# microsoft/VidTok

Hardware: AMD Instinct MI355X
Metric: encode+decode frames/sec, vidtok_kl_causal_488_4chn 17x256x256 (higher is better)
Workload: dtype bf16; 1 GPU; vidtok_kl_causal_488_4chn forward (encode+KL+decode), bf16, B=4 clips/GPU, 17x256x256; global_batch=4, launch=hipGraph replay (engine graph cache)

## Files before the change

### include/vidtok_amd.h

```cpp
#ifndef VIDTOK_AMD_H
#define VIDTOK_AMD_H

#include <stddef.h>
#include <stdint.h>

#ifdef __cplusplus
extern "C" {
#endif

typedef void* vt_stream;

typedef enum vt_status {
  VT_OK = 0,
  VT_ERR_ARG = -1,
  VT_ERR_HIP = -2,
  VT_ERR_UNSUPPORTED = -3
} vt_status;

typedef enum vt_dtype { VT_F32 = 0, VT_BF16 = 1, VT_I32 = 2, VT_BF16X3 = 3 , VT_F16 = 4 } vt_dtype;

typedef enum vt_tmode {
  VT_TPAD_ZERO = 0,
  VT_TPAD_REPLICATE = 1,
  VT_TPAD_CACHE = 2,
  VT_TPAD_ZERO_BACK = 3
} vt_tmode;

typedef enum vt_resmode {
  VT_RES_NONE = 0,
  VT_RES_ADD = 1,
  VT_RES_MIX = 2
} vt_resmode;

typedef enum vt_layout { VT_NDHWC = 0, VT_NCTHW = 1 } vt_layout;

const char* vt_last_error(void);
int vt_version(void);
int vt_graph_launch(void* graph_exec, vt_stream stream);
int vt_conv_max_lds_bytes(void);

int vt_set_option(const char* name, int32_t value);
int vt_get_option(const char* name, int32_t* value);
int vt_reset_options(void);
int vt_option_count(void);
const char* vt_option_name(int32_t i);

typedef struct vt_conv_desc {
  const void* x;
  const void* w;
  const float* bias;
  void* y;
  const void* res;
  const void* cache;
  const float* mix_factor;
  const float* ln_gamma;
  const float* ln_beta;
  void* ln_out;
  int32_t B, Ti, Hi, Wi, Cin;
  int32_t To, Ho, Wo, Cout;
  int32_t ldw;
  int32_t ldy;
  int32_t KT, KH, KW;
  int32_t st, sh, sw;
  int32_t pt, ph, pw;
  int32_t tmode, ncache;
  int32_t ups_t, ups_s;
  int32_t res_mode;
  int32_t res_tshift;
  int32_t Tr, ldr;
  int32_t out_layout;
  int32_t t_trim;
  int32_t dtype;
  int32_t out_dtype;
  int32_t nbatch;
  int32_t ln_mode;
  int32_t ln_keep_y;
  int32_t ldn;
  int32_t yt_mul, yt_off;
  int32_t ys_mul, ys_oh, ys_ow;
  float ln_eps;
  int64_t xs_z, ws_z, ys_z, rs_z;
  void* work;
  int64_t work_bytes;
} vt_conv_desc;

int vt_conv(const vt_conv_desc* d, vt_stream stream);
int64_t vt_conv_work_bytes(const vt_conv_desc* d);
int vt_conv_plan(const vt_conv_desc* d, int32_t* out8);
int vt_conv_profile(const vt_conv_desc* d, uint64_t* stamps_out, vt_stream stream);
int vt_conv_desc_size(void);

typedef struct vt_tblock_desc {
  const void* x;
  void* y;
  void* n_out;
  const void* w1; const float* b1;
  const void* w2; const float* b2;
  const float* norm1_gamma; const float* norm1_beta;
  const float* norm2_gamma; const float* norm2_beta;
  const float* next_gamma; const float* next_beta;
  int32_t dtype;
  int32_t C, ld;
  int32_t B, T;
  int64_t HW;
  int32_t tmode;
  int32_t keep_y;
  int32_t ln_next_mode;
  float eps;
  int32_t cache_offset;
  void* cache1;
  void* cache2;
} vt_tblock_desc;

int vt_tblock_desc_size(void);
int vt_temporal_block_supported(const vt_tblock_desc* d);
int vt_temporal_block(const vt_tblock_desc* d, vt_stream stream);
int vt_temporal_block_profile(const vt_tblock_desc* d, uint64_t* stamps_out, vt_stream stream);

int vt_layernorm_act(const void* x, int in_dtype, int64_t ldx, void* y, int out_dtype, int64_t ldy,
                     const float* gamma, const float* beta, int64_t M, int32_t C, float eps,
                     int32_t silu, vt_stream stream);

typedef enum { VT_GN_FRAME = 0, VT_GN_PIXEL = 1, VT_GN_CLIP = 2 } vt_gn_scope;
int64_t vt_groupnorm_work_bytes(int32_t B, int32_t T, int32_t groups, int32_t scope);
int vt_groupnorm_act(const void* x, int in_dtype, int64_t ldx, void* y, int out_dtype, int64_t ldy,
                     const float* gamma, const float* beta, int32_t B, int32_t T, int64_t HW, int32_t C,
                     int32_t groups, int32_t scope, float eps, int32_t silu, void* work, vt_stream stream);

int vt_flash_attention_supported(int32_t dtype, int32_t S, int32_t C, int32_t ldv);
int vt_flash_attention(const void* q, const void* k, const void* vt, const float* bias_v, void* o, int32_t dtype, int32_t Z, int32_t S,
                       int32_t C, int32_t ldv, float scale, vt_stream stream);

int vt_tanh_inplace(float* x, int64_t n, vt_stream stream);
int vt_softmax_rows(const float* s, void* p, int out_dtype, int64_t rows, int32_t cols,
                    int64_t ldp, float scale, vt_stream stream);

int vt_ncthw_to_ndhwc(const float* x, void* y, int out_dtype, int32_t B, int32_t C, int32_t T,
                      int32_t H, int32_t W, int32_t ldy, int32_t tpad, vt_stream stream);
int vt_ndhwc_to_ncthw(const void* x, int in_dtype, float* y, int32_t B, int32_t C, int32_t T,
                      int32_t H, int32_t W, int32_t ldx, int32_t ttrim, vt_stream stream);

int vt_time_avgpool3s2(const void* x, const void* cache, void* y, int dtype, int32_t B, int32_t Ti,
                       int64_t HW, int32_t C, int32_t tmode, vt_stream stream);
int vt_time_lerp2x(const void* x, void* y, int dtype, int32_t B, int32_t Ti, int64_t HWC,
                   vt_stream stream);
int vt_time_lerp2x_cat(const void* head, int32_t nh, const void* x, void* y, int dtype, int32_t B, int32_t Tx, int32_t skip,
                       int64_t HWC, vt_stream stream);

int vt_pack_conv_weight(const float* w, void* out, int32_t out_dtype, int32_t Cout, int32_t Cin, int32_t cin_p, int32_t taps_in,
                        int32_t taps_out, const int32_t* mix_host, int64_t ldw, vt_stream stream);

int vt_fsq_consts(const int32_t* levels_host, int32_t D, float* out_host);
int vt_kl_sample(const float* h, const float* noise, float* z, float* kl_out, int32_t B,
                 int32_t zc, int64_t S, vt_stream stream);
int vt_fsq_quantize(const float* h, float* z, int32_t* indices, const int32_t* levels_host,
                    int32_t D, int32_t B, int64_t S, vt_stream stream);
int vt_fsq_indices_to_codes(const int32_t* indices, float* z, const int32_t* levels_host,
                            int32_t D, int32_t B, int64_t S, vt_stream stream);
int vt_fsq_quantize_cb(const float* h, float* z, int32_t* indices, const int32_t* levels_host,
                       int32_t D, int32_t B, int32_t ncb, int64_t S, vt_stream stream);
int vt_fsq_indices_to_codes_cb(const int32_t* indices, float* z, const int32_t* levels_host,
                               int32_t D, int32_t B, int32_t ncb, int64_t S, vt_stream stream);
int64_t vt_fsq_aux_work_floats(const int32_t* levels_host, int32_t D, int32_t B, int64_t S);
int vt_fsq_aux_stats(const float* h, const int32_t* levels_host, int32_t D, int32_t B, int64_t S,
                     float inv_temperature, float* work, float* out3, vt_stream stream);
int vt_fsq_aux_stats_avg(const float* h, const int32_t* levels_host, int32_t D, int32_t B, int64_t S,
                         float inv_temperature, float* work, float* out3, float* avg_out, vt_stream stream);
int vt_fsq_aux_loss(const float* stats3, const float* codebook_entropy, float diversity_gamma, float entropy_weight,
                    float commitment_weight, float* out, vt_stream stream);
int vt_entropy(const float* avg, int64_t J, float* out, vt_stream stream);

typedef struct vt_model_config {
  int32_t version;
// ... 164 lines not shown
```

### vidtok_amd/build.py

```python
import hashlib
import os
import shutil
import subprocess
import sys

HERE = os.path.dirname(os.path.abspath(__file__))
CSRC = os.path.join(HERE, "csrc")
LIB = os.path.join(HERE, "libvidtok_amd.so")
SOURCES = ["conv_igemm_bf16.hip", "conv_igemm_f16.hip", "conv_igemm_f32.hip", "conv_igemm_x3.hip", "conv_igemm_act.hip", "conv_igemm.hip", "conv_in8.hip", "conv_ws2.hip", "conv_narrow.hip", "tblock_ws128.hip", "attention.hip", "pointwise.hip", "groupnorm.hip", "regularizers.hip", "metrics.hip", "lpips.hip", "lpips_grad.hip", "video_io.hip", "segments.hip", "grad.hip", "grad_decoder.hip", "packing.hip", "error.cpp", "options.cpp", "model.cpp"]
HEADERS = ["common.h", "conv_common.h", "conv_select.h", "conv_igemm_kernel.h", "options.h", "row8.h", os.path.join("..", "..", "include", "vidtok_amd.h")]
FLAGS = ["--offload-arch=gfx950", "-O3", "-std=c++17", "-fPIC", "-Wall", "-Wno-unused-function"]
EXTRA_FLAGS = {"conv_ws2.hip": ["-fno-slp-vectorize"], "tblock_ws128.hip": ["-fno-slp-vectorize"]}


NO_SPILL = {"tblock_ws128.hip": "tblock_pair_kernel", "conv_ws2.hip": "conv3x3_ws2_kernel"}
LLVM_BIN = "/opt/rocm/lib/llvm/bin"


def kernel_resources(obj):
    import re
    import tempfile
    with tempfile.TemporaryDirectory() as d:
        fat, dev = os.path.join(d, "fat.bin"), os.path.join(d, "dev.o")
        subprocess.check_call([f"{LLVM_BIN}/llvm-objcopy", "--dump-section", f".hip_fatbin={fat}", obj])
        subprocess.check_call([f"{LLVM_BIN}/clang-offload-bundler", "--unbundle", "--type=o", f"--input={fat}",
                               "--targets=hipv4-amdgcn-amd-amdhsa--gfx950", f"--output={dev}"])
        notes = subprocess.check_output([f"{LLVM_BIN}/llvm-readelf", "--notes", dev], text=True)
    out = []
    for blk in notes.split("- .agpr_count:")[1:]:
        g = lambda k: re.search(r"\." + k + r":\s+(\S+)", blk).group(1)
        out.append((g("name"), int(g("vgpr_count")), int(blk.split()[0]), int(g("vgpr_spill_count")), int(g("private_segment_fixed_size"))))
    return out


def check_no_spill(objdir):
    if not all(os.path.exists(os.path.join(LLVM_BIN, t)) for t in ("llvm-objcopy", "clang-offload-bundler", "llvm-readelf")):
        print("[vidtok_amd.build] spill check skipped: LLVM binutils not found under", LLVM_BIN, flush=True)
        return
    bad = []
    for src, kern in NO_SPILL.items():
        obj = os.path.join(objdir, os.path.splitext(src)[0] + ".o")
        for name, _v, _a, spill, scratch in kernel_resources(obj):
            measured = name.endswith("Lb1EEEvNS_10TBlockArgsE") or name.endswith("Lb1EEEvNS_8ConvArgsE")
            if kern in name and not measured and (spill or scratch):
                bad.append(f"{name}: {spill} spilled registers, {scratch} B scratch")
    if bad:
        raise RuntimeError("register spills in hand-scheduled kernels (wrong results, not only slow):\n  " + "\n  ".join(bad))


def _hipcc():
    for c in (os.environ.get("HIPCC"), shutil.which("hipcc"), "/opt/rocm/bin/hipcc"):
        if c and os.path.exists(c):
            return c
    raise RuntimeError("hipcc not found (set HIPCC)")


def _src_digest(src):
    h = hashlib.sha256()
    for f in [src] + HEADERS:
        with open(os.path.join(CSRC, f), "rb") as fh:
            h.update(fh.read())
    h.update(" ".join(FLAGS + EXTRA_FLAGS.get(src, [])).encode())
    return h.hexdigest()


def _digest():
    h = hashlib.sha256()
    for src in SOURCES:
        h.update(_src_digest(src).encode())
    return h.hexdigest()


def build(force: bool = False, verbose: bool = True) -> str:
    stamp = LIB + ".stamp"
    dig = _digest()
    if not force and os.path.exists(LIB) and os.path.exists(stamp) and open(stamp).read() == dig:
        return LIB
    hipcc = _hipcc()
    objdir = os.path.join(HERE, "build")
    os.makedirs(objdir, exist_ok=True)
    objs = []
    procs = []
    for src in SOURCES:
        obj = os.path.join(objdir, os.path.splitext(src)[0] + ".o")
        objs.append(obj)
        ostamp, odig = obj + ".stamp", _src_digest(src)
        if not force and os.path.exists(obj) and os.path.exists(ostamp) and open(ostamp).read() == odig:
            continue
        if os.path.exists(ostamp):
            os.remove(ostamp)
        cmd = [hipcc, *FLAGS, *EXTRA_FLAGS.get(src, []), "-x", "hip", "-c", os.path.join(CSRC, src), "-o", obj]
        if verbose:
            print("[vidtok_amd.build]", " ".join(cmd), flush=True)
        procs.append((src, subprocess.Popen(cmd), ostamp, odig))
    failed = []
    for src, p, ostamp, odig in procs:
        if p.wait() != 0:
            failed.append(src)
        else:
            with open(ostamp, "w") as f:
                f.write(odig)
    if failed:
        raise RuntimeError(f"hipcc failed on {', '.join(failed)}")
    check_no_spill(objdir)
    cmd = [hipcc, "--offload-arch=gfx950", "-shared", "-fPIC", *objs, "-o", LIB]
    if verbose:
        print("[vidtok_amd.build]", " ".join(cmd), flush=True)
    subprocess.check_call(cmd)
    with open(stamp, "w") as f:
        f.write(dig)
    return LIB


if __name__ == "__main__":
    build(force="--force" in sys.argv)
    print(LIB)
```

### vidtok_amd/csrc/conv_common.h

```cpp
#pragma once
#include "common.h"
#include "options.h"

namespace {

constexpr int kRowBytes = 128;

struct FastDiv {
  unsigned mul, shift, d;
};
inline FastDiv make_fastdiv(unsigned d) {
  FastDiv f;
  f.d = d;
  if (d <= 1) { f.mul = 0; f.shift = 0; return f; }
  unsigned l = 0;
  while ((1ull << l) < d) ++l;
  f.mul = (unsigned)((((1ull << 32) * ((1ull << l) - d)) / d) + 1);
  f.shift = l - 1;
  return f;
}
__device__ __forceinline__ unsigned fast_div(unsigned n, const FastDiv& f) {
  if (f.d <= 1) return n;
  const unsigned t = __umulhi(n, f.mul);
  return (t + ((n - t) >> 1)) >> f.shift;
}

struct ConvArgs;
__device__ __forceinline__ long long out_row(const ConvArgs& p, int m);

struct ConvArgs {
  const char* x;
  const char* w;
  const float* bias;
  char* y;
  const char* res;
  const char* cache;
  const float* mix_factor;
  const float* ln_gamma;
  const float* ln_beta;
  char* ln_out;
  int B, Ti, Hi, Wi, Cin;
  int To, Ho, Wo, Cout;
  int ldw, ldy;
  int KT, KH, KW;
  int st, sh, sw;
  int pt, ph, pw;
  int tmode, ncache;
  int ups_t, ups_s;
  int res_mode, res_tshift, Tr, ldr;
  int out_layout, t_trim;
  int M, K, ntaps, nsteps;
  int m_tiles, n_tiles;
  int ln_mode, ln_keep_y, ldn;
  float ln_eps;
  FastDiv fd_wo, fd_ho, fd_to;
  FastDiv fd_hw;
  int yt_mul;
  long long yt_step, yt_base;
  int ys_mul, ys_oh, ys_ow;
  int lds_epi;
  int hw_tiles;
  unsigned x_bytes, w_bytes;
  unsigned c_bytes;
  long long xs_z, ws_z, ys_z, rs_z;
  int in8_rt, in8_ct, in8_ctl2, in8_segs;
  int tskip;
  int ksplit;
  unsigned plane_bytes;
  int nt_store;
  unsigned long long* prof;
  int prof_mode;
};

struct split3_t {
  float v;
};
template <typename MT>
struct is_split3 {
  [[maybe_unused]] static constexpr bool value = false;
};
template <>
struct is_split3<split3_t> {
  [[maybe_unused]] static constexpr bool value = true;
};
template <typename MT>
struct storage_of {
  typedef MT type;
};
template <>
struct storage_of<split3_t> {
  typedef float type;
};

__device__ __forceinline__ void split3_x(const u32x4& r0, const u32x4& r1, u32x4& hi, u32x4& lo) {
#pragma unroll
  for (int e = 0; e < 4; ++e) {
    const float f0 = __uint_as_float(e < 2 ? r0[2 * e] : r1[2 * e - 4]);
    const float f1 = __uint_as_float(e < 2 ? r0[2 * e + 1] : r1[2 * e - 3]);
    const uint32_t h = pack_bf16x2(f0, f1);
    hi[e] = h;
    float d0, d1;
    asm("v_sub_f32_e32 %0, %1, %2" : "=v"(d0) : "v"(f0), "v"(h << 16));
    asm("v_sub_f32_e32 %0, %1, %2" : "=v"(d1) : "v"(f1), "v"(h & 0xffff0000u));
    lo[e] = pack_bf16x2(d0, d1);
  }
}
__device__ __forceinline__ void mma_bf16(const u32x4& wfrag, const u32x4& xfrag, f32x16& acc) {
  acc = __builtin_amdgcn_mfma_f32_32x32x16_bf16(__builtin_bit_cast(bf16x8, wfrag), __builtin_bit_cast(bf16x8, xfrag), acc, 0, 0, 0);
}

template <typename MT>
__device__ __forceinline__ void mma_step(const u32x4& wfrag, const u32x4& xfrag, f32x16& acc);

template <>
__device__ __forceinline__ void mma_step<bf16_t>(const u32x4& wfrag, const u32x4& xfrag, f32x16& acc) {
  acc = __builtin_amdgcn_mfma_f32_32x32x16_bf16(__builtin_bit_cast(bf16x8, wfrag),
                                                __builtin_bit_cast(bf16x8, xfrag), acc, 0, 0, 0);
}
template <>
__device__ __forceinline__ void mma_step<f16_t>(const u32x4& wfrag, const u32x4& xfrag, f32x16& acc) {
  acc = h16<f16_t>::mfma32(wfrag, xfrag, acc);
}
template <>
__device__ __forceinline__ void mma_step<float>(const u32x4& wfrag, const u32x4& xfrag, f32x16& acc) {
#pragma unroll
  for (int e = 0; e < 4; ++e)
    acc = __builtin_amdgcn_mfma_f32_32x32x2f32(__uint_as_float(wfrag[e]), __uint_as_float(xfrag[e]),
                                               acc, 0, 0, 0);
}

__device__ __forceinline__ int xcd_remap(int bid, int nblk) {
  const int xcd = bid & 7, loc = bid >> 3;
  const int q = nblk >> 3, r = nblk & 7;
  const int start = (xcd < r) ? xcd * (q + 1) : r * (q + 1) + (xcd - r) * q;
  return start + loc;
}

template <typename TOut>
struct Quad;
template <>
struct Quad<float> {
  f32x4 v;
  __device__ __forceinline__ float get(int e) const { return v[e]; }
};
template <typename H>
struct Quad16 {
  u32x2 v;
  __device__ __forceinline__ float get(int e) const {
    const uint32_t w = v[e >> 1];
    return (e & 1) ? h16<H>::hi(w) : h16<H>::lo(w);
  }
};
template <>
struct Quad<bf16_t> : Quad16<bf16_t> {};
// ... 95 lines not shown
```

### vidtok_amd/csrc/conv_igemm.hip

```cpp
#include <algorithm>
#include <atomic>
#include <type_traits>

#include "conv_select.h"

namespace {

template <typename H>
__global__ __launch_bounds__(256) void splitk_reduce_kernel(const float* __restrict__ part, int planes, long long M, int Cout, const float* __restrict__ bias,
                                                            const H* __restrict__ res, H* __restrict__ y) {
  const long long n8 = M * (Cout / 8);
  const long long plane = M * (long long)Cout;
  for (long long i = (long long)blockIdx.x * blockDim.x + threadIdx.x; i < n8; i += (long long)gridDim.x * blockDim.x) {
    const long long e = i * 8;
    const int c = (int)(e % Cout);
    float v[8];
    {
      const f32x4 a = *reinterpret_cast<const f32x4*>(part + e), b = *reinterpret_cast<const f32x4*>(part + e + 4);
#pragma unroll
      for (int k = 0; k < 4; ++k) { v[k] = a[k]; v[4 + k] = b[k]; }
    }
    for (int pz = 1; pz < planes; ++pz) {
      const f32x4 a = *reinterpret_cast<const f32x4*>(part + pz * plane + e), b = *reinterpret_cast<const f32x4*>(part + pz * plane + e + 4);
#pragma unroll
// ... 54 lines not shown
  return VT_OK;
}

}

extern "C" int vt_conv_max_lds_bytes(void) { return 163840; }

extern "C" int vt_conv_plan(const vt_conv_desc* d, int32_t* out8) {
  VT_CHECK_ARG(out8 != nullptr, "vt_conv_plan: null output");
  ConvArgs a;
  ConvPlan p;
  const int rc = conv_decide(d, a, p);
  if (rc != VT_OK) return rc;
  out8[4] = p.ln_fused ? 1 : 0;
  out8[5] = 1;
  out8[6] = p.kernel;
  out8[7] = 0;
  switch (p.kernel) {
    case CONV_NARROW:
      vt_conv_narrow_plan(&a, out8);
      out8[5] = p.narrow_mode == 2 ? 2 : 1;
      break;
    case CONV_WS2:
      out8[0] = 64; out8[1] = 128; out8[2] = 8;
      out8[3] = (a.Wo / 16) * (a.Ho / 4) * a.B * a.To;
      break;
    case CONV_IN8:
      out8[0] = 128; out8[1] = 128; out8[2] = 4;
      out8[3] = a.M / 128;
      out8[7] = 1;
      break;
    case CONV_IGEMM: {
      const TileShape& t = kTileShapes[p.igemm.tile];
      out8[0] = t.bm(); out8[1] = t.bn(); out8[2] = t.waves();
      out8[3] = (int32_t)((long long)((a.M + t.bm() - 1) / t.bm()) * ((a.Cout + t.bn() - 1) / t.bn()) * p.nbatch);
      if (d->ln_mode != 0 && !p.ln_fused) out8[5] += 1;
      if (splitk_runs(p, a, d, false)) out8[5] += 1;
      out8[7] = p.igemm.tile == TILE_256x256 ? (p.igemm.ln256 ? 1 : 0) : (p.igemm.stages == 4 ? 2 : 0);
      break;
    }
  }
  return VT_OK;
}

extern "C" int vt_conv_profile(const vt_conv_desc* d, uint64_t* stamps_out, vt_stream stream_) {
  VT_CHECK_ARG(stamps_out != nullptr, "vt_conv_profile: null output");
  ConvArgs a;
  ConvPlan p;
  const int rc = conv_decide(d, a, p, reinterpret_cast<unsigned long long*>(stamps_out));
  if (rc != VT_OK) return rc;
  a.prof_mode = vt_opt(OPT_WS_PROF_MODE);
  if (p.kernel == CONV_WS2) return vt_ws2_launch(&a, d->dtype, stream_);
  VT_CHECK_ARG(p.kernel == CONV_IGEMM && ((d->dtype == VT_BF16 && d->out_dtype == VT_BF16) || d->dtype == VT_BF16X3) && d->ln_mode == 0 &&
                   p.igemm.tile == TILE_256x256,
               "vt_conv_profile: bf16 / split-bf16 launches on the 256 x 256 tile without LayerNorm, or on the weight-stationary kernel");
  return launch_igemm(d->dtype, false, a, p.igemm, p.nbatch, stream_);
}

extern "C" int64_t vt_conv_work_bytes(const vt_conv_desc* d) {
  ConvArgs a;
  ConvPlan p;
  if (conv_decide(d, a, p) != VT_OK || p.kernel != CONV_IGEMM) return 0;
  return (int64_t)p.splitk_planes * a.M * a.Cout * 4;
}

extern "C" int vt_conv(const vt_conv_desc* d, vt_stream stream_) {
  ConvArgs a;
  ConvPlan p;
  int rc = conv_decide(d, a, p);
  if (rc != VT_OK) return rc;
  switch (p.kernel) {
    case CONV_WS2: return vt_ws2_launch(&a, d->dtype, stream_);
    case CONV_NARROW: return vt_conv_narrow_launch(&a, stream_, p.narrow_mode);
    case CONV_IN8: return vt_conv_in8_launch(&a, d->dtype, stream_);
    case CONV_IGEMM: break;
  }
  rc = splitk_runs(p, a, d, true) ? launch_splitk(d, a, p, reinterpret_cast<hipStream_t>(stream_))
                                  : launch_igemm(d->dtype, d->out_dtype == VT_F32, a, p.igemm, p.nbatch, stream_);
  if (rc != VT_OK || d->ln_mode == 0 || p.ln_fused) return rc;
  return vt_layernorm_act(d->y, d->out_dtype, d->ldy, d->ln_out, d->out_dtype, d->ldn, d->ln_gamma, d->ln_beta, a.M, d->Cout,
                          d->ln_eps, d->ln_mode == 2 ? 1 : 0, stream_);
}

extern "C" int vt_conv_act(const vt_conv_desc* d, int32_t act, vt_stream stream_) {
  VT_CHECK_ARG(act == VT_ACT_RELU, "vt_conv_act: act %d (VT_ACT_RELU = %d is the one activation)", act, VT_ACT_RELU);
  ConvArgs a;
  ConvPlan p;
  const int rc = conv_decide(d, a, p, nullptr, act);
  if (rc != VT_OK) return rc;
  VT_CHECK_ARG(d->dtype != VT_BF16X3 && d->out_dtype == d->dtype, "vt_conv_act: fp32, bf16 or fp16 arithmetic with results in the same type");
  VT_CHECK_ARG(d->out_layout == VT_NDHWC && d->res_mode == VT_RES_NONE && d->ln_mode == 0 && p.nbatch == 1 && a.yt_mul == 1 && a.ys_mul == 1,
               "vt_conv_act: NDHWC output without residual, LayerNorm, batching or interleave");
  return vt_igemm_dispatch_relu(&a, &p.igemm, d->dtype, stream_);
}
```

### vidtok_amd/csrc/conv_igemm_kernel.h

```cpp
#include <atomic>
#include <type_traits>

#pragma once
#include "conv_select.h"

namespace {

__device__ __forceinline__ float act_relu(float v) { return v > 0.0f ? v : 0.0f; }

template <typename TOut, int TM, int TN, bool GENERAL = true, int ACT = 0>
__device__ __forceinline__ void conv_epilogue(const ConvArgs& p, f32x16 (&acc)[TN][TM], int m_blk, int n_blk, int bn_tile,
                                              int wm, int wn, int lane, long long z) {
  TOut* __restrict__ yg = reinterpret_cast<TOut*>(p.y) + z * p.ys_z;
  const TOut* __restrict__ rg = reinterpret_cast<const TOut*>(p.res) + z * p.rs_z;
  const long long HWo = (long long)p.Ho * p.Wo;
  const bool has_res = p.res_mode != VT_RES_NONE;
  const int nlast = p.Cout - 1;
  const int nq = n_blk + wn * TN * 32 + 4 * (lane >> 5);

  float alpha = 0.0f;
  if (p.res_mode == VT_RES_MIX) alpha = 1.0f / (1.0f + __expf(-p.mix_factor[0]));

  bool store_ok[TM];
  long long mr[TM], ybase[TM];
// ... 259 lines not shown
    {
      const int prl = wm * 32 + (lane & 31);
#pragma unroll
      for (int a = 0; a < 4; ++a)
#pragma unroll
        for (int g = 0; g < 4; ++g) {
          const int c = wn * 128 + 32 * a + 8 * g + 4 * h;
          f32x4 bq;
          if (p.bias) bq = *reinterpret_cast<const f32x4*>(p.bias + n_blk + c);
          else bq[0] = bq[1] = bq[2] = bq[3] = 0.0f;
          f32x4 v;
#pragma unroll
          for (int e = 0; e < 4; ++e) v[e] = acc[a][PZ][4 * g + e] + bq[e];
          *reinterpret_cast<f32x4*>(T + prl * 256 + (((c >> 2) ^ (prl & 63)) << 2)) = v;
        }
    }
    __syncthreads();
#pragma unroll
    for (int it = 0; it < 8; ++it) {
      const int r = rsub + RS * it;
      const int m = m_blk + ((RS * it) >> 5) * 64 + PZ * 32 + rsub + ((RS * it) & 31);
      const long long orow = out_row(p, m);
      const f32x4 t0 = *reinterpret_cast<const f32x4*>(T + r * 256 + (((2 * j) ^ (r & 63)) << 2));
      const f32x4 t1 = *reinterpret_cast<const f32x4*>(T + r * 256 + (((2 * j + 1) ^ (r & 63)) << 2));
      f32x2 v[4] = {f32x2{t0[0], t0[1]}, f32x2{t0[2], t0[3]}, f32x2{t1[0], t1[1]}, f32x2{t1[2], t1[3]}};
      if (p.res_mode == VT_RES_ADD) {
#pragma unroll
        for (int q = 0; q < 4; ++q) v[q] = f32x2{rq[it].get(2 * q), rq[it].get(2 * q + 1)} + v[q];
      } else if (p.res_mode == VT_RES_MIX) {
#pragma unroll
        for (int q = 0; q < 4; ++q) v[q] = f32x2{rq[it].get(2 * q), rq[it].get(2 * q + 1)} * alpha + v[q] * (1.0f - alpha);
      }
      if constexpr (ACT == VT_ACT_RELU) {
#pragma unroll
        for (int q = 0; q < 4; ++q) v[q] = f32x2{act_relu(v[q][0]), act_relu(v[q][1])};
      }
      if (p.ln_keep_y || !has_ln) {
        const float yv[8] = {v[0][0], v[0][1], v[1][0], v[1][1], v[2][0], v[2][1], v[3][0], v[3][1]};
        Oct<TOut>::store(yg + orow * p.ldy + n_blk + 8 * j, yv, p.nt_store != 0);
      }
      if (!has_ln) continue;
      float o[8];
      if constexpr (sizeof(TOut) == 2) {
        const f32x2 s = (v[0] + v[1]) + (v[2] + v[3]);
        f32x2 qq = v[0] * v[0];
#pragma unroll
        for (int q = 1; q < 4; ++q) qq = __builtin_elementwise_fma(v[q], v[q], qq);
        float nm;
        const float rstd = ln_row_stats<32>(s[0] + s[1], qq[0] + qq[1], p.ln_eps, &nm);
        const f32x2 rstd2 = {rstd, rstd}, nm2 = {nm, nm}, c2 = {kNegLog2e, kNegLog2e};
#pragma unroll
        for (int q = 0; q < 4; ++q) {
          f32x2 u = __builtin_elementwise_fma(__builtin_elementwise_fma(v[q], rstd2, nm2), lg[q], lb[q]);
          if (p.ln_mode == 2) {
            const f32x2 den = __builtin_elementwise_fma(f32x2{__builtin_amdgcn_exp2f(u[0]), __builtin_amdgcn_exp2f(u[1])}, c2, c2);
            u = u * f32x2{__builtin_amdgcn_rcpf(den[0]), __builtin_amdgcn_rcpf(den[1])};
          }
          o[2 * q] = u[0];
          o[2 * q + 1] = u[1];
        }
      } else {
        const f32x2 s = (v[0] + v[1]) + (v[2] + v[3]);
        const float mean = group_sum_dpp<32>(s[0] + s[1]) * (1.0f / 256.0f);
        f32x2 d[4], qq = {0.f, 0.f};
#pragma unroll
        for (int q = 0; q < 4; ++q) {
          d[q] = v[q] - mean;
          qq = __builtin_elementwise_fma(d[q], d[q], qq);
        }
        const float rstd = __builtin_amdgcn_rsqf(__builtin_fmaf(group_sum_dpp<32>(qq[0] + qq[1]), 1.0f / 256.0f, p.ln_eps));
#pragma unroll
        for (int q = 0; q < 4; ++q) {
          f32x2 u = __builtin_elementwise_fma(d[q] * rstd, lg[q], lb[q]);
          if (p.ln_mode == 2) {
            const f32x2 t = u * -1.4426950408889634f;
            const f32x2 e = f32x2{__builtin_amdgcn_exp2f(t[0]), __builtin_amdgcn_exp2f(t[1])} + 1.0f;
            u = u * f32x2{__builtin_amdgcn_rcpf(e[0]), __builtin_amdgcn_rcpf(e[1])};
          }
          o[2 * q] = u[0];
          o[2 * q + 1] = u[1];
        }
      }
      Oct<TOut>::store(ng + orow * p.ldn + 8 * j, o, p.nt_store != 0);
    }
  };
  half(std::integral_constant<int, 0>{});
  half(std::integral_constant<int, 1>{});
}

[[maybe_unused]] __device__ u32x4 g_zero_page[8];


template <typename MT, typename TOut, int WAVES_M, int WAVES_N, int TM, int TN, bool FAST, int ROWB, int STAGES, bool BUF, int LN256 = 0, bool PROF = false, int SCHED = 0, int ACT = 0>
__global__ __launch_bounds__(64 * WAVES_M * WAVES_N, 2) void conv_igemm_glds_kernel(const ConvArgs p) {
#if defined(__HIP_DEVICE_COMPILE__)
  constexpr int THREADS = 64 * WAVES_M * WAVES_N;
  constexpr int NS = ROWB / 16;
  constexpr int RSTEP = THREADS / NS;
  constexpr int ROWS_PER_WAVE = 64 / NS;
  constexpr int SWZ_SHIFT = (ROWB == 128) ? 1 : 2;
  constexpr int VEC = 16 / (int)sizeof(MT);
  constexpr int BK = ROWB / (int)sizeof(MT);
  constexpr int KS = ROWB / 32;
  constexpr int BM = WAVES_M * TM * 32;
  constexpr int BN = WAVES_N * TN * 32;
  constexpr int A_VECS = BM * NS / THREADS;
  constexpr int B_VECS = BN * NS / THREADS;
  constexpr int IPS = A_VECS + B_VECS;
  constexpr int A_BYTES = BM * ROWB;
  constexpr int STAGE_BYTES = (BM + BN) * ROWB;
  constexpr int D = STAGES - 1;
  constexpr bool X3 = is_split3<MT>::value;
  static_assert(ROWB == 128 || ROWB == 64, "row bytes");
  static_assert(A_VECS >= 1 && B_VECS >= 1 && BM % RSTEP == 0 && BN % RSTEP == 0, "tile / workgroup mismatch");
  static_assert(D >= 1 && D <= 3 && (D - 1) * IPS <= 63, "pipeline depth");

  extern __shared__ __attribute__((aligned(16))) char smem[];
  typedef __attribute__((address_space(3))) void* lds_ptr_t;
  typedef const __attribute__((address_space(1))) void* glb_ptr_t;

  const int tid = threadIdx.x;
  const int lane = tid & 63;
  const int wave = tid >> 6;
  const int wm = wave % WAVES_M;
  const int wn = wave / WAVES_M;

  const int tile = xcd_remap(blockIdx.x, p.m_tiles * p.n_tiles);
  const int nt = tile / p.m_tiles;
  int mt = tile - nt * p.m_tiles;
  if (p.hw_tiles > 0) {
    const int per_b = p.hw_tiles * p.To;
    const int b = mt / per_b;
    const int r = mt - b * per_b;
    const int hwt = r / p.To;
    mt = (b * p.To + (r - hwt * p.To)) * p.hw_tiles + hwt;
  }
  const int m_blk = mt * BM;
  const int n_blk = nt * BN;

  const long long z = blockIdx.z;
  const MT* __restrict__ xg = reinterpret_cast<const MT*>(p.x) + z * p.xs_z;
  const MT* __restrict__ wg = reinterpret_cast<const MT*>(p.w) + z * p.ws_z;
  const MT* __restrict__ cg = reinterpret_cast<const MT*>(p.cache);
  const MT* zero = reinterpret_cast<const MT*>(g_zero_page);
  constexpr unsigned kOob = 0xFFFF0000u;
  unsigned ext_x = BUF ? p.x_bytes : 0u, ext_w = BUF ? p.w_bytes : 0u;
  const MT* x_cur = xg;
  if constexpr (PROF) {
    if (p.prof_mode & 1) ext_x = 0u;
    if (p.prof_mode & 2) ext_w = 0u;
  }

  const int pos = tid % NS;
  const int srow = tid / NS;
  const int chunk = pos ^ ((srow >> SWZ_SHIFT) & (NS - 1));
  const int lds_row_off = __builtin_amdgcn_readfirstlane(wave * ROWS_PER_WAVE * ROWB);

  const int Hv = p.Hi << p.ups_s, Wv = p.Wi << p.ups_s;
  const int Tv = p.Ti << p.ups_t;

  int a_b[A_VECS], a_t0[A_VECS], a_h0[A_VECS], a_w0[A_VECS];
#pragma unroll
  for (int i = 0; i < A_VECS; ++i) {
    const int m = m_blk + srow + RSTEP * i;
    if (m < p.M) {
      const unsigned r1 = fast_div((unsigned)m, p.fd_wo);
// ... 527 lines not shown
    read_frags(0, 0, 0);
    for (int s = 0; s < nsteps; ++s) {
      s_cur = s;
      stamp(0);
      const bool fire = s < n_fire;
      if (!fire && BUF) ext_x = ext_w = 0u;
      const bool fire_rt = BUF || fire;
      const int dst = (stage + D) % STAGES;
      const int nxt = (stage + 1 == STAGES) ? 0 : stage + 1;
#pragma unroll
      for (int k = 0; k < KS; ++k) {
        if (((k ^ wgrp) & 1) == 0) __builtin_amdgcn_s_setprio(2);
        else __builtin_amdgcn_s_setprio(0);
        if (k + 1 < KS) read_frags(stage, k + 1, (k + 1) & 1);
#pragma unroll
        for (int qq = 0; qq < TM * TN; ++qq) {
          const int a = qq / TM, b = qq % TM;
          const int q = k * TM * TN + qq;
          if (k + 1 == KS && qq == BAR_AT) {
            stamp(1);
            asm volatile("s_waitcnt lgkmcnt(0)" ::: "memory");
            wait_vmcnt<(D - 1) * IPS>();
            stamp(2);
            __builtin_amdgcn_s_barrier();
            asm volatile("" ::: "memory");
            stamp(3);
            read_frags(nxt, 0, 0);
          }
          mma_step<MT>(wf[k & 1][a], xf[k & 1][b], acc[a][b]);
          if ((q + 1) % MPP1 == 0) {
            const int piece = q / MPP1;
            if (piece < IPS && fire_rt) fire_piece(piece, dst);
          }
          if (q + 1 == NM / 2) {
            if (s + 1 < n_fire) prep_step(s + 1 + D);
          }
        }
      }
      stage = nxt;
      stamp(4);
    }
    __builtin_amdgcn_s_setprio(0);
  } else {
  for (int s = 0; s < nsteps; ++s) {
    s_cur = s;
    stamp(0);
    const int newer = min(D - 1, nsteps - 1 - s);
    if (D >= 3 && newer >= 2) wait_vmcnt<2 * IPS>();
    else if (D >= 2 && newer >= 1) wait_vmcnt<IPS>();
    else wait_vmcnt<0>();
    stamp(1);
    __builtin_amdgcn_s_barrier();
    asm volatile("" ::: "memory");
    stamp(2);
    const bool fire = s < n_fire;
    if (fire) prep_step(s + D);
    else if (BUF) ext_x = ext_w = 0u;
    const bool fire_rt = BUF || fire;
    stamp(3);
    if (EIGHT_WAVES) {
      compute_stage(stage, TagTrue{}, fire_rt, (stage + D) % STAGES);
    } else {
      if (fire_rt) {
#pragma unroll
        for (int q = 0; q < IPS; ++q) fire_piece(q, (stage + D) % STAGES);
      }
      compute_stage(stage, TagFalse{}, false, 0);
    }
    stage = (stage + 1 == STAGES) ? 0 : stage + 1;
    stamp(4);
  }
  }
  if constexpr (BUF) wait_vmcnt<0>();
  if constexpr (PROF) {
    if (blockIdx.x == 0 && blockIdx.y == 0 && blockIdx.z == 0 && lane == 0 && p.prof != nullptr) {
      constexpr int NW = THREADS / 64;
      for (int i = 0; i < 4 * 8; ++i) p.prof[(tid >> 6) * 32 + i] = stamps[((i / 8) * NW + (tid >> 6)) * 8 + (i % 8)];
    }
  }
  if constexpr (LN256 != 0) {
    static_assert(WAVES_M == 4 && WAVES_N == 2 && TM == 2 && TN == 4 && std::is_same<typename storage_of<MT>::type, TOut>::value, "LN256: the 8-wave 256 x 256 tile");
    static_assert(STAGES * STAGE_BYTES >= 128 * 256 * 4, "LN256: the transposition tile must fit the ring");
    if constexpr (!BUF) wait_vmcnt<0>();
    conv_epilogue_lds256<TOut, ACT>(p, acc, m_blk, n_blk, wm, wn, lane, tid, smem, z);
    return;
  }
  if constexpr (WAVES_M == 2 && WAVES_N == 2 && TM == 2 && TN == 2 && STAGES * STAGE_BYTES >= 128 * 128 * 4) {
    if (p.lds_epi && m_blk + BM <= p.M && n_blk + BN <= p.Cout) {
      if constexpr (!BUF) wait_vmcnt<0>();
      conv_epilogue_lds128<TOut, ACT>(p, acc, m_blk, n_blk, wm, wn, lane, tid, smem, z);
      return;
    }
  }
  conv_epilogue<TOut, TM, TN, (TM * TN < 8), ACT>(p, acc, m_blk, n_blk, BN, wm, wn, lane, z);
#endif
}

template <typename MT, typename TOut, int WAVES_M, int WAVES_N, int TM, int TN, bool FAST, int LN256 = 0, int STAGES = 2, int ROWB = kRowBytes, int ACT = 0>
int launch_variant(const ConvArgs& a_in, int nbatch, hipStream_t stream) {
  constexpr int BM = WAVES_M * TM * 32;
  constexpr int BN = WAVES_N * TN * 32;
  constexpr int BK = ROWB / (int)sizeof(MT);
  constexpr int THREADS = 64 * WAVES_M * WAVES_N;
  constexpr int LDS = STAGES * (BM + BN) * ROWB;
  ConvArgs a = a_in;
  a.m_tiles = (a.M + BM - 1) / BM;
  a.n_tiles = (a.Cout + BN - 1) / BN;
  a.nsteps = FAST ? a.ntaps * (a.Cin / BK) : (a.K + BK - 1) / BK;
  if (a.ksplit) {
    VT_CHECK_ARG(FAST, "vt_conv: split-K needs the tap-walk form");
    a.nsteps = (a.ksplit == 1 ? a.KH * a.KW : a.KW) * (a.Cin / BK);
  }
  constexpr int kOctAlign = 16 / (int)sizeof(TOut) > 4 ? 8 : 4;
  a.lds_epi = (vt_opt(OPT_CONV_LDSEPI) != 0 && a.out_layout == VT_NDHWC && a.ldy % kOctAlign == 0 &&
               (a.res_mode == VT_RES_NONE || a.ldr % kOctAlign == 0) && (a.ln_mode == 0 || a.ldn % kOctAlign == 0)) ? 1 : 0;
  a.hw_tiles = 0;
  if (conv_tinner() && a.KT > 1 && a.To > 1 && ((long long)a.Ho * a.Wo) % BM == 0) a.hw_tiles = (int)(((long long)a.Ho * a.Wo) / BM);
  const unsigned long long xb = (unsigned long long)a.B * a.Ti * a.Hi * a.Wi * a.Cin * sizeof(MT);
  const unsigned long long wb = (unsigned long long)a.Cout * a.ldw * sizeof(MT);
  const unsigned long long cb = a.tmode == VT_TPAD_CACHE ? (unsigned long long)a.B * a.ncache * a.Hi * a.Wi * a.Cin * sizeof(MT) : 0ull;
  const bool cache_ok = a.tmode != VT_TPAD_CACHE ||
                        (FAST && (nbatch == 1 || a.ksplit) && a.prof == nullptr && cb < 0xFFFF0000ull && ((long long)a.Ho * a.Wo) % BM == 0 && a.ups_t == 0);
  const bool buf = conv_buf() && xb < 0xFFFF0000ull && wb < 0xFFFF0000ull && cache_ok &&
                   a.KH <= 8 && a.KW <= 8;
  VT_CHECK_ARG(!a.ksplit || buf, "vt_conv: split-K needs the descriptor gather");
  a.tskip = (FAST && buf && vt_opt(OPT_CONV_TSKIP) != 0 && a.tmode == VT_TPAD_ZERO && a.KT > 1 && a.pt > 0 && a.ups_t == 0 && !a.ksplit &&
             nbatch == 1 && a.prof == nullptr && ((long long)a.Ho * a.Wo) % BM == 0) ? 1 : 0;
  constexpr bool EIGHT = WAVES_M * WAVES_N == 8;
  constexpr int SCHED_BUF = !(EIGHT && FAST) ? 0
                            : (is_split3<MT>::value ? ((ROWB == 64 && STAGES == 4) ? 5 : 0)
                               : ((ROWB == kRowBytes && STAGES == 2) ? (is_h16<MT>::value ? 2 : 1) : 0));
  const void* kern;
  if (buf) {
    a.x_bytes = (unsigned)xb;
    a.w_bytes = (unsigned)wb;
    a.c_bytes = (unsigned)cb;
    kern = reinterpret_cast<const void*>(&conv_igemm_glds_kernel<MT, TOut, WAVES_M, WAVES_N, TM, TN, FAST, ROWB, STAGES, true, LN256, false, SCHED_BUF, ACT>);
  } else {
    kern = reinterpret_cast<const void*>(&conv_igemm_glds_kernel<MT, TOut, WAVES_M, WAVES_N, TM, TN, FAST, ROWB, STAGES, false, LN256, false, 0, ACT>);
  }
  int lds_bytes = LDS;
  static std::atomic<bool> attr_done[3][kMaxDevices];
  int ki = buf ? 1 : 0;
  if (a.prof != nullptr) {
    if constexpr (EIGHT && FAST && LN256 == 0 && ACT == 0 && (SCHED_BUF == 2 || SCHED_BUF == 5) && !std::is_same<MT, f16_t>::value &&
                  std::is_same<typename storage_of<MT>::type, TOut>::value) {
      VT_CHECK_ARG(buf, "vt_conv_profile: descriptor gather only");
      kern = reinterpret_cast<const void*>(&conv_igemm_glds_kernel<MT, TOut, WAVES_M, WAVES_N, TM, TN, FAST, ROWB, STAGES, true, 0, true, SCHED_BUF>);
      lds_bytes = LDS + 4096;
      ki = 2;
    } else {
      VT_CHECK_ARG(false, "vt_conv_profile: only the bf16 / split-bf16 8-wave 256 x 256 tile without fused LayerNorm is instrumented");
    }
  }
  if (const int rc = vt_dynamic_lds(kern, lds_bytes, attr_done[ki])) return rc;
  const long long nblk = (long long)a.m_tiles * a.n_tiles;
  VT_CHECK_ARG(nblk < (1ll << 31), "vt_conv: too many tiles (%lld)", nblk);
  void* kargs[] = {&a};
  VT_CHECK_HIP(hipLaunchKernel(kern, dim3((unsigned)nblk, 1, (unsigned)nbatch), dim3(THREADS), kargs, lds_bytes, stream));
  return VT_OK;
}

template <typename MT, typename TOut, TileKind T, bool FAST, int LN256 = 0, int STAGES = 2, int ROWB = kRowBytes, int ACT = 0>
int launch_tile(const ConvArgs& a, int nbatch, hipStream_t stream) {
  constexpr TileShape S = kTileShapes[T];
  return launch_variant<MT, TOut, S.wm, S.wn, S.tm, S.tn, FAST, LN256, STAGES, ROWB, ACT>(a, nbatch, stream);
}

#define VT_CHECK_VARIANT(cond) \
  VT_CHECK_ARG(cond, "vt_conv: no instantiation of tile %d with fast %d, ln256 %d, stages %d, row bytes %d in this arithmetic", (int)v.tile, (int)v.fast, v.ln256, v.stages, v.rowb)

template <typename MT, typename TOut, TileKind T>
int launch_fast_or_general(const ConvArgs& a, const IgemmVariant& v, int nbatch, hipStream_t stream) {
  VT_CHECK_VARIANT(v.ln256 == 0 && v.stages == 2 && v.rowb == kRowBytes);
  return v.fast ? launch_tile<MT, TOut, T, true>(a, nbatch, stream) : launch_tile<MT, TOut, T, false>(a, nbatch, stream);
}

template <typename MT, typename TOut>
int dispatch_tile(const ConvArgs& a, const IgemmVariant& v, int nbatch, hipStream_t stream) {
  switch (v.tile) {
    case TILE_256x32: return launch_fast_or_general<MT, TOut, TILE_256x32>(a, v, nbatch, stream);
    case TILE_256x64: return launch_fast_or_general<MT, TOut, TILE_256x64>(a, v, nbatch, stream);
    case TILE_256x256:
      if constexpr (is_split3<MT>::value) {
        if (v.rowb == 64) {
          VT_CHECK_VARIANT(v.fast && v.stages == 4);
          return v.ln256 ? launch_tile<MT, TOut, TILE_256x256, true, 1, 4, 64>(a, nbatch, stream) : launch_tile<MT, TOut, TILE_256x256, true, 0, 4, 64>(a, nbatch, stream);
        }
      } else if constexpr (std::is_same<MT, TOut>::value) {
        if (v.ln256) {
          VT_CHECK_VARIANT(v.fast && v.stages == 2 && v.rowb == kRowBytes);
          return launch_tile<MT, TOut, TILE_256x256, true, 1>(a, nbatch, stream);
        }
      }
      return launch_fast_or_general<MT, TOut, TILE_256x256>(a, v, nbatch, stream);
    default:
      if (v.stages == 4) {
        VT_CHECK_VARIANT(v.tile == TILE_128x128 && v.fast && v.ln256 == 0 && v.rowb == kRowBytes);
        return launch_tile<MT, TOut, TILE_128x128, true, 0, 4>(a, nbatch, stream);
      }
      return launch_fast_or_general<MT, TOut, TILE_128x128>(a, v, nbatch, stream);
  }
}

}
```

### vidtok_amd/csrc/conv_select.h

```cpp
#pragma once
#include "conv_common.h"

namespace {

inline bool conv_buf() { return vt_opt(OPT_CONV_BUF) != 0; }
inline bool conv_tinner() { return vt_opt(OPT_CONV_TINNER) != 0; }

inline bool in8_eligible(const ConvArgs& a, int nbatch, int dtype, int out_dtype, bool ln_fused, int ln_mode_asked) {
  if (vt_opt(OPT_CONV_IN8) == 0 || !conv_buf() || nbatch != 1 || a.prof != nullptr) return false;
  if (!vt_is_h16(dtype) || out_dtype != dtype || a.Cin != 8 || a.Cout != 128 || a.ldw != 216) return false;
  if (a.KT != 3 || a.KH != 3 || a.KW != 3 || a.st != 1 || a.sh != 1 || a.sw != 1 || a.pt != 2 || a.ph != 1 || a.pw != 1) return false;
  if (a.To != a.Ti || a.Ho != a.Hi || a.Wo != a.Wi || a.ups_t || a.ups_s || a.tmode == VT_TPAD_CACHE) return false;
  if (a.out_layout != VT_NDHWC || a.res_mode != VT_RES_NONE || a.yt_mul != 1 || a.ys_mul == 2) return false;
  if (a.Wo < 8 || !((a.Wo % 128 == 0) || (128 % a.Wo == 0)) || ((long long)a.Ho * a.Wo) % 128 != 0) return false;
  if (ln_mode_asked != 0 && !ln_fused) return false;
  if (a.ldy % 8 != 0 || (a.ln_mode != 0 && a.ldn % 8 != 0) || vt_opt(OPT_CONV_LDSEPI) == 0) return false;
  const unsigned long long xb = (unsigned long long)a.B * a.Ti * a.Hi * a.Wi * 8 * 2;
  return xb < 0xFFFF0000ull;
}

inline bool deep_ring_eligible(const ConvArgs& a, int nbatch, int elem_bytes) {
  if (vt_opt(OPT_CONV_DEEP) == 0 || a.prof != nullptr) return false;
  const int bk = kRowBytes / elem_bytes;
  if (a.Cin % bk != 0 || a.ntaps * (a.Cin / bk) < 8) return false;
  const long long tiles = (long long)((a.M + 127) / 128) * ((a.Cout + 127) / 128) * nbatch;
  return tiles <= device_cus();
}

enum TileKind { TILE_256x32 = 0, TILE_256x64, TILE_256x256, TILE_128x128 };
struct TileShape {
  int wm, wn, tm, tn;
  constexpr int bm() const { return wm * tm * 32; }
  constexpr int bn() const { return wn * tn * 32; }
  constexpr int waves() const { return wm * wn; }
};
constexpr TileShape kTileShapes[4] = {{4, 1, 2, 1}, {4, 1, 2, 2}, {4, 2, 2, 4}, {2, 2, 2, 2}};

inline bool ws_eligible(const ConvArgs& a, int nbatch, bool h16_io) {
  if (!h16_io || vt_opt(OPT_CONV_WS) == 0) return false;
  if (a.Cin != 128 || a.Cout != 128 || a.ldw != 1152 || a.ldy != 128) return false;
  if (a.KT != 1 || a.KH != 3 || a.KW != 3 || a.st != 1 || a.sh != 1 || a.sw != 1 || a.ph != 1 || a.pw != 1) return false;
  if (a.ups_t || a.ups_s || a.Ho != a.Hi || a.Wo != a.Wi || a.To != a.Ti) return false;
  if (a.Ho % 8 != 0 || a.Wo % 16 != 0 || (long long)a.Ho * a.Wo * 256 > (1ll << 30)) return false;
  if (a.out_layout != VT_NDHWC || a.yt_mul != 1 || a.ys_mul == 2 || nbatch != 1) return false;
  if (a.res_mode == VT_RES_MIX) return false;
  if (a.res_mode == VT_RES_ADD && (a.ldr != 128 || a.Tr != a.To || a.res_tshift != 0 || (reinterpret_cast<uintptr_t>(a.res) & 15))) return false;
  if ((reinterpret_cast<uintptr_t>(a.y) & 15) || (a.bias && (reinterpret_cast<uintptr_t>(a.bias) & 15))) return false;
  return true;
}

inline bool narrow_eligible(const ConvArgs& a, int nbatch, int dtype, int out_dtype, int ln_mode) {
  if ((!vt_is_h16(dtype) && dtype != VT_BF16X3) || out_dtype != VT_F32 || a.out_layout != VT_NCTHW || vt_opt(OPT_CONV_NARROW) == 0) return false;
  if (a.Cin != 128 || a.Cout > 4 || a.KT != 3 || a.KH != 3 || a.KW != 3) return false;
  if (a.st != 1 || a.sh != 1 || a.sw != 1 || a.ph != 1 || a.pw != 1 || a.pt < 1 || a.pt > 2) return false;
  if (a.ups_t || a.ups_s || a.Ho != a.Hi || a.Wo != a.Wi || a.To != a.Ti) return false;
  if (a.res_mode != VT_RES_NONE || ln_mode != 0 || nbatch != 1 || a.yt_mul != 1 || a.ys_mul == 2) return false;
  if ((long long)a.Ho * a.Wo * 256 > (1ll << 30)) return false;
  if (a.tmode == VT_TPAD_CACHE && a.ncache < a.pt) return false;
  if (dtype == VT_BF16X3 && a.ldw != 27 * 128) return false;
  return true;
}

inline TileKind select_tile(const ConvArgs& a, int nbatch) {
  auto blocks = [&](int bm, int bn) {
    return (long long)((a.M + bm - 1) / bm) * ((a.Cout + bn - 1) / bn) * nbatch;
  };
  const bool vec_epi = a.out_layout == VT_NDHWC && (a.ldy & 3) == 0 && (a.res_mode == VT_RES_NONE || (a.ldr & 3) == 0);
  if (a.Cout <= 32) return TILE_256x32;
  if (a.Cout <= 64) return TILE_256x64;
  const int force = vt_opt(OPT_CONV_TILE);
  if (a.Cout % 256 == 0 && vec_epi && force != 128 && (blocks(256, 256) >= vt_opt(OPT_CONV_TILE_MIN) || force == 256)) return TILE_256x256;
  return TILE_128x128;
}

inline bool lds256_plain_eligible(const ConvArgs& a, int nbatch, bool h16_io) {
  return h16_io && a.ln_mode == 0 && a.prof == nullptr && vt_opt(OPT_CONV_LDSEPI) != 0 &&
         a.M % 256 == 0 && a.Cout % 256 == 0 && nbatch == 1 && a.Cin % (kRowBytes / 2) == 0 && a.out_layout == VT_NDHWC &&
         (a.ldy & 7) == 0 && (a.res_mode == VT_RES_NONE || ((a.ldr & 7) == 0 && a.Tr == a.To && a.res_tshift == 0));
}

struct IgemmVariant {
  TileKind tile;
  bool fast;
  int ln256;
  int stages;
  int rowb;
};

enum ConvKernel { CONV_IGEMM = 0, CONV_NARROW = 2, CONV_WS2 = 3, CONV_IN8 = 4 };

struct ConvPlan {
  ConvKernel kernel;
  IgemmVariant igemm;
  IgemmVariant split;
  int splitk_planes;
  bool ln_fused;
  int nbatch;
  int narrow_mode;
};

inline int splitk_planes(const vt_conv_desc* d, const ConvArgs& a, const ConvPlan& p, TileKind tile) {
  if (vt_opt(OPT_CONV_SPLITK) == 0 || !conv_buf()) return 0;
  if (!vt_is_h16(d->dtype) || d->out_dtype != d->dtype || p.nbatch != 1 || p.ln_fused || a.prof != nullptr) return 0;
  const bool by_kt = a.KT == 3 && a.st == 1, by_kh = a.KT == 1 && a.KH == 3;
  if (!(by_kt || by_kh) || a.ups_t || a.ups_s || a.out_layout != VT_NDHWC || a.yt_mul != 1 || a.ys_mul == 2) return 0;
  if (a.Cin % 64 != 0 || a.Cout % 128 != 0 || a.ldy != a.Cout || a.KT * a.KH * a.KW * a.Cin < 4608) return 0;
  if (a.res_mode == VT_RES_MIX || (a.res_mode == VT_RES_ADD && (a.ldr != a.Cout || a.Tr != a.To || a.res_tshift != 0))) return 0;
  if (a.tmode == VT_TPAD_CACHE && ((long long)a.Ho * a.Wo) % 256 != 0) return 0;
  const unsigned long long xb = (unsigned long long)a.B * a.Ti * a.Hi * a.Wi * a.Cin * 2, wb = (unsigned long long)a.Cout * a.ldw * 2;
  if (xb >= 0xFFFF0000ull || wb >= 0xFFFF0000ull) return 0;
  if (tile != TILE_256x256 && tile != TILE_128x128) return 0;
  const long long clip_tiles = (((long long)a.To * a.Ho * a.Wo + 127) / 128) * ((a.Cout + 127) / 128);
  return clip_tiles <= device_cus() ? 3 : 0;
}

inline int conv_decide(const vt_conv_desc* d, ConvArgs& a, ConvPlan& p, unsigned long long* prof = nullptr, int act = 0) {
  VT_CHECK_ARG(d != nullptr, "vt_conv: null descriptor");
  VT_CHECK_ARG(d->x && d->w && d->y, "vt_conv: null tensor pointer");
  VT_CHECK_ARG(d->dtype == VT_F32 || d->dtype == VT_BF16 || d->dtype == VT_F16 || d->dtype == VT_BF16X3, "vt_conv: dtype %d", d->dtype);
  VT_CHECK_ARG((d->out_dtype == d->dtype && d->dtype != VT_BF16X3) || d->out_dtype == VT_F32, "vt_conv: out_dtype %d with dtype %d",
               d->out_dtype, d->dtype);
  const int vec = vt_is_h16(d->dtype) ? 8 : 4;
  if (d->dtype == VT_BF16X3)
    VT_CHECK_ARG(d->ldw % 32 == 0 && d->ldw >= (d->KT * d->KH * d->KW * d->Cin + 31) / 32 * 32 && d->nbatch <= 1,
                 "vt_conv: VT_BF16X3 needs ldw = K rounded up to 32 (got %d) and nbatch 1", d->ldw);
  VT_CHECK_ARG(d->B > 0 && d->Ti > 0 && d->Hi > 0 && d->Wi > 0 && d->Cin > 0, "vt_conv: bad input dims");
  VT_CHECK_ARG(d->To > 0 && d->Ho > 0 && d->Wo > 0 && d->Cout > 0, "vt_conv: bad output dims");
  VT_CHECK_ARG(d->Cin % vec == 0, "vt_conv: Cin=%d must be a multiple of %d (pad the channel dim)", d->Cin, vec);
  VT_CHECK_ARG(d->KT > 0 && d->KH > 0 && d->KW > 0 && d->KT * d->KH * d->KW <= 64, "vt_conv: bad taps");
  VT_CHECK_ARG(d->st > 0 && d->sh > 0 && d->sw > 0, "vt_conv: bad strides");
  VT_CHECK_ARG(d->ldw >= d->KT * d->KH * d->KW * d->Cin && d->ldw % vec == 0, "vt_conv: ldw=%d", d->ldw);
  VT_CHECK_ARG((reinterpret_cast<uintptr_t>(d->x) & 15) == 0 && (reinterpret_cast<uintptr_t>(d->w) & 15) == 0,
               "vt_conv: x / w must be 16-byte aligned");
  VT_CHECK_ARG(d->ups_t == 0 || d->ups_t == 1, "vt_conv: ups_t");
  VT_CHECK_ARG(d->ups_s == 0 || d->ups_s == 1, "vt_conv: ups_s");
  VT_CHECK_ARG(d->tmode >= VT_TPAD_ZERO && d->tmode <= VT_TPAD_CACHE, "vt_conv: tmode %d", d->tmode);
  if (d->tmode == VT_TPAD_CACHE && d->pt > 0) {
    VT_CHECK_ARG(d->cache != nullptr && d->ncache >= d->pt, "vt_conv: cache mode needs cache with >= pt frames");
    VT_CHECK_ARG(d->ups_t == 0, "vt_conv: cache mode with ups_t");
    VT_CHECK_ARG((reinterpret_cast<uintptr_t>(d->cache) & 15) == 0, "vt_conv: cache must be 16-byte aligned");
  }
  VT_CHECK_ARG(d->res_mode >= VT_RES_NONE && d->res_mode <= VT_RES_MIX, "vt_conv: res_mode %d", d->res_mode);
  if (d->res_mode != VT_RES_NONE) {
    VT_CHECK_ARG(d->res != nullptr && d->Tr > 0 && d->ldr >= d->Cout, "vt_conv: residual operand");
    VT_CHECK_ARG(((d->To - 1) >> d->res_tshift) < d->Tr, "vt_conv: residual time extent");
  }
  if (d->res_mode == VT_RES_MIX) VT_CHECK_ARG(d->mix_factor != nullptr, "vt_conv: mix_factor is null");
  if (d->out_layout == VT_NCTHW) {
    VT_CHECK_ARG(d->out_dtype == VT_F32, "vt_conv: NCTHW output is fp32 only");
    VT_CHECK_ARG(d->t_trim >= 0 && d->t_trim < d->To, "vt_conv: t_trim");
  } else {
    VT_CHECK_ARG(d->out_layout == VT_NDHWC && d->ldy >= d->Cout, "vt_conv: ldy=%d < Cout=%d", d->ldy, d->Cout);
  }
  const long long M = (long long)d->B * d->To * d->Ho * d->Wo;
  VT_CHECK_ARG(M < (1ll << 31), "vt_conv: M too large");
  const int nbatch = d->nbatch > 0 ? d->nbatch : 1;
  const int yt_mul = d->yt_mul > 0 ? d->yt_mul : 1;
  if (yt_mul != 1)
    VT_CHECK_ARG(d->out_layout == VT_NDHWC && nbatch == 1 && d->yt_off >= 0 && d->yt_off < yt_mul,
                 "vt_conv: output frame interleave needs NDHWC, nbatch 1 and 0 <= yt_off < yt_mul");
  const int ys_mul = d->ys_mul == 2 ? 2 : 1;
  VT_CHECK_ARG(d->ys_mul == 0 || d->ys_mul == 1 || d->ys_mul == 2, "vt_conv: ys_mul %d", d->ys_mul);
  if (ys_mul == 2)
    VT_CHECK_ARG(d->out_layout == VT_NDHWC && nbatch == 1 && yt_mul == 1 && (d->ys_oh | d->ys_ow | 1) == 1,
                 "vt_conv: output pixel interleave needs NDHWC, nbatch 1, no frame interleave, offsets in {0,1}");
  if (d->ln_mode != 0) {
    VT_CHECK_ARG(d->ln_mode == 1 || d->ln_mode == 2, "vt_conv: ln_mode %d", d->ln_mode);
    VT_CHECK_ARG(d->ln_gamma && d->ln_beta && d->ln_out, "vt_conv: fused LayerNorm needs gamma, beta and ln_out");
    VT_CHECK_ARG(d->out_layout == VT_NDHWC && nbatch == 1 && d->ldn >= d->Cout, "vt_conv: fused LayerNorm: NDHWC, nbatch 1, ldn >= Cout");
  }

  memset(&a, 0, sizeof(a));
  a.x = (const char*)d->x; a.w = (const char*)d->w; a.bias = d->bias; a.y = (char*)d->y;
  a.res = (const char*)d->res; a.cache = (const char*)d->cache; a.mix_factor = d->mix_factor;
  a.B = d->B; a.Ti = d->Ti; a.Hi = d->Hi; a.Wi = d->Wi; a.Cin = d->Cin;
  a.To = d->To; a.Ho = d->Ho; a.Wo = d->Wo; a.Cout = d->Cout;
  a.ldw = d->ldw; a.ldy = d->ldy;
  a.KT = d->KT; a.KH = d->KH; a.KW = d->KW;
  a.st = d->st; a.sh = d->sh; a.sw = d->sw;
  a.pt = d->pt; a.ph = d->ph; a.pw = d->pw;
  a.tmode = d->tmode; a.ncache = d->ncache;
  a.ups_t = d->ups_t; a.ups_s = d->ups_s;
  a.res_mode = d->res_mode; a.res_tshift = d->res_tshift;
  a.Tr = d->res_mode != VT_RES_NONE ? d->Tr : d->To;
  a.ldr = d->ldr;
  a.nt_store = (vt_opt(OPT_CONV_NT_MB) > 0 && M * d->Cout * (vt_is_h16(d->out_dtype) ? 2 : 4) >= ((long long)vt_opt(OPT_CONV_NT_MB) << 20)) ? 1 : 0;
  a.out_layout = d->out_layout; a.t_trim = d->t_trim;
  a.M = (int)M; a.ntaps = d->KT * d->KH * d->KW; a.K = a.ntaps * d->Cin;
  a.ys_mul = ys_mul; a.ys_oh = d->ys_oh; a.ys_ow = d->ys_ow;
  a.yt_mul = yt_mul;
  a.yt_step = (long long)(yt_mul - 1) * d->Ho * d->Wo;
  a.yt_base = (long long)(yt_mul != 1 ? d->yt_off : 0) * d->Ho * d->Wo;
  a.fd_hw = make_fastdiv((unsigned)(d->Ho * d->Wo));
  a.fd_wo = make_fastdiv((unsigned)d->Wo); a.fd_ho = make_fastdiv((unsigned)d->Ho); a.fd_to = make_fastdiv((unsigned)d->To);
  a.xs_z = d->xs_z; a.ws_z = d->ws_z; a.ys_z = d->ys_z; a.rs_z = d->rs_z;

// ... 73 lines not shown
```

### vidtok_amd/csrc/model.cpp

```cpp
#include <hip/hip_runtime.h>
#include <stdint.h>
#include <string.h>

#include <algorithm>
#include <cmath>
#include <map>
#include <memory>
#include <set>
#include <string>
#include <vector>

#include "../../include/vidtok_amd.h"

void vt_set_error(const char* fmt, ...);

namespace {

struct Fail {
  int code;
};
#define M_CHECK(cond, ...)        \
  do {                            \
    if (!(cond)) {                \
      vt_set_error(__VA_ARGS__);  \
      throw Fail{VT_ERR_ARG};     \
    }                             \
  } while (0)
#define M_CALL(expr)                 \
  do {                               \
    const int rc_ = (expr);          \
    if (rc_ != VT_OK) throw Fail{rc_}; \
  } while (0)
#define M_HIP(expr)                                                        \
  do {                                                                     \
    const hipError_t e_ = (expr);                                          \
    if (e_ != hipSuccess) {                                                \
      vt_set_error("%s: %s", #expr, hipGetErrorString(e_));                \
      throw Fail{VT_ERR_HIP};                                              \
    }                                                                      \
  } while (0)

int pad8(int c) { return (c + 7) / 8 * 8; }
size_t esize(int dt) { return dt == VT_F32 ? 4 : 2; }

uint16_t bf16_rne(float f) {
  uint32_t u;
  memcpy(&u, &f, 4);
  if ((u & 0x7fffffffu) > 0x7f800000u) return (uint16_t)((u >> 16) | 0x40);
  u += 0x7fffu + ((u >> 16) & 1u);
  return (uint16_t)(u >> 16);
}

struct Arena {
  char* base = nullptr;
  size_t cap = 0, off = 0, peak = 0;
  void reset() { off = 0; }
  char* alloc(size_t n, bool dry) {
    off = (off + 255) & ~(size_t)255;
    char* p = base + off;
    off += n;
    if (off > peak) peak = off;
    if (!dry) M_CHECK(off <= cap, "vt_model: workspace too small (%zu of %zu bytes in one arena; ask vt_workspace_bytes)", off, cap);
    return p;
  }
};

struct Tens {
  char* p = nullptr;
  int B = 0, T = 0, H = 0, W = 0, ld = 0, dt = VT_BF16;
  size_t bytes() const { return (size_t)B * T * H * W * ld * esize(dt); }
};

struct Norm;
struct Act {
  Tens y, n;
  const Norm* norm = nullptr;
  bool silu = false;
  bool has_n() const { return norm != nullptr; }
};
struct NormRef {
  const Norm* norm = nullptr;
  bool silu = false;
};

struct Param {
  std::vector<float> data;
  std::vector<int64_t> shape;
};

struct Model;
struct Ctx {
  Model* m;
  hipStream_t stream;
  bool dry;
  Arena* cur;
  Tens alloc(int B, int T, int H, int W, int ld, int dt, int c_real) {
    Tens t;
    t.B = B; t.T = T; t.H = H; t.W = W; t.ld = ld; t.dt = dt;
    t.p = cur->alloc(t.bytes(), dry);
    if (ld != c_real && !dry) M_HIP(hipMemsetAsync(t.p, 0, t.bytes(), stream));
    return t;
  }
};

struct DevBuf {
  void* p = nullptr;
  ~DevBuf() {
    if (p) (void)hipFree(p);
  }
};

struct CState {
  std::unique_ptr<DevBuf> buf;
  size_t cap = 0;
  int frames = 0;
  int offset = 0;
  size_t need = 0;
};

struct Model {
  vt_model_config cfg;
  bool tiled = false;
  bool first_chunk = true;
  std::vector<CState*> states;
  std::vector<std::unique_ptr<DevBuf>> retired;
  char* persistent(CState& st, size_t bytes, bool dry) {
    if (dry) {
      st.need = std::max(st.need, bytes);
      return nullptr;
    }
    if (st.cap < bytes) {
      auto b = std::make_unique<DevBuf>();
      if (hipMalloc(&b->p, bytes) != hipSuccess) {
        vt_set_error("vt_model: hipMalloc of a %zu-byte chunk cache failed", bytes);
        throw Fail{VT_ERR_HIP};
      }
      if (st.buf) retired.push_back(std::move(st.buf));
      st.buf = std::move(b);
      st.cap = bytes;
    }
    return (char*)st.buf->p;
  }
  int dt;
  bool x3 = false;
  bool v11() const { return cfg.version == 1; }
  bool noncausal() const { return cfg.version == 2; }
  std::string cv() const { return noncausal() ? "" : ".conv"; }
  int tpad() const { return v11() ? VT_TPAD_REPLICATE : VT_TPAD_ZERO; }
  std::map<std::string, Param> params;
  std::map<std::string, std::unique_ptr<DevBuf>> packed;
  std::unique_ptr<DevBuf> reg_buf;
  size_t reg_cap = 0;
  float* reg_scratch(size_t floats) {
    if (reg_cap < floats * 4) {
      auto b = std::make_unique<DevBuf>();
      if (hipMalloc(&b->p, floats * 4) != hipSuccess) {
        vt_set_error("vt_model: hipMalloc of the %zu-byte FSQ projection scratch failed", floats * 4);
        throw Fail{VT_ERR_HIP};
      }
      if (reg_buf) retired.push_back(std::move(reg_buf));
      reg_buf = std::move(b);
// ... 20 lines not shown
    void* p = b->p;
    packed[ckey] = std::move(b);
    return p;
  }
  const float* f32(const std::string& key, bool dry) {
    if (dry && !prepare) {
      expected.push_back(key);
      return nullptr;
    }
    auto it = packed.find("f32:" + key);
    if (it != packed.end()) return (const float*)it->second->p;
    const Param& p = param(key);
    return (const float*)upload("f32:" + key, p.data.data(), p.data.size() * 4);
  }
  typedef std::vector<float> (*Xform)(const Param&, std::vector<int64_t>& shape, int a, int b);
  const void* conv_w(const std::string& key, int cin_p, bool dry, Xform xf = nullptr, int xa = 0, int xb = 0, bool rows = false) {
    if (dry && !prepare) {
      expected.push_back(key);
      return nullptr;
    }
    const bool split = x3 && !rows;
    const std::string ckey = "w:" + key + ":" + std::to_string(cin_p) + ":" + std::to_string(dt) + (split ? "x3" : "") + ":" + std::to_string((xf ? 1 : 0) * 100 + xa * 10 + xb);
    auto it = packed.find(ckey);
    if (it != packed.end()) return it->second->p;
    const Param& p = param(key);
    std::vector<int64_t> shape = p.shape;
    std::vector<float> tmp;
    const float* src = p.data.data();
    if (xf) {
      tmp = xf(p, shape, xa, xb);
      src = tmp.data();
    }
    M_CHECK(shape.size() >= 3, "vt_model: '%s' is not a convolution weight", key.c_str());
    const int64_t cout = shape[0], cin = shape[1];
    int64_t taps = 1;
    for (size_t i = 2; i < shape.size(); ++i) taps *= shape[i];
    M_CHECK(cin <= cin_p, "vt_model: '%s' has %lld input channels, the activation stores %d", key.c_str(), (long long)cin, cin_p);
    std::vector<float> w((size_t)cout * taps * cin_p, 0.0f);
    for (int64_t o = 0; o < cout; ++o)
      for (int64_t c = 0; c < cin; ++c)
        for (int64_t t = 0; t < taps; ++t) w[((size_t)o * taps + t) * cin_p + c] = src[((size_t)o * cin + c) * taps + t];
    if (split) {
      const size_t K = (size_t)taps * cin_p, Kp = (K + 31) / 32 * 32;
      std::vector<uint16_t> pl((size_t)cout * Kp * 2, 0);
      for (int64_t o = 0; o < cout; ++o)
        for (size_t k = 0; k < K; ++k) {
          const float v = w[(size_t)o * K + k];
          const uint16_t hi = bf16_rne(v);
          uint32_t hb = (uint32_t)hi << 16;
          float hf;
          memcpy(&hf, &hb, 4);
          uint16_t* blk = &pl[((size_t)o * Kp + (k / 16) * 16) * 2];
          blk[k % 16] = hi;
          blk[16 + k % 16] = bf16_rne(v - hf);
        }
      return upload(ckey, pl.data(), pl.size() * 2);
    }
    if (dt == VT_F32) return upload(ckey, w.data(), w.size() * 4);
    std::vector<uint16_t> h(w.size());
    if (dt == VT_F16) {
      for (size_t i = 0; i < w.size(); ++i) {
        const _Float16 f = (_Float16)w[i];
        memcpy(&h[i], &f, 2);
      }
    } else {
      for (size_t i = 0; i < w.size(); ++i) h[i] = bf16_rne(w[i]);
    }
    return upload(ckey, h.data(), h.size() * 2);
  }
};

std::vector<float> xf_time_parity(const Param& p, std::vector<int64_t>& shape, int early, int) {
  const int64_t co = shape[0], ci = shape[1], hw = shape[3] * shape[4];
  std::vector<float> o((size_t)co * ci * 2 * hw);
  for (int64_t a = 0; a < co * ci; ++a)
    for (int64_t s = 0; s < hw; ++s) {
      const float w0 = p.data[(a * 3 + 0) * hw + s], w1 = p.data[(a * 3 + 1) * hw + s], w2 = p.data[(a * 3 + 2) * hw + s];
      o[(a * 2 + 0) * hw + s] = early ? w0 + w1 : w0;
      o[(a * 2 + 1) * hw + s] = early ? w2 : w1 + w2;
    }
  shape[2] = 2;
  return o;
}
std::vector<float> xf_space_parity(const Param& p, std::vector<int64_t>& shape, int py, int px) {
  const int64_t n = shape[0] * shape[1];
  std::vector<float> o((size_t)n * 4);
  for (int64_t a = 0; a < n; ++a) {
    const float* w = &p.data[a * 9];
    float rows[2][3];
    for (int c = 0; c < 3; ++c) {
      rows[0][c] = py == 0 ? w[0 * 3 + c] : w[0 * 3 + c] + w[1 * 3 + c];
      rows[1][c] = py == 0 ? w[1 * 3 + c] + w[2 * 3 + c] : w[2 * 3 + c];
    }
    for (int r = 0; r < 2; ++r) {
      o[a * 4 + r * 2 + 0] = px == 0 ? rows[r][0] : rows[r][0] + rows[r][1];
      o[a * 4 + r * 2 + 1] = px == 0 ? rows[r][1] + rows[r][2] : rows[r][2];
    }
  }
  shape[2] = 2;
  shape[3] = 2;
  return o;
}

struct Geom {
  int kt = 1, kh = 1, kw = 1, st = 1, sh = 1, sw = 1, pt = 0, ph = 0, pw = 0, ph_hi = 0, pw_hi = 0;
  int pt_hi = 0;
  void out_dims(int Ti, int Hi, int Wi, int& To, int& Ho, int& Wo) const {
    To = (Ti + pt + pt_hi - kt) / st + 1;
    Ho = (Hi + ph + ph_hi - kh) / sh + 1;
    Wo = (Wi + pw + pw_hi - kw) / sw + 1;
  }
};
Geom causal3d(int kt, int kh, int kw, int st = 1, int sh = 1, int sw = 1) {
  Geom g;
  g.kt = kt; g.kh = kh; g.kw = kw; g.st = st; g.sh = sh; g.sw = sw;
  g.pt = (kt - 1) + (1 - st);
  const int hp = (kh - 1) + (1 - sh), wp = (kw - 1) + (1 - sw);
  g.ph = hp / 2; g.pw = wp / 2; g.ph_hi = hp - hp / 2; g.pw_hi = wp - wp / 2;
  return g;
}
Geom centred(Geom g, int before) {
  g.pt_hi = g.pt - before;
  g.pt = before;
  return g;
}

struct Norm {
  std::string key;
  float eps = 1e-6f;
  bool group = false;
  int site = VT_GN_FRAME;
  std::string wkey() const { return key + (group ? ".weight" : ".norm.weight"); }
  std::string bkey() const { return key + (group ? ".bias" : ".norm.bias"); }
  Tens of(Ctx& c, const Tens& t, bool silu, int c_real) const {
    Tens o = c.alloc(t.B, t.T, t.H, t.W, t.ld, c.m->dt, c_real);
    const float* g = c.m->f32(wkey(), c.dry);
    const float* b = c.m->f32(bkey(), c.dry);
    if (!group) {
      if (!c.dry)
        M_CALL(vt_layernorm_act(t.p, t.dt, t.ld, o.p, o.dt, o.ld, g, b, (int64_t)t.B * t.T * t.H * t.W, c_real, eps, silu ? 1 : 0, c.stream));
      return o;
    }
    const int scope = site < 0 ? VT_GN_PIXEL : site;
    const int B = site < 0 ? 1 : t.B, T = site < 0 ? 1 : t.T;
    const int64_t HW = site < 0 ? (int64_t)t.B * t.T * t.H * t.W : (int64_t)t.H * t.W;
    const int64_t wb = std::max<int64_t>(vt_groupnorm_work_bytes(B, T, 32, scope), 8);
    void* work = c.cur->alloc((size_t)wb, c.dry);
    if (!c.dry) M_CALL(vt_groupnorm_act(t.p, t.dt, t.ld, o.p, o.dt, o.ld, g, b, B, T, HW, c_real, 32, scope, eps, silu ? 1 : 0, work, c.stream));
    return o;
  }
  Tens apply(Ctx& c, const Act& x, bool silu, int c_real) const {
    if (x.has_n() && x.norm == this && x.silu == silu) return x.n;
    return of(c, x.y, silu, c_real);
  }
  NormRef ref(bool silu) const { return group ? NormRef() : NormRef{this, silu}; }
};

struct ConvOpts {
  const Tens* res = nullptr;
  int res_mode = VT_RES_NONE;
  const float* mix = nullptr;
  NormRef ln;
  bool keep_y = true;
  Tens* out = nullptr;
  Tens* ln_out = nullptr;
  bool ln_optional = false;
  bool plan_only = false;
  int yt_mul = 1, yt_off = 0, ys = 0, ys_oh = 0, ys_ow = 0;
  float* ncthw = nullptr;
  int t_trim = 0;
  int tmode = VT_TPAD_ZERO;
  const void* cache = nullptr;
  int ncache = 0;
};

Act conv(Ctx& c, const Tens& x, const void* w, int ldw, const float* bias, const Geom& g, int cout, const ConvOpts& o) {
  int To, Ho, Wo;
  g.out_dims(x.T, x.H, x.W, To, Ho, Wo);
  M_CHECK(To > 0 && Ho > 0 && Wo > 0, "vt_model: convolution output is empty (%d x %d x %d)", To, Ho, Wo);
  Act r;
  vt_conv_desc d;
  memset(&d, 0, sizeof(d));
  int ldy;
  if (o.out) {
    r.y = *o.out;
    ldy = o.out->ld;
  } else if (o.ncthw) {
    ldy = cout;
  } else {
    ldy = pad8(cout);
    r.y = c.alloc(x.B, To, Ho, Wo, ldy, c.m->dt, cout);
  }
  d.x = x.p; d.w = w; d.bias = bias; d.y = o.ncthw ? (void*)o.ncthw : (void*)r.y.p;
  d.B = x.B; d.Ti = x.T; d.Hi = x.H; d.Wi = x.W; d.Cin = x.ld;
  d.To = To; d.Ho = Ho; d.Wo = Wo; d.Cout = cout;
  d.ldw = c.m->x3 ? (ldw + 31) / 32 * 32 : ldw; d.ldy = ldy;
  d.KT = g.kt; d.KH = g.kh; d.KW = g.kw; d.st = g.st; d.sh = g.sh; d.sw = g.sw; d.pt = g.pt; d.ph = g.ph; d.pw = g.pw;
  d.tmode = g.pt > 0 ? o.tmode : VT_TPAD_ZERO;
  if (d.tmode == VT_TPAD_CACHE) { d.cache = o.cache; d.ncache = o.ncache; }
  d.res_mode = o.res_mode;
  if (o.res_mode != VT_RES_NONE) {
    d.res = o.res->p; d.res_tshift = 0; d.Tr = o.res->T; d.ldr = o.res->ld;
    d.mix_factor = o.mix;
  }
  d.out_layout = o.ncthw ? VT_NCTHW : VT_NDHWC;
  d.t_trim = o.t_trim;
  d.dtype = c.m->x3 ? VT_BF16X3 : x.dt; d.out_dtype = o.ncthw ? VT_F32 : c.m->dt;
  d.nbatch = 1;
  d.yt_mul = o.yt_mul; d.yt_off = o.yt_off;
  if (o.ys) { d.ys_mul = 2; d.ys_oh = o.ys_oh; d.ys_ow = o.ys_ow; }
  const bool ln_after = o.ln.norm && o.ln.norm->group;
  if (o.ln.norm && !ln_after) {
    r.n = o.ln_out ? *o.ln_out : c.alloc(x.B, To, Ho, Wo, ldy, c.m->dt, cout);
    d.ln_gamma = c.m->f32(o.ln.norm->wkey(), c.dry);
    d.ln_beta = c.m->f32(o.ln.norm->bkey(), c.dry);
    d.ln_out = r.n.p;
    d.ln_mode = o.ln.silu ? 2 : 1; d.ln_keep_y = o.keep_y ? 1 : 0; d.ldn = ldy; d.ln_eps = o.ln.norm->eps;
    r.norm = o.ln.norm; r.silu = o.ln.silu;
  }
  auto standins = [&](vt_conv_desc& q) {
    if (!c.dry) return;
    q.x = q.w = q.y = (void*)16;
    if (q.res_mode != VT_RES_NONE) q.res = (void*)16;
    if (q.res_mode == VT_RES_MIX) q.mix_factor = (const float*)16;
    if (q.tmode == VT_TPAD_CACHE) q.cache = (void*)16;
    if (q.ln_mode != 0) { q.ln_gamma = q.ln_beta = (const float*)16; q.ln_out = (void*)16; }
  };
  if (o.ln_optional && d.ln_mode != 0) {
    vt_conv_desc q = d;
    standins(q);
    int32_t plan[8];
    if (q.ln_out == nullptr) q.ln_out = (void*)16;
    if (!(vt_conv_plan(&q, plan) == VT_OK && plan[4] == 1)) {
      d.ln_gamma = d.ln_beta = nullptr; d.ln_out = nullptr; d.ln_mode = 0;
      r.n = Tens(); r.norm = nullptr;
    }
  }
  if (o.plan_only) return r;
  {
    vt_conv_desc q = d;
    standins(q);
    const int64_t wb = ((x.dt == VT_BF16 || x.dt == VT_F16) && (g.kt == 3 || g.kh == 3)) ? vt_conv_work_bytes(&q) : 0;
    if (wb > 0) {
      d.work = c.cur->alloc((size_t)wb, c.dry);
      d.work_bytes = wb;
    }
  }
  if (!c.dry) M_CALL(vt_conv(&d, c.stream));
  if (ln_after) {
    M_CHECK(!o.out && !o.ncthw, "vt_model: GroupNorm of an interleaved / NCTHW result");
    r.n = o.ln.norm->of(c, r.y, o.ln.silu, cout);
    r.norm = o.ln.norm; r.silu = o.ln.silu;
  }
  return r;
}

void gather(Ctx& c, const char* src, int Ts, char* dst, int Td, int t0, const std::vector<int>& idx, int B, int64_t frame_elems, int es) {
  for (size_t j0 = 0; j0 < idx.size(); j0 += 128) {
    int32_t part[128];
    const int n = (int)std::min<size_t>(128, idx.size() - j0);
    for (int j = 0; j < n; ++j) part[j] = idx[j0 + j];
    if (!c.dry)
      M_CALL(vt_gather_frames(src, dst + (size_t)(t0 + (int)j0) * frame_elems * es, es, B, frame_elems, (int64_t)Ts * frame_elems, (int64_t)Td * frame_elems, part, n, c.stream));
  }
}

void update_cache(Ctx& c, CState& st, const Tens& x, int P) {
  if (P == 0) return;
  Model* m = c.m;
  const int T = x.T, off = st.offset, es = (int)esize(x.dt);
  const int64_t fr = (int64_t)x.H * x.W * x.ld;
  std::vector<int> sx, sc;
  int jx = -1, jc = -1;
  for (int j = 0; j < P; ++j) {
    const int q = T - off + j;
    M_CHECK(q >= 0, "vt_model: chunk of %d frames is shorter than its cache offset %d", T, off);
    if (q >= P) { if (jx < 0) jx = j; sx.push_back(q - P); }
    else if (m->first_chunk) { if (jx < 0) jx = j; sx.push_back(0); }
    else { if (jc < 0) jc = j; sc.push_back(q); }
  }
  char* kept = nullptr;
  if (!sc.empty()) {
    M_CHECK(c.dry || st.frames >= P, "vt_model: causal cache missing (the first chunk must come first)");
    kept = c.cur->alloc((size_t)x.B * sc.size() * fr * es, c.dry);
    gather(c, c.dry ? nullptr : (const char*)st.buf->p, P, kept, (int)sc.size(), 0, sc, x.B, fr, es);
  }
  char* buf = m->persistent(st, (size_t)x.B * P * fr * es, c.dry);
  if (kept) {
    std::vector<int> id(sc.size());
    for (size_t i = 0; i < id.size(); ++i) id[i] = (int)i;
    gather(c, kept, (int)sc.size(), buf, P, jc, id, x.B, fr, es);
  }
  if (!sx.empty()) gather(c, x.p, T, buf, P, jx, sx, x.B, fr, es);
  if (!c.dry) st.frames = P;
}

Act conv_causal(Ctx& c, CState& st, const Tens& x, const void* w, int ldw, const float* bias, const Geom& g, int cout, ConvOpts o) {
  Model* m = c.m;
  const int P = g.pt;
  if (m->tiled && P > 0) {
    if (m->first_chunk) o.tmode = VT_TPAD_REPLICATE;
    else {
      M_CHECK(c.dry || st.frames >= P, "vt_model: causal cache missing (the first chunk must come first)");
      o.tmode = VT_TPAD_CACHE;
      o.cache = c.dry ? (const void*)16 : st.buf->p;
      o.ncache = c.dry ? P : st.frames;
    }
  }
  const Act r = conv(c, x, w, ldw, bias, g, cout, o);
  if (m->tiled) update_cache(c, st, x, P);
  return r;
}

char* gemm_nt(Ctx& c, const void* a, bool a_batched, const void* b, int Z, int M, int N, int K, int in_dt, int out_dt, int ldo, const float* bias) {
  const size_t bytes = (size_t)Z * M * ldo * esize(out_dt);
  char* y = c.cur->alloc(bytes, c.dry);
  if (ldo != N && !c.dry) M_HIP(hipMemsetAsync(y, 0, bytes, c.stream));
  vt_conv_desc d;
  memset(&d, 0, sizeof(d));
  d.x = a; d.w = b; d.y = y; d.bias = bias;
  d.B = 1; d.Ti = 1; d.Hi = 1; d.Wi = M; d.Cin = K;
// ... 252 lines not shown
      char* buf = m->persistent(su, (size_t)xp.B * keep.size() * fr * es, c.dry);
      gather(c, xp.p, T, buf, (int)keep.size(), 0, keep, xp.B, fr, es);
      if (!c.dry) su.frames = (int)keep.size();
      return up;
    }
    Tens xc = c.alloc(xp.B, Tc, xp.H, xp.W, xp.ld, xp.dt, xp.ld);
    std::vector<int> all;
    for (int t = 0; t < nc; ++t) all.push_back(t);
    gather(c, head, nc, xc.p, Tc, 0, all, xp.B, fr, es);
    all.clear();
    for (int t = 0; t < T; ++t) all.push_back(t);
    gather(c, xp.p, T, xc.p, Tc, nc, all, xp.B, fr, es);
    std::vector<int> keep;
    for (int t = std::max(0, Tc - 2 * n); t < Tc - n; ++t) keep.push_back(t);
    char* buf = m->persistent(su, (size_t)xp.B * keep.size() * fr * es, c.dry);
    gather(c, xc.p, Tc, buf, (int)keep.size(), 0, keep, xp.B, fr, es);
    if (!c.dry) su.frames = (int)keep.size();
    Tens full = c.alloc(xp.B, 2 * Tc, xp.H, xp.W, xp.ld, xp.dt, xp.ld);
    if (!c.dry) M_CALL(vt_time_lerp2x(xc.p, full.p, xp.dt, xp.B, Tc, fr, c.stream));
    Tens up = c.alloc(xp.B, 2 * Tc - 2 * n, xp.H, xp.W, xp.ld, xp.dt, xp.ld);
    all.clear();
    for (int t = 2 * n; t < 2 * Tc; ++t) all.push_back(t);
    gather(c, full.p, 2 * Tc, up.p, 2 * Tc - 2 * n, 0, all, xp.B, fr, es);
    return up;
  }
  Act conv_of(Ctx& c, const Tens& up, NormRef next) {
    ConvOpts o = emit(next, VT_TPAD_REPLICATE);
    o.res = &up;
    o.res_mode = VT_RES_MIX;
    o.mix = c.m->f32(key + ".mix_factor", c.dry);
    return conv_causal(c, sc, up, c.m->conv_w(key + ".conv.conv.weight", up.ld, c.dry), 27 * up.ld, c.m->f32(key + ".conv.conv.bias", c.dry), causal3d(3, 3, 3), ch, o);
  }
  Act run_v11(Ctx& c, const Act& x, NormRef next) {
    const Tens& xp = x.y;
    const int T = xp.T;
    const int64_t fr = (int64_t)xp.H * xp.W * xp.ld;
    if (c.m->tiled && !c.m->first_chunk && c.m->cfg.interpolation_mode == 1) return conv_of(c, interp_cached(c, xp), next);
    Tens up = c.alloc(xp.B, 2 * T, xp.H, xp.W, xp.ld, xp.dt, xp.ld);
    if (c.m->cfg.interpolation_mode == 0) {
      for (int j0 = 0; j0 < 2 * T; j0 += 128) {
        int32_t idx[128];
        const int n = std::min(128, 2 * T - j0);
        for (int j = 0; j < n; ++j) idx[j] = (j0 + j) / 2;
        if (!c.dry) M_CALL(vt_gather_frames(xp.p, up.p + (size_t)j0 * fr * esize(xp.dt), (int)esize(xp.dt), xp.B, fr, (int64_t)T * fr, (int64_t)2 * T * fr, idx, n, c.stream));
      }
    } else {
      const int hn = std::min(n_up, T);
      auto lerp_part = [&](int t0, int n, int out_t0) {
        Tens part = c.alloc(xp.B, n, xp.H, xp.W, xp.ld, xp.dt, xp.ld);
        for (int j0 = 0; j0 < n; j0 += 128) {
          int32_t idx[128];
          const int m = std::min(128, n - j0);
          for (int j = 0; j < m; ++j) idx[j] = t0 + j0 + j;
          if (!c.dry) M_CALL(vt_gather_frames(xp.p, part.p + (size_t)j0 * fr * esize(xp.dt), (int)esize(xp.dt), xp.B, fr, (int64_t)T * fr, (int64_t)n * fr, idx, m, c.stream));
        }
        for (int b = 0; b < xp.B; ++b)
          if (!c.dry)
            M_CALL(vt_time_lerp2x(part.p + (size_t)b * n * fr * esize(xp.dt), up.p + ((size_t)b * 2 * T + out_t0) * fr * esize(xp.dt), xp.dt, 1, n, fr, c.stream));
      };
      if (c.m->tiled) {
        std::vector<int> keep;
        for (int t = std::max(0, T - n_up); t < T; ++t) keep.push_back(t);
        char* buf = c.m->persistent(su, (size_t)xp.B * keep.size() * fr * esize(xp.dt), c.dry);
        gather(c, xp.p, T, buf, (int)keep.size(), 0, keep, xp.B, fr, (int)esize(xp.dt));
        if (!c.dry) su.frames = (int)keep.size();
      }
      lerp_part(0, hn, 0);
      if (T > n_up) lerp_part(n_up, T - n_up, 2 * hn);
    }
    return conv_of(c, up, next);
  }
  Act run(Ctx& c, const Act& x, NormRef next) override {
    if (c.m->v11()) return run_v11(c, x, next);
    const Tens& xp = x.y;
    Act r;
    r.y = c.alloc(xp.B, 2 * xp.T, xp.H, xp.W, pad8(ch), c.m->dt, ch);
    bool emit_ln = next.norm != nullptr;
    Tens nbuf;
    Geom g;
    g.kt = 2; g.kh = 3; g.kw = 3; g.pt = 1; g.ph = 1; g.pw = 1; g.ph_hi = 1; g.pw_hi = 1;
    const float* mf = c.m->f32(key + ".mix_factor", c.dry);
    const bool nc = c.m->noncausal();
    const std::string ck = key + ".conv" + c.m->cv();
    if (emit_ln) {
      ConvOpts o;
      Tens probe = r.y;
      probe.p = nullptr;
      o.out = &r.y; o.yt_mul = 2; o.yt_off = 0; o.ln = next; o.ln_out = &probe; o.ln_optional = true; o.plan_only = true;
      o.res = &xp; o.res_mode = VT_RES_MIX; o.mix = mf;
      Geom gp = g;
      if (nc) gp = centred(g, 1);
      emit_ln = conv(c, xp, c.m->conv_w(ck + ".weight", xp.ld, c.dry, xf_time_parity, nc ? 0 : 1, 0), 18 * xp.ld, c.m->f32(ck + ".bias", c.dry), gp, ch, o).has_n();
      if (emit_ln) nbuf = c.alloc(xp.B, 2 * xp.T, xp.H, xp.W, pad8(ch), c.m->dt, ch);
    }
    for (int par = 0; par < 2; ++par) {
      ConvOpts o;
      o.out = &r.y; o.yt_mul = 2; o.yt_off = par;
      if (emit_ln) { o.ln = next; o.ln_out = &nbuf; o.ln_optional = true; }
      o.res = &xp; o.res_mode = VT_RES_MIX; o.mix = mf;
      const int early = nc ? par : (par == 0 ? 1 : 0);
      Geom gp = g;
      if (nc) gp = centred(g, par == 0 ? 1 : 0);
      const Act a = conv(c, xp, c.m->conv_w(ck + ".weight", xp.ld, c.dry, xf_time_parity, early, 0), 18 * xp.ld, c.m->f32(ck + ".bias", c.dry), gp, ch, o);
      if (emit_ln && !a.has_n()) emit_ln = false;
    }
    if (emit_ln) { r.n = nbuf; r.norm = next.norm; r.silu = next.silu; }
    return r;
  }
};

bool in_list(const int32_t* v, int n, int x) {
  for (int i = 0; i < n; ++i)
    if (v[i] == x) return true;
  return false;
}

typedef std::map<std::string, std::vector<int64_t>> Shapes;
void sh_conv(Shapes& sh, const std::string& key, int cout, int cin, std::vector<int64_t> k) {
  std::vector<int64_t> w = {cout, cin};
  w.insert(w.end(), k.begin(), k.end());
  sh[key + ".weight"] = w;
  sh[key + ".bias"] = {cout};
}
bool g_group_norm = false;
void sh_norm(Shapes& sh, const std::string& key, int c) {
  sh[key + (g_group_norm ? ".weight" : ".norm.weight")] = {c};
  sh[key + (g_group_norm ? ".bias" : ".norm.bias")] = {c};
}
void set_norm(Norm& n, const std::string& key, int site) {
  n.key = key;
  n.group = g_group_norm;
  n.site = site;
}

struct Graph {
  std::vector<std::unique_ptr<Stage>> stages;
  std::string conv_in, conv_out;
  Norm norm_out;
  int c_first = 0, c_last = 0;
  CState st_in, st_out;
  void states(std::vector<CState*>& v) {
    v.push_back(&st_in);
    for (auto& st : stages) st->states(v);
    v.push_back(&st_out);
  }
  void set_offsets(bool overlap) {
    int off = overlap ? 1 : 0;
    st_in.offset = off;
    for (auto& st : stages) {
      if (st->time_up()) off *= 2;
      std::vector<CState*> v;
      st->states(v);
      for (CState* s : v) s->offset = off;
    }
    st_out.offset = off;
  }
};

ResBlock* res_block(Shapes& sh, const std::string& key, int cin, int cout, bool causal, bool wrap = true, int site = VT_GN_FRAME) {
  const std::string sfx0 = (causal && wrap) ? ".conv" : "";
  const std::vector<int64_t> k3 = causal ? std::vector<int64_t>{3, 3, 3} : std::vector<int64_t>{3, 3};
  const std::vector<int64_t> k1 = causal ? std::vector<int64_t>{1, 1, 1} : std::vector<int64_t>{1, 1};
  sh_norm(sh, key + ".norm1", cin);
  sh_norm(sh, key + ".norm2", cout);
  sh_conv(sh, key + ".conv1" + sfx0, cout, cin, k3);
  sh_conv(sh, key + ".conv2" + sfx0, cout, cout, k3);
// ... 934 lines not shown
```

### vidtok_amd/csrc/options.cpp

```cpp
#include "options.h"

#include <stdlib.h>
#include <string.h>

#include <atomic>
#include <mutex>

#include "../../include/vidtok_amd.h"

void vt_set_error(const char* fmt, ...);

namespace {
struct OptDef {
  const char* name;
  int dflt;
};
const OptDef kDefs[OPT_COUNT] = {
    {"conv_buf", 1},        {"conv_tinner", 1},     {"conv_ldsepi", 1},      {"conv_ws", 2},
    {"conv_narrow", 1},     {"conv_tile", 0},       {"conv_tile_min", 128},  {"conv_fuse_ln", 1}, {"conv_fuse_ln256", 1},
    {"tblock_fused", 1},    {"tblock_prof_mode", 0},
    {"conv_deep", 1},       {"ws_prof_mode", 0},    {"attn_flash", 1},      {"conv_splitk", 1},
    {"conv_tskip", 1},      {"conv_in8", 1},        {"conv_tup_ln", 1},     {"conv_nt_mb", 64},
};
std::atomic<int> g_val[OPT_COUNT];
std::once_flag g_once;

int env_default(int id) {
  char var[64] = "VT_";
  size_t n = 3;
  for (const char* s = kDefs[id].name; *s && n + 1 < sizeof(var); ++s) var[n++] = (*s >= 'a' && *s <= 'z') ? (char)(*s - 32) : *s;
  var[n] = 0;
  const char* e = getenv(var);
  return e ? atoi(e) : kDefs[id].dflt;
}
void init_all() {
  for (int i = 0; i < OPT_COUNT; ++i) g_val[i].store(env_default(i), std::memory_order_relaxed);
}
int find(const char* name) {
  if (!name) return -1;
  for (int i = 0; i < OPT_COUNT; ++i)
    if (strcmp(name, kDefs[i].name) == 0) return i;
  return -1;
}
}

int vt_opt(int id) {
  std::call_once(g_once, init_all);
  return g_val[id].load(std::memory_order_relaxed);
}

extern "C" int vt_set_option(const char* name, int32_t value) {
  const int id = find(name);
  if (id < 0) {
    vt_set_error("vt_set_option: unknown option '%s'", name ? name : "(null)");
    return VT_ERR_ARG;
  }
  std::call_once(g_once, init_all);
  g_val[id].store(value, std::memory_order_relaxed);
  return VT_OK;
}

extern "C" int vt_get_option(const char* name, int32_t* value) {
  const int id = find(name);
  if (id < 0 || !value) {
    vt_set_error("vt_get_option: unknown option '%s' or null output", name ? name : "(null)");
    return VT_ERR_ARG;
  }
  *value = vt_opt(id);
  return VT_OK;
}

extern "C" int vt_reset_options(void) {
  std::call_once(g_once, init_all);
  init_all();
  return VT_OK;
}

extern "C" int vt_option_count(void) { return OPT_COUNT; }
extern "C" const char* vt_option_name(int32_t i) { return (i >= 0 && i < OPT_COUNT) ? kDefs[i].name : nullptr; }
```

### vidtok_amd/csrc/options.h

```cpp
#pragma once

enum VtOpt {
  OPT_CONV_BUF = 0,
  OPT_CONV_TINNER,
  OPT_CONV_LDSEPI,
  OPT_CONV_WS,
  OPT_CONV_NARROW,
  OPT_CONV_TILE,
  OPT_CONV_TILE_MIN,
  OPT_CONV_FUSE_LN,
  OPT_CONV_FUSE_LN256,
  OPT_TBLOCK_FUSED,
  OPT_TBLOCK_PROF_MODE,
  OPT_CONV_DEEP,
  OPT_WS_PROF_MODE,
  OPT_ATTN_FLASH,
  OPT_CONV_SPLITK,
  OPT_CONV_TSKIP,
  OPT_CONV_IN8,
  OPT_CONV_TUP_LN,
  OPT_CONV_NT_MB,
  OPT_COUNT
};

int vt_opt(int id);
```

### vidtok_amd/lib.py

```python
import ctypes as C
import os

import torch

_HERE = os.path.dirname(os.path.abspath(__file__))
LIB_PATH = os.path.join(_HERE, "libvidtok_amd.so")

VT_F32, VT_BF16, VT_I32, VT_BF16X3, VT_F16 = 0, 1, 2, 3, 4
VT_TPAD_ZERO, VT_TPAD_REPLICATE, VT_TPAD_CACHE, VT_TPAD_ZERO_BACK = 0, 1, 2, 3
VT_GN_FRAME, VT_GN_PIXEL, VT_GN_CLIP = 0, 1, 2
VT_RES_NONE, VT_RES_ADD, VT_RES_MIX = 0, 1, 2
VT_NDHWC, VT_NCTHW = 0, 1
VT_ACT_RELU = 1
VT_LPIPS_CLAMP_Y, VT_LPIPS_ROUNDTRIP, VT_LPIPS_UNIT = 1, 2, 4
VT_SESSION_ENCODE, VT_SESSION_DECODE = 0, 1


class VtError(RuntimeError):
    pass


class ConvDesc(C.Structure):

    _fields_ = (
# ... 39 lines not shown
        [(n, C.c_void_p) for n in ("x", "dy", "dw", "db", "work")]
        + [("work_bytes", C.c_int64)]
        + [(n, C.c_int32) for n in (
            "B", "Ti", "Hi", "Wi", "ldx", "Cin",
            "To", "Ho", "Wo", "lddy", "Cout",
            "KT", "KH", "KW", "st", "sh", "sw",
            "pt", "ph", "pw", "pt_hi", "ph_hi", "pw_hi",
            "tmode", "ups_t", "ups_s", "dtype",
        )]
    )


class DgradDesc(C.Structure):

    _fields_ = (
        [(n, C.c_void_p) for n in ("dy", "wt", "dx", "acc", "work")]
        + [("work_bytes", C.c_int64)]
        + [(n, C.c_int32) for n in (
            "B", "Ti", "Hi", "Wi", "lddx", "Cin",
            "To", "Ho", "Wo", "lddy", "Cout",
            "KT", "KH", "KW", "st", "sh", "sw",
            "pt", "ph", "pw", "pt_hi", "ph_hi", "pw_hi",
            "tmode", "ups_t", "ups_s", "dtype", "dx_dtype",
            "ldw", "ldacc",
        )]
    )


class ModelConfig(C.Structure):

    _fields_ = (
        [(n, C.c_int32) for n in ("version", "ch", "num_res_blocks", "in_channels", "out_ch", "z_channels", "double_z", "num_resolutions")]
        + [("ch_mult", C.c_int32 * 8)]
        + [("n_spatial_ds", C.c_int32), ("spatial_ds", C.c_int32 * 8), ("n_tempo_ds", C.c_int32), ("tempo_ds", C.c_int32 * 8)]
        + [("n_spatial_us", C.c_int32), ("spatial_us", C.c_int32 * 8), ("n_tempo_us", C.c_int32), ("tempo_us", C.c_int32 * 8)]
        + [("time_downsample_factor", C.c_int32), ("regularizer", C.c_int32), ("n_levels", C.c_int32), ("levels", C.c_int32 * 8),
           ("interpolation_mode", C.c_int32), ("norm_type", C.c_int32), ("fsq_num_codebooks", C.c_int32), ("fsq_dim", C.c_int32)]
    )


_P, _I32, _I64, _F = C.c_void_p, C.c_int32, C.c_int64, C.c_float
SIGNATURES = {
    "vt_last_error": (C.c_char_p, []),
    "vt_version": (C.c_int, []),
    "vt_graph_launch": (C.c_int, [_P, _P]),
    "vt_conv_max_lds_bytes": (C.c_int, []),
    "vt_set_option": (C.c_int, [C.c_char_p, _I32]),
    "vt_get_option": (C.c_int, [C.c_char_p, C.POINTER(_I32)]),
    "vt_reset_options": (C.c_int, []),
    "vt_option_count": (C.c_int, []),
    "vt_option_name": (C.c_char_p, [_I32]),
    "vt_model_config_size": (C.c_int, []),
    "vt_create": (C.c_int, [C.POINTER(ModelConfig), _I32, C.POINTER(_P)]),
    "vt_destroy": (C.c_int, [_P]),
    "vt_load_weight": (C.c_int, [_P, C.c_char_p, _P, C.POINTER(_I64), _I32]),
    "vt_weight_count": (C.c_int, [_P]),
    "vt_weight_name": (C.c_char_p, [_P, _I32]),
    "vt_weight_shape": (C.c_int, [_P, _I32, C.POINTER(_I64), C.POINTER(_I32)]),
    "vt_workspace_bytes": (_I64, [_P, _I32, _I32, _I32, _I32]),
    "vt_latent_dims": (C.c_int, [_P, _I32, _I32, _I32, C.POINTER(_I32)]),
    "vt_encode": (C.c_int, [_P, _P, _I32, _I32, _I32, _I32, _P, _P, _I64, _P]),
    "vt_regularize_kl": (C.c_int, [_P, _P, _P, _P, _P, _I32, _I32, _I32, _I32, _P]),
    "vt_regularize_fsq": (C.c_int, [_P, _P, _P, _P, _I32, _I32, _I32, _I32, _P]),
    "vt_indices_to_latent": (C.c_int, [_P, _P, _P, _I32, _I32, _I32, _I32, _P]),
    "vt_decode": (C.c_int, [_P, _P, _I32, _I32, _I32, _I32, _P, _P, _I64, _P]),
    "vt_reset_cache": (C.c_int, [_P]),
    "vt_prepare": (C.c_int, [_P]),
    "vt_regularize_fsq_aux": (C.c_int, [_P, _P, _I32, _I32, _I32, _I32, _F, _P, _P, _P]),
    "vt_tile_latent_frames": (_I32, [_P, _I32, _I32]),
    "vt_tile_workspace_bytes": (_I64, [_P, _I32, _I32, _I32, _I32, _I32, _I32]),
    "vt_tile_encode": (C.c_int, [_P, _P, _I32, _I32, _I32, _I32, _I32, _P, _P, _I64, _P]),
    "vt_tile_decode": (C.c_int, [_P, _P, _I32, _I32, _I32, _I32, _I32, _I32, _P, _P, _I64, _P]),
    "vt_session_create": (C.c_int, [_P, _I32, _I32, _I32, _I32, _I32, _I32, C.POINTER(_P)]),
    "vt_session_workspace_bytes": (_I64, [_P]),
    "vt_session_push": (C.c_int, [_P, _P, _I32, _P, _I32, C.POINTER(_I32), _P, _I64, _P]),
    "vt_session_finish": (C.c_int, [_P, _P, _I32, C.POINTER(_I32), _P, _I64, _P]),
    "vt_session_destroy": (C.c_int, [_P]),
    "vt_copy_segments": (C.c_int, [_P, _I32, _I64, _P]),
    "vt_conv": (C.c_int, [C.POINTER(ConvDesc), _P]),
    "vt_conv_desc_size": (C.c_int, []),
    "vt_conv_work_bytes": (_I64, [C.POINTER(ConvDesc)]),
    "vt_conv_plan": (C.c_int, [C.POINTER(ConvDesc), C.POINTER(_I32)]),
    "vt_conv_profile": (C.c_int, [C.POINTER(ConvDesc), _P, _P]),
    "vt_frames_work_floats": (_I64, [_I32, _I32, _I32]),
    "vt_frames_u8_to_ncthw": (C.c_int, [_P, _I32, _I32, _I32, _I32, _I32, _I32, _I32, _P, _I32, _I32, _I32, _I32, _P, _P]),
    "vt_ncthw_to_frames_u8": (C.c_int, [_P, _I32, _I32, _I32, _I32, _I32, _P, _I32, _I32, _P]),
    "vt_ncthw_copy_frames": (C.c_int, [_P, _P, _I32, _I32, _I32, _I32, _I32, _I32, _I64, _I32, _P]),
    "vt_tblock_desc_size": (C.c_int, []),
    "vt_temporal_block_supported": (C.c_int, [C.POINTER(TBlockDesc)]),
    "vt_temporal_block": (C.c_int, [C.POINTER(TBlockDesc), _P]),
    "vt_temporal_block_profile": (C.c_int, [C.POINTER(TBlockDesc), _P, _P]),
    "vt_flash_attention_supported": (C.c_int, [_I32, _I32, _I32, _I32]),
    "vt_flash_attention": (C.c_int, [_P, _P, _P, _P, _P, _I32, _I32, _I32, _I32, _I32, _F, _P]),
    "vt_layernorm_act": (C.c_int, [_P, C.c_int, _I64, _P, C.c_int, _I64, _P, _P, _I64, _I32, _F, _I32, _P]),
    "vt_tanh_inplace": (C.c_int, [_P, _I64, _P]),
    "vt_softmax_rows": (C.c_int, [_P, _P, C.c_int, _I64, _I32, _I64, _F, _P]),
    "vt_ncthw_to_ndhwc": (C.c_int, [_P, _P, C.c_int, _I32, _I32, _I32, _I32, _I32, _I32, _I32, _P]),
    "vt_ndhwc_to_ncthw": (C.c_int, [_P, C.c_int, _P, _I32, _I32, _I32, _I32, _I32, _I32, _I32, _P]),
    "vt_time_avgpool3s2": (C.c_int, [_P, _P, _P, C.c_int, _I32, _I32, _I64, _I32, _I32, _P]),
    "vt_time_lerp2x": (C.c_int, [_P, _P, C.c_int, _I32, _I32, _I64, _P]),
    "vt_time_lerp2x_cat": (C.c_int, [_P, _I32, _P, _P, C.c_int, _I32, _I32, _I32, _I64, _P]),
    "vt_pack_conv_weight": (C.c_int, [_P, _P, _I32, _I32, _I32, _I32, _I32, _I32, C.POINTER(_I32), _I64, _P]),
    "vt_fsq_consts": (C.c_int, [C.POINTER(_I32), _I32, C.POINTER(_F)]),
    "vt_kl_sample": (C.c_int, [_P, _P, _P, _P, _I32, _I32, _I64, _P]),
    "vt_fsq_quantize": (C.c_int, [_P, _P, _P, C.POINTER(_I32), _I32, _I32, _I64, _P]),
    "vt_fsq_indices_to_codes": (C.c_int, [_P, _P, C.POINTER(_I32), _I32, _I32, _I64, _P]),
    "vt_fsq_quantize_cb": (C.c_int, [_P, _P, _P, C.POINTER(_I32), _I32, _I32, _I32, _I64, _P]),
    "vt_fsq_indices_to_codes_cb": (C.c_int, [_P, _P, C.POINTER(_I32), _I32, _I32, _I32, _I64, _P]),
    "vt_fsq_aux_work_floats": (_I64, [C.POINTER(_I32), _I32, _I32, _I64]),
    "vt_fsq_aux_stats": (C.c_int, [_P, C.POINTER(_I32), _I32, _I32, _I64, _F, _P, _P, _P]),
    "vt_fsq_aux_stats_avg": (C.c_int, [_P, C.POINTER(_I32), _I32, _I32, _I64, _F, _P, _P, _P, _P]),
    "vt_entropy": (C.c_int, [_P, _I64, _P, _P]),
    "vt_fsq_aux_loss": (C.c_int, [_P, _P, _F, _F, _F, _P, _P]),
    "vt_groupnorm_work_bytes": (_I64, [_I32, _I32, _I32, _I32]),
    "vt_groupnorm_act": (C.c_int, [_P, C.c_int, _I64, _P, C.c_int, _I64, _P, _P, _I32, _I32, _I64, _I32, _I32, _I32,
                                   C.c_float, _I32, _P, _P]),
    "vt_channel_linear": (C.c_int, [_P, _P, _P, _P, _I32, _I32, _I32, _I64, _P]),
    "vt_eval_work_floats": (_I64, [_I32, _I32]),
    "vt_eval_psnr_ssim": (C.c_int, [_P, _P, _P, _P, _P, _I32, _I32, _I32, _I32, _I32, _I32, _P]),
    "vt_gather_frames": (C.c_int, [_P, _P, _I32, _I32, _I64, _I64, _I64, C.POINTER(_I32), _I32, _P]),
    "vt_conv_act": (C.c_int, [C.POINTER(ConvDesc), _I32, _P]),
    "vt_lpips_work_bytes": (_I64, [_I32, _I32, _I32]),
    "vt_lpips_prep": (C.c_int, [_P, _P, _P, _P, _P, _I32, _I32, _I32, _I32, _I32, _I32, _P]),
    "vt_lpips_tap": (C.c_int, [_P, _P, _P, _P, _I64, _I32, _I32, _I32, _I32, _I32, _I32, _P]),
    "vt_lpips_finish": (C.c_int, [_P, _I64, _P, _P, _I32, _I32, _I32, _P]),
    "vt_lpips_tap_backward": (C.c_int, [_P, _P, _P, _P, _I32, _P, _I32, _I32, _I32, _I32, _I32, _P]),
    "vt_relu_backward": (C.c_int, [_P, _I32, _P, _P, _I32, _I64, _P]),
    "vt_lpips_prep_backward": (C.c_int, [_P, _I32, _P, _P, _I32, _I32, _I32, _P]),
    "vt_wgrad_desc_size": (C.c_int, []),
    "vt_conv_wgrad_work_bytes": (_I64, [C.POINTER(WgradDesc)]),
    "vt_conv_wgrad": (C.c_int, [C.POINTER(WgradDesc), _P]),
    "vt_layernorm_act_backward_work_bytes": (_I64, [_I64, _I32]),
    "vt_layernorm_act_backward": (C.c_int, [_P, _P, _I32, _I64, _P, _I32, _I64, _P, _P, _P, _P, _I64, _I32, _F, _I32, _P, _I64, _P]),
    "vt_dgrad_desc_size": (C.c_int, []),
    "vt_pack_conv_weight_dgrad": (C.c_int, [_P, _P, _I32, _I32, _I32, _I32, _I32, _I32, _I32, _I64, _P]),
    "vt_conv_dgrad_work_bytes": (_I64, [C.POINTER(DgradDesc)]),
    "vt_conv_dgrad": (C.c_int, [C.POINTER(DgradDesc), _P]),
    "vt_grad_fold": (C.c_int, [_P, _I32, _P, _P, _I32, _I32, _I32, _I32, _I32, _I32, _I32, _I32, _I32, _I32, _I32, _I32, _P]),
    "vt_softmax_rows_backward": (C.c_int, [_P, _I64, _P, _P, _I64, _I32, _I64, _I32, _F, _P]),
    "vt_transpose_batched": (C.c_int, [_P, _P, _I32, _I32, _I32, _I32, _I64, _I64, _P]),
    "vt_upsample_mix": (C.c_int, [_P, _P, _P, _P, _I32, _I64, _I32, _I32, _P]),
    "vt_upsample_mix_backward_work_bytes": (_I64, [_I64, _I32]),
    "vt_upsample_mix_backward": (C.c_int, [_P, _P, _P, _P, _P, _P, _P, _I32, _I64, _I32, _I32, _P, _I64, _P]),
    "vt_time_lerp2x_backward": (C.c_int, [_P, _P, _I32, _I32, _I32, _I64, _P]),
    "vt_grad_ncthw_to_ndhwc": (C.c_int, [_P, _P, _I32, _I32, _I32, _I32, _I32, _I32, _I32, _I32, _P]),
    "vt_grad_add": (C.c_int, [_P, _P, _P, _I32, _I64, _P]),
}

_lib = None


def load(path: str = None):
    global _lib
    if _lib is not None and path is None:
        return _lib
    path = path or os.environ.get("VIDTOK_AMD_LIB", LIB_PATH)
    if not os.path.exists(path):
        raise VtError(
            f"{path} not found: build the HIP extension first (python -m vidtok_amd.build). "
            "vidtok_amd has no CPU fallback."
        )
    lib = C.CDLL(path)
    for name, (res, args) in SIGNATURES.items():
        fn = getattr(lib, name)
        fn.restype = res
        fn.argtypes = args
# ... 41 lines not shown
```

### vidtok_amd/modules.py

```python
import dataclasses
import functools
import os

import torch
import torch.nn as nn

from . import lib as L
from . import ops
from .ops import ConvGeom
from .packing import (ConvSite, space_upsample_parity_mix, space_upsample_parity_weights, time_upsample_parity_mix,
                      time_upsample_parity_weights)


def _check_norm(norm_type):
    if norm_type not in ("layernorm", "groupnorm"):
        raise NotImplementedError(f"norm_type={norm_type!r}: the reference knows 'layernorm' and 'groupnorm'")


SITE_FRAME, SITE_PIXEL, SITE_CLIP, SITE_POS = L.VT_GN_FRAME, L.VT_GN_PIXEL, L.VT_GN_CLIP, ops.GN_POS


class Normed:

    __slots__ = ("y", "n", "norm", "silu")

    def __init__(self, y, n, norm, silu):
        self.y, self.n, self.norm, self.silu = y, n, norm, silu


def plain(x):
    return x.y if isinstance(x, Normed) else x


_EMIT_NEXT_NORM = os.environ.get("VIDTOK_AMD_EMIT_NEXT_NORM", "1") != "0"
_FUSE_TBLOCK = os.environ.get("VIDTOK_AMD_FUSE_TBLOCK", "1") != "0"


def _emit(next_norm):
    if next_norm is None or not _EMIT_NEXT_NORM or not next_norm[0].fusable:
        return {}
    return dict(ln=next_norm[0].fused(next_norm[1]), ln_keep_y=True)


def _wrap(out, next_norm):
    if next_norm is None or not _EMIT_NEXT_NORM or not next_norm[0].fusable:
        return out
    return Normed(out[0], out[1], next_norm[0], next_norm[1])


class LayerNorm(nn.Module):

    def __init__(self, num_channels, eps=1e-6):
        super().__init__()
        self.norm = nn.LayerNorm(num_channels, eps=eps, elementwise_affine=True)
        self._cache = None

    def affine(self):
        w, b = self.norm.weight, self.norm.bias
        key = (w._version, b._version, w.device, w.data_ptr())
        if self._cache is None or self._cache[0] != key:
            self._cache = (key, w.detach().float().contiguous(), b.detach().float().contiguous())
        return self._cache[1], self._cache[2]

    fusable = True

    def apply_ndhwc(self, x, silu, dt, site=None):
        if isinstance(x, Normed):
            if x.norm is self and x.silu == silu:
                return x.n
            x = x.y
        g, b = self.affine()
        return ops.layernorm_act(x, g, b, silu=silu, eps=self.norm.eps, out_dtype=dt)

    def fused(self, silu):
        g, b = self.affine()
        return (g, b, self.norm.eps, silu)

    def after(self, conv, silu, dt, site=None):
        return conv(ln=self.fused(silu), ln_keep_y=False)


class GroupNorm32(nn.GroupNorm):

    fusable = False

    def __init__(self, num_channels):
        super().__init__(num_groups=32, num_channels=num_channels, eps=1e-6, affine=True)

    def apply_ndhwc(self, x, silu, dt, site=SITE_FRAME):
        x = plain(x)
        return ops.groupnorm_act(x, self.weight.detach().float().contiguous(), self.bias.detach().float().contiguous(),
                                 scope=site, silu=silu, eps=self.eps, out_dtype=dt, c=self.num_channels)

    def after(self, conv, silu, dt, site=SITE_FRAME):
# ... 116 lines not shown
        self.with_conv = with_conv
        self.in_channels = in_channels
        self._ident = {}
        if not with_conv:
            return
        self.conv = nn.Conv2d(in_channels, in_channels, kernel_size=3, stride=1, padding=1)
        self.parity_sites = [(py, px, ConvSite(self.conv, ConvGeom(kh=2, kw=2, ph=1 - py, pw=1 - px, ph_hi=py, pw_hi=px),
                                               transform=functools.partial(space_upsample_parity_weights, py=py, px=px),
                                               mix=functools.partial(space_upsample_parity_mix, py=py, px=px)))
                             for py in (0, 1) for px in (0, 1)]
        self.fold_site = ConvSite(self.conv, dataclasses.replace(_G3x3, ups_s=1))

    def run(self, x, dt, next_norm=None):
        x = plain(x)
        B, T, H, W, C = x.shape
        if not self.with_conv:
            key = (dt, x.device, C)
            if key not in self._ident:
                self._ident[key] = torch.eye(C, dtype=torch.float32, device=x.device).to(dt).contiguous()
            return ops.conv(x, self._ident[key], None, ConvGeom(ups_s=1), cout=self.in_channels, ldy=C)
        cout = self.conv.out_channels
        ld = ops.pad_channels(cout)
        y = (torch.empty if ld == cout else torch.zeros)((B, T, 2 * H, 2 * W, ld), dtype=dt, device=x.device)
        for py, px, site in self.parity_sites:
            site.run(x, dt, out=y, out_s=(py, px))
        return y


class Downsample(nn.Module):

    def __init__(self, in_channels, with_conv):
        super().__init__()
        self.with_conv = with_conv
        self.in_channels = in_channels
        self._pool_w = {}
        if not with_conv:
            return
        self.conv = nn.Conv2d(in_channels, in_channels, kernel_size=3, stride=2, padding=0)
        self.site = ConvSite(self.conv, ConvGeom(kh=3, kw=3, sh=2, sw=2, ph=0, pw=0, ph_hi=1, pw_hi=1))

    def run(self, x, dt, next_norm=None):
        if not self.with_conv:
            xp = plain(x)
            C = xp.shape[-1]
            key = (dt, xp.device, C)
            if key not in self._pool_w:
                w = (0.25 * torch.eye(C, dtype=torch.float32, device=xp.device)).repeat(1, 4)
                self._pool_w[key] = w.to(dt).contiguous()
            y = ops.conv(xp, self._pool_w[key], None, ConvGeom(kh=2, kw=2, sh=2, sw=2), cout=self.in_channels, ldy=C,
                         **_emit(next_norm))
            return _wrap(y, next_norm)
        return _wrap(self.site.run(plain(x), dt, **_emit(next_norm)), next_norm)


class TimeDownsampleResCausal2x(nn.Module):

    def __init__(self, in_channels, out_channels, mix_factor: float = 2.0, version="v1_0"):
        super().__init__()
        self.conv = CausalConv3d(in_channels, out_channels, 3, stride=(2, 1, 1), version=version)
        self.mix_factor = nn.Parameter(torch.Tensor([mix_factor]))
        self.version = version
        self.is_first_chunk = True
        self.causal_cache = None

    def run(self, x, dt, next_norm=None):
        x = plain(x)
        if self.version == "v1_0":
            x1 = ops.time_avgpool3s2(x, L.VT_TPAD_ZERO)
        else:
            if self.is_first_chunk:
                x1 = ops.time_avgpool3s2(x, L.VT_TPAD_REPLICATE)
            else:
                x1 = ops.time_avgpool3s2(x, L.VT_TPAD_CACHE, cache=self.causal_cache)
            self.causal_cache = ops.gather_frames(x, [x.shape[1] - 1], out=_persistent_cache(self, (x.shape[0], 1) + tuple(x.shape[2:]), x))
        return _wrap(self.conv.run(x, dt, res=x1, res_mode=L.VT_RES_MIX, mix_factor=self.mix_factor.detach(),
                                   **_emit(next_norm)), next_norm)


def time_parity_class(conv, geom, early):
    return ConvSite(conv, geom, transform=functools.partial(time_upsample_parity_weights, early=early),
                    mix=functools.partial(time_upsample_parity_mix, early=early))


def time_parity_upsample(sites, x, dt, mix_factor, next_norm):
    B, T, H, W, _C = x.shape
    cout = sites[0].cout
    ld = ops.pad_channels(cout)
    y = (torch.empty if ld == cout else torch.zeros)((B, 2 * T, H, W, ld), dtype=dt, device=x.device)
    emit = dict(_emit(next_norm))
    n = None

    def alloc_n():
        return (torch.empty if ld == cout else torch.zeros)(y.shape, dtype=dt, device=x.device)

    for par, site in enumerate(sites):
        r = site.run(x, dt, res=x, res_mode=L.VT_RES_MIX, mix_factor=mix_factor, out=y, out_t=(2, par),
                     **(dict(emit, ln_out=(alloc_n if n is None else n), ln_optional=True) if emit else {}))
        if emit and not isinstance(r, tuple):
            emit, n = {}, None
        elif emit:
            n = r[1]
    return y if n is None else Normed(y, n, next_norm[0], next_norm[1])


class TimeUpsampleResCausal2x(nn.Module):

    def __init__(self, in_channels, out_channels, mix_factor: float = 2.0, interpolation_mode="nearest",
                 num_temp_upsample=1, version="v1_0"):
        super().__init__()
        self.conv = CausalConv3d(in_channels, out_channels, 3, version=version)
        self.mix_factor = nn.Parameter(torch.Tensor([mix_factor]))
        self.interpolation_mode = interpolation_mode
        self.num_temp_upsample = num_temp_upsample
        self.enable_cached = interpolation_mode == "trilinear"
        self.version = version
        self.is_first_chunk = True
        self.causal_cache = None
        g = ConvGeom(kt=2, kh=3, kw=3, pt=1, ph=1, pw=1, ph_hi=1, pw_hi=1)
        self.parity_sites = (time_parity_class(self.conv.conv, g, early=True), time_parity_class(self.conv.conv, g, early=False))

    def _interp_v11(self, x):
        n, T = self.num_temp_upsample, x.shape[1]
        if not self.enable_cached:
            return ops.gather_frames(x, [t // 2 for t in range(2 * T)])
        if not self.is_first_chunk:
            nc = self.causal_cache.shape[1]
            Tc = nc + T
            if Tc - 2 * n >= nc:
                up = ops.time_lerp2x_cat(self.causal_cache, x, 2 * n)
                keep = list(range(Tc - 2 * n - nc, Tc - n - nc))
                self.causal_cache = ops.gather_frames(x, keep, out=_persistent_cache(self, (x.shape[0], len(keep)) + tuple(x.shape[2:]), x))
                return up
            xc = torch.empty((x.shape[0], Tc) + tuple(x.shape[2:]), dtype=x.dtype, device=x.device)
            ops.gather_frames(self.causal_cache, list(range(nc)), out=xc, out_t0=0)
            ops.gather_frames(x, list(range(T)), out=xc, out_t0=nc)
            keep = list(range(max(0, Tc - 2 * n), Tc - n))
            self.causal_cache = ops.gather_frames(xc, keep, out=_persistent_cache(self, (x.shape[0], len(keep)) + tuple(x.shape[2:]), x))
            up = ops.time_lerp2x(xc)
            return ops.gather_frames(up, list(range(2 * n, 2 * Tc)))
        keep = list(range(max(0, T - n), T))
        self.causal_cache = ops.gather_frames(x, keep, out=_persistent_cache(self, (x.shape[0], len(keep)) + tuple(x.shape[2:]), x))
        hn = min(n, T)
        up = torch.empty((x.shape[0], 2 * T) + tuple(x.shape[2:]), dtype=x.dtype, device=x.device)
        ops.time_lerp2x(ops.gather_frames(x, list(range(0, hn))), out=up, out_t0=0)
        if T > n:
            ops.time_lerp2x(ops.gather_frames(x, list(range(n, T))), out=up, out_t0=2 * hn)
        return up

    def run(self, x, dt, next_norm=None):
        x = plain(x)
        mf = self.mix_factor.detach()
        if self.version == "v1_0":
            return time_parity_upsample(self.parity_sites, x, dt, mf, next_norm)
        xi = self._interp_v11(x)
        return _wrap(self.conv.run(xi, dt, res=xi, res_mode=L.VT_RES_MIX, mix_factor=mf, **_emit(next_norm)), next_norm)


def residual_block(blk, view, convs, x, dt, next_norm):
    conv1, conv2, nin = convs
    h = blk.norm1.apply_ndhwc(x, True, dt, view)
    x = plain(x)
    h = blk.norm2.after(lambda **kw: conv1.run(h, dt, **kw), True, dt, view)
    if nin is not None:
        x = nin.run(x, dt)
    return _wrap(conv2.run(h, dt, res=x, res_mode=L.VT_RES_ADD, **_emit(next_norm)), next_norm)


class ResnetBlock(nn.Module):

    def __init__(self, *, in_channels, out_channels=None, conv_shortcut=False, dropout=0.0, temb_channels=0,
                 use_checkpoint=False, norm_type="layernorm"):
        super().__init__()
        assert temb_channels == 0 and not conv_shortcut
        out_channels = in_channels if out_channels is None else out_channels
        self.in_channels, self.out_channels = in_channels, out_channels
        self.norm1 = Normalize(in_channels, norm_type)
        self.conv1 = nn.Conv2d(in_channels, out_channels, kernel_size=3, stride=1, padding=1)
        self.norm2 = Normalize(out_channels, norm_type)
        self.conv2 = nn.Conv2d(out_channels, out_channels, kernel_size=3, stride=1, padding=1)
        if in_channels != out_channels:
            self.nin_shortcut = nn.Conv2d(in_channels, out_channels, kernel_size=1, stride=1, padding=0)
        self.sites = (ConvSite(self.conv1, _G3x3), ConvSite(self.conv2, _G3x3),
                      ConvSite(self.nin_shortcut, _G1x1) if in_channels != out_channels else None)

    def first_norm(self, dt=None):
        return (self.norm1, True)

    def run(self, x, dt, next_norm=None):
        return residual_block(self, SITE_FRAME, self.sites, x, dt, next_norm)


def _causal_convs(blk):
    return blk.conv1, blk.conv2, (blk.nin_shortcut if blk.in_channels != blk.out_channels else None)


class ResnetCausalBlock(nn.Module):

    def __init__(self, *, in_channels, out_channels=None, conv_shortcut=False, dropout=0.0, temb_channels=0,
                 use_checkpoint=False, norm_type="layernorm", version="v1_0"):
        super().__init__()
        assert temb_channels == 0 and not conv_shortcut
        out_channels = in_channels if out_channels is None else out_channels
        self.in_channels, self.out_channels = in_channels, out_channels
        self.norm1 = Normalize(in_channels, norm_type)
        self.conv1 = CausalConv3d(in_channels, out_channels, 3, version=version)
        self.norm2 = Normalize(out_channels, norm_type)
        self.conv2 = CausalConv3d(out_channels, out_channels, 3, version=version)
        if in_channels != out_channels:
            self.nin_shortcut = CausalConv3d(in_channels, out_channels, 1, version=version)
        self.sites = tuple(c and c.site for c in _causal_convs(self))

    def first_norm(self, dt=None):
        return (self.norm1, True)

    def run(self, x, dt, next_norm=None):
        return residual_block(self, SITE_FRAME, _causal_convs(self), x, dt, next_norm)


class ResnetCausalBlock1D(nn.Module):

    def __init__(self, *, in_channels, out_channels=None, conv_shortcut=False, dropout=0.0, temb_channels=0,
                 zero_init=False, use_checkpoint=False, norm_type="layernorm", version="v1_0"):
        super().__init__()
        assert temb_channels == 0 and not conv_shortcut
        out_channels = in_channels if out_channels is None else out_channels
        self.in_channels, self.out_channels = in_channels, out_channels
        self.norm1 = Normalize(in_channels, norm_type)
        self.conv1 = CausalConv1d(in_channels, out_channels, 3, version=version)
        self.norm2 = Normalize(out_channels, norm_type)
        self.conv2 = CausalConv1d(out_channels, out_channels, 3, version=version)
        if in_channels != out_channels:
            self.nin_shortcut = CausalConv1d(in_channels, out_channels, 1, version=version)
        self.sites = tuple(c and c.site for c in _causal_convs(self))
        if zero_init:
            self.conv2.conv.weight.data.zero_()
            self.conv2.conv.bias.data.zero_()
# ... 327 lines not shown
```

### vidtok_amd/ops.py

```python
import ctypes as C
from dataclasses import dataclass
from typing import Optional

import torch

from . import lib as L

_DT = {torch.float32: L.VT_F32, torch.bfloat16: L.VT_BF16, torch.float16: L.VT_F16}
H16 = (torch.bfloat16, torch.float16)
CH_ALIGN = 8


CONV_RECORD = None


def _conv_launch(lib, d, what, keep=()):
    L.check(lib.vt_conv(C.byref(d), _stream()), what)
    if CONV_RECORD is not None:
        CONV_RECORD.append((d, keep, (d.B * d.To * d.Ho * d.Wo * max(1, d.nbatch), d.Cout, d.KT * d.KH * d.KW * d.Cin)))


def conv_plan(d):
    out = (C.c_int32 * 8)()
    L.check(L.load().vt_conv_plan(C.byref(d), out), "vt_conv_plan")
    return dict(tile=(out[0], out[1]), waves=out[2], workgroups=out[3], ln_fused=bool(out[4]), launches=out[5],
                kernel={2: "narrow", 3: "ws2", 4: "in8"}.get(out[6], "igemm"), lds_epilogue=out[7] == 1, deep_ring=out[7] == 2)


def replay_convs(record, conv_kernel_only=True):
    lib = L.load()
    for d, _keep, _label in record:
        if isinstance(d, L.TBlockDesc):
            L.check(lib.vt_temporal_block(C.byref(d), _stream()), "vt_temporal_block(replay)")
            continue
        if isinstance(d, tuple):
            _, q, k, vT, bias, o, scale = d
            L.check(lib.vt_flash_attention(_ptr(q), _ptr(k), _ptr(vT), _ptr(bias), _ptr(o), _DT[q.dtype], q.shape[0], q.shape[1], q.shape[2],
                                           vT.shape[2], scale, _stream()), "vt_flash_attention(replay)")
            continue
        if conv_kernel_only and d.ln_mode != 0 and not conv_plan(d)["ln_fused"]:
            d2 = L.ConvDesc()
            C.memmove(C.byref(d2), C.byref(d), C.sizeof(d))
            d2.ln_mode = 0
            d = d2
        L.check(lib.vt_conv(C.byref(d), _stream()), "vt_conv(replay)")


def pad_channels(c: int) -> int:
    return (c + CH_ALIGN - 1) // CH_ALIGN * CH_ALIGN


def _stream():
    return C.c_void_p(torch.cuda.current_stream().cuda_stream)


def _ptr(t: Optional[torch.Tensor]):
    return None if t is None else C.c_void_p(t.data_ptr())


def _chk(t: torch.Tensor, name: str):
    if not t.is_cuda:
        raise L.VtError(f"{name}: tensor is on {t.device}; vidtok_amd runs on the GPU only (no CPU fallback)")
    if not t.is_contiguous():
        raise L.VtError(f"{name}: tensor must be contiguous")


@dataclass(frozen=True)
class ConvGeom:

    kt: int = 1
    kh: int = 1
    kw: int = 1
    st: int = 1
    sh: int = 1
    sw: int = 1
    pt: int = 0
    ph: int = 0
    pw: int = 0
    ph_hi: int = 0
    pw_hi: int = 0
    pt_hi: int = 0
    ups_t: int = 0
    ups_s: int = 0

    def out_dims(self, Ti, Hi, Wi):
        Tv, Hv, Wv = Ti << self.ups_t, Hi << self.ups_s, Wi << self.ups_s
        To = (Tv + self.pt + self.pt_hi - self.kt) // self.st + 1
        Ho = (Hv + self.ph + self.ph_hi - self.kh) // self.sh + 1
        Wo = (Wv + self.pw + self.pw_hi - self.kw) // self.sw + 1
        return To, Ho, Wo


def conv(x, w, bias, geom: ConvGeom, *, cout: int, out_dtype=None, tmode=L.VT_TPAD_ZERO, cache=None,
         res=None, res_mode=L.VT_RES_NONE, res_tshift=0, mix_factor=None, out_layout=L.VT_NDHWC,
         t_trim=0, ldy=None, ln=None, ln_keep_y=True, out=None, ln_out=None, out_t=None, out_s=None, ln_optional=False):
    lib = L.load()
    _chk(x, "conv.x"); _chk(w, "conv.w")
    B, Ti, Hi, Wi, Cin = x.shape
    x3 = w.dtype == torch.int32
    assert (w.dtype == x.dtype or (x3 and x.dtype == torch.float32)) and x.dtype in _DT, (w.dtype, x.dtype)
    out_dtype = out_dtype or x.dtype
    To, Ho, Wo = geom.out_dims(Ti, Hi, Wi)
    assert To > 0 and Ho > 0 and Wo > 0, (To, Ho, Wo)
    mul, off = out_t or (1, 0)
    if out is not None:
        assert out_layout == L.VT_NDHWC and out.is_contiguous() and out.dtype == out_dtype
        smul = 2 if out_s is not None else 1
        assert tuple(out.shape[:4]) == (B, To * mul, Ho * smul, Wo * smul), (out.shape, (B, To * mul, Ho, Wo))
        y, ldy = out, out.shape[4]
    elif out_layout == L.VT_NCTHW:
        y = torch.empty((B, cout, To - t_trim, Ho, Wo), dtype=torch.float32, device=x.device)
        out_dtype = torch.float32
        ldy = cout
    else:
        assert mul == 1
        ldy = ldy or pad_channels(cout)
        if ldy != cout:
            y = torch.zeros((B, To, Ho, Wo, ldy), dtype=out_dtype, device=x.device)
        else:
            y = torch.empty((B, To, Ho, Wo, ldy), dtype=out_dtype, device=x.device)
    d = L.ConvDesc()
    d.x, d.w, d.bias, d.y = x.data_ptr(), w.data_ptr(), (bias.data_ptr() if bias is not None else None), y.data_ptr()
    if bias is not None:
        assert bias.dtype == torch.float32 and bias.numel() >= cout
    d.B, d.Ti, d.Hi, d.Wi, d.Cin = B, Ti, Hi, Wi, Cin
    d.To, d.Ho, d.Wo, d.Cout = To, Ho, Wo, cout
    d.ldw, d.ldy = w.shape[1], ldy
    assert not x3 or out_dtype == torch.float32
    d.KT, d.KH, d.KW = geom.kt, geom.kh, geom.kw
    d.st, d.sh, d.sw = geom.st, geom.sh, geom.sw
    d.pt, d.ph, d.pw = geom.pt, geom.ph, geom.pw
    d.tmode = tmode
    if cache is not None:
        _chk(cache, "conv.cache")
        assert cache.dtype == x.dtype and cache.shape[0] == B and tuple(cache.shape[2:]) == (Hi, Wi, Cin), cache.shape
        d.cache, d.ncache = cache.data_ptr(), cache.shape[1]
    d.ups_t, d.ups_s = geom.ups_t, geom.ups_s
    d.res_mode = res_mode
    if res_mode != L.VT_RES_NONE:
        _chk(res, "conv.res")
        assert res.dtype == out_dtype, (res.dtype, out_dtype)
        assert res.shape[0] == B and tuple(res.shape[2:4]) == (Ho, Wo) and res.shape[4] >= cout, (res.shape, y.shape)
        d.res, d.res_tshift, d.Tr, d.ldr = res.data_ptr(), res_tshift, res.shape[1], res.shape[4]
        if res_mode == L.VT_RES_MIX:
            assert mix_factor is not None and mix_factor.dtype == torch.float32 and mix_factor.is_cuda
            d.mix_factor = mix_factor.data_ptr()
    d.out_layout, d.t_trim = out_layout, t_trim
    d.dtype, d.out_dtype = (L.VT_BF16X3 if x3 else _DT[x.dtype]), _DT[out_dtype]
    d.nbatch = 1
    d.yt_mul, d.yt_off = mul, off
    if out_s is not None:
        assert out is not None and mul == 1
        d.ys_mul, d.ys_oh, d.ys_ow = 2, int(out_s[0]), int(out_s[1])
    n = None
    if ln is not None:
        gamma, beta, eps, silu = ln
        assert out_layout == L.VT_NDHWC and gamma.dtype == torch.float32 and beta.dtype == torch.float32
        assert gamma.numel() >= cout and beta.numel() >= cout and gamma.is_cuda and beta.is_cuda
        d.ln_gamma, d.ln_beta, d.ln_out = gamma.data_ptr(), beta.data_ptr(), y.data_ptr()
        d.ln_mode, d.ln_keep_y, d.ldn, d.ln_eps = (2 if silu else 1), int(bool(ln_keep_y)), ldy, float(eps)
        fused = True
        if ln_optional:
            try:
                fused = conv_plan(d)["ln_fused"]
            except L.VtError:
                fused = False
        if fused:
            if callable(ln_out):
                ln_out = ln_out()
            if ln_out is not None:
                assert ln_out.shape == y.shape and ln_out.dtype == out_dtype and ln_out.is_contiguous()
                n = ln_out
            else:
                n = (torch.zeros if ldy != cout else torch.empty)(y.shape, dtype=out_dtype, device=x.device)
            d.ln_out = n.data_ptr()
        else:
            assert ln_keep_y
            d.ln_gamma = d.ln_beta = d.ln_out = None
            d.ln_mode = 0
            ln, n = None, None
    work = None
    if x.dtype in H16 and (geom.kt == 3 or geom.kh == 3):
        nb = lib.vt_conv_work_bytes(C.byref(d))
        if nb > 0:
            work = torch.empty((nb,), dtype=torch.uint8, device=x.device)
            d.work, d.work_bytes = work.data_ptr(), nb
    _conv_launch(lib, d, "vt_conv", (x, w, bias, y, res, cache, mix_factor, n, ln, work))
    if ln is None:
        return y
    return (y, n) if ln_keep_y else n


def _tblock_desc(x, tmode, c=None, caches=None, cache_offset=0):
    d = L.TBlockDesc()
    B, T, H, W, ld = x.shape
    d.dtype, d.C, d.ld, d.B, d.T, d.HW, d.tmode = _DT.get(x.dtype, -1), (ld if c is None else c), ld, B, T, H * W, tmode
    if caches is not None:
        for t in caches:
            _chk(t, "tblock.cache")
            assert tuple(t.shape) == (B, 2, H, W, ld) and t.dtype == x.dtype, (tuple(t.shape), tuple(x.shape))
        d.cache1, d.cache2, d.cache_offset = caches[0].data_ptr(), caches[1].data_ptr(), int(cache_offset)
    return d


def temporal_block_supported(x, tmode, c=None, caches=None, cache_offset=0) -> bool:
    if not x.is_cuda or x.dtype not in _DT:
        return False
    return bool(L.load().vt_temporal_block_supported(C.byref(_tblock_desc(x, tmode, c, caches, cache_offset))))


def temporal_block(x, w1, b1, w2, b2, norm1, norm2, *, tmode=L.VT_TPAD_ZERO, eps=1e-6, next_ln=None, keep_y=True, profile_out=None, c=None,
                   caches=None, cache_offset=0):
    lib = L.load()
    _chk(x, "tblock.x"); _chk(w1, "tblock.w1"); _chk(w2, "tblock.w2")
    d = _tblock_desc(x, tmode, c, caches, cache_offset)
    y = torch.empty_like(x) if keep_y else None
    n = torch.empty_like(x) if next_ln is not None else None
    d.x, d.y, d.n_out = x.data_ptr(), (y.data_ptr() if keep_y else None), (n.data_ptr() if n is not None else None)
    d.w1, d.w2 = w1.data_ptr(), w2.data_ptr()
    d.b1 = b1.data_ptr() if b1 is not None else None
    d.b2 = b2.data_ptr() if b2 is not None else None
    for t in (norm1[0], norm1[1], norm2[0], norm2[1]):
        assert t.dtype == torch.float32 and t.is_cuda and t.numel() >= x.shape[-1]
    d.norm1_gamma, d.norm1_beta, d.norm2_gamma, d.norm2_beta = (t.data_ptr() for t in (norm1[0], norm1[1], norm2[0], norm2[1]))
    if next_ln is not None:
        assert next_ln[0].dtype == torch.float32 and next_ln[1].dtype == torch.float32
        d.next_gamma, d.next_beta, d.ln_next_mode = next_ln[0].data_ptr(), next_ln[1].data_ptr(), (2 if next_ln[2] else 1)
    d.keep_y, d.eps = int(bool(keep_y)), float(eps)
    if profile_out is not None:
        L.check(lib.vt_temporal_block_profile(C.byref(d), profile_out.data_ptr(), _stream()), "vt_temporal_block_profile")
        return (y, n)
    L.check(lib.vt_temporal_block(C.byref(d), _stream()), "vt_temporal_block")
    if CONV_RECORD is not None:
        CONV_RECORD.append((d, (x, w1, b1, w2, b2, norm1, norm2, next_ln, y, n, caches), (d.B * d.T * d.HW, d.C, 6 * d.C)))
    if next_ln is None:
        return y
    return (y, n) if keep_y else n


def gemm_nt(a, b, *, out_dtype=None, bias=None, ld_out=None):
    lib = L.load()
    _chk(a, "gemm.a"); _chk(b, "gemm.b")
    Za, M, K = a.shape
    Z, N, Kb = b.shape
    assert Za in (1, Z) and K == Kb and a.dtype == b.dtype
    out_dtype = out_dtype or a.dtype
    ldo = ld_out or N
    assert ldo >= N
    y = (torch.empty if ldo == N else torch.zeros)((Z, M, ldo), dtype=out_dtype, device=a.device)
    d = L.ConvDesc()
    d.x, d.w, d.y = a.data_ptr(), b.data_ptr(), y.data_ptr()
    d.bias = bias.data_ptr() if bias is not None else None
    d.B, d.Ti, d.Hi, d.Wi, d.Cin = 1, 1, 1, M, K
    d.To, d.Ho, d.Wo, d.Cout = 1, 1, M, N
    d.ldw, d.ldy = K, ldo
    d.KT = d.KH = d.KW = 1
    d.st = d.sh = d.sw = 1
    d.dtype, d.out_dtype = _DT[a.dtype], _DT[out_dtype]
    d.nbatch = Z
    d.xs_z, d.ws_z, d.ys_z = (M * K if Za == Z else 0), N * K, M * ldo
    _conv_launch(lib, d, "vt_conv(gemm)", (a, b, bias, y))
    return y


def flash_attention_supported(q, vT) -> bool:
    if not q.is_cuda or q.dtype not in _DT:
        return False
    return bool(L.load().vt_flash_attention_supported(_DT[q.dtype], q.shape[1], q.shape[2], vT.shape[2]))


def flash_attention(q, k, vT, bias_v, scale: float):
    lib = L.load()
    _chk(q, "attn.q"); _chk(k, "attn.k"); _chk(vT, "attn.vT")
    Z, S, Cc = q.shape
    assert k.shape == q.shape and k.dtype == q.dtype == vT.dtype and vT.shape[:2] == (Z, Cc)
    o = torch.empty_like(q)
    if bias_v is not None:
        assert bias_v.dtype == torch.float32 and bias_v.numel() >= Cc and bias_v.is_cuda
    L.check(lib.vt_flash_attention(_ptr(q), _ptr(k), _ptr(vT), _ptr(bias_v), _ptr(o), _DT[q.dtype], Z, S, Cc, vT.shape[2], float(scale), _stream()),
            "vt_flash_attention")
    if CONV_RECORD is not None:
        CONV_RECORD.append((("flash", q, k, vT, bias_v, o, float(scale)), (), (Z * S, S, 2 * Cc)))
    return o


LN_RECORD = None


def layernorm_act(x, gamma, beta, *, silu: bool, eps: float = 1e-6, out_dtype=None, c: int = None):
    lib = L.load()
    _chk(x, "layernorm.x")
    ld = x.shape[-1]
    c = c or ld
    M = x.numel() // ld
    out_dtype = out_dtype or x.dtype
    y = torch.empty(x.shape, dtype=out_dtype, device=x.device) if c == ld else torch.zeros(
        x.shape, dtype=out_dtype, device=x.device)
    assert gamma.dtype == torch.float32 and beta.dtype == torch.float32 and gamma.numel() == c
    L.check(lib.vt_layernorm_act(_ptr(x), _DT[x.dtype], ld, _ptr(y), _DT[out_dtype], ld, _ptr(gamma), _ptr(beta),
                                 M, c, float(eps), int(bool(silu)), _stream()), "vt_layernorm_act")
    if LN_RECORD is not None:
        LN_RECORD.append((x, y, gamma, beta, M, c, float(eps), bool(silu)))
    return y


def replay_layernorms(record):
    lib = L.load()
    for x, y, gamma, beta, M, c, eps, silu in record:
        ld = x.shape[-1]
        L.check(lib.vt_layernorm_act(_ptr(x), _DT[x.dtype], ld, _ptr(y), _DT[y.dtype], ld, _ptr(gamma), _ptr(beta), M, c, eps,
                                     int(silu), _stream()), "vt_layernorm_act(replay)")


def launch_bytes(d):
    if isinstance(d, tuple):
        _, q, k, vT, _b, o, _s = d
        return (q.numel() + k.numel() + vT.numel() + o.numel()) * q.element_size()
    if isinstance(d, L.TBlockDesc):
        es = 2
        px = d.B * d.T * d.HW
        return px * d.ld * es * (1 + (1 if d.keep_y else 0) + (1 if d.ln_next_mode else 0)) + 2 * d.C * 3 * d.C * es
    es = 2 if d.dtype in (L.VT_BF16, L.VT_F16) else 4
    eo = 4 if d.out_dtype == L.VT_F32 else 2
    nb = max(1, d.nbatch)
    M = d.B * d.To * d.Ho * d.Wo * nb
    plan = conv_plan(d)
    nbytes = d.B * d.Ti * d.Hi * d.Wi * d.Cin * es * (nb if d.xs_z or nb == 1 else 1) + d.Cout * d.ldw * es * nb
    if not (d.ln_mode != 0 and plan["ln_fused"] and not d.ln_keep_y):
        nbytes += M * d.Cout * eo
    if d.res_mode != L.VT_RES_NONE:
        nbytes += M * d.Cout * eo
    if d.ln_mode != 0 and plan["ln_fused"]:
        nbytes += M * d.Cout * eo
    return nbytes


def launch_class(d):
    if isinstance(d, tuple):
        return None
    if isinstance(d, L.TBlockDesc):
        return "temporal block fused (C=128)", launch_bytes(d)
    taps = d.KT * d.KH * d.KW
    if conv_plan(d)["kernel"] == "narrow":
        name = "conv_out 3x3x3 128->3 (conv3d_narrow_kernel)"
    elif taps == 1 and d.nbatch <= 1:
        name = "1x1 convolutions (nin_shortcut, attention projections)"
    elif d.Cin <= 8:
        name = "conv_in 3x3x3 (3 -> C)"
    elif d.KH == 1 and d.KW == 1 and d.KT == 3 and d.Cin <= 256:
        name = f"temporal k3 convolutions, unfused (C={d.Cin})"
    else:
        return None
    return name, launch_bytes(d)


GN_POS = 3


def groupnorm_act(x, gamma, beta, *, scope, silu, eps=1e-6, out_dtype=None, c=None, groups=32):
    lib = L.load()
    _chk(x, "groupnorm.x")
    if scope == GN_POS:
        shp = x.shape
        return groupnorm_act(x.reshape(1, 1, -1, 1, shp[-1]), gamma, beta, scope=L.VT_GN_PIXEL, silu=silu, eps=eps,
                             out_dtype=out_dtype, c=c, groups=groups).reshape(shp)
    B, T, H, W, ld = x.shape
    c = c or ld
    out_dtype = out_dtype or x.dtype
    y = (torch.zeros if c != ld else torch.empty)(x.shape, dtype=out_dtype, device=x.device)
    nbytes = lib.vt_groupnorm_work_bytes(B, T, groups, scope)
    work = torch.empty((max(nbytes, 8) // 8,), dtype=torch.float64, device=x.device)
    L.check(lib.vt_groupnorm_act(_ptr(x), _DT[x.dtype], ld, _ptr(y), _DT[out_dtype], ld, _ptr(gamma), _ptr(beta), B, T, H * W,
                                 c, groups, scope, float(eps), int(bool(silu)), _ptr(work), _stream()), "vt_groupnorm_act")
    return y


def tanh_(x):
    _chk(x, "tanh.x")
    assert x.dtype == torch.float32
    L.check(L.load().vt_tanh_inplace(_ptr(x), x.numel(), _stream()), "vt_tanh_inplace")
    return x


def softmax_rows(s, scale: float, out_dtype, ld_out=None):
    lib = L.load()
    _chk(s, "softmax.s")
    assert s.dtype == torch.float32
    cols = s.shape[-1]
    rows = s.numel() // cols
    ldo = ld_out or cols
    p = (torch.empty if ldo == cols else torch.zeros)(tuple(s.shape[:-1]) + (ldo,), dtype=out_dtype, device=s.device)
    L.check(lib.vt_softmax_rows(_ptr(s), _ptr(p), _DT[out_dtype], rows, cols, ldo, float(scale), _stream()),
            "vt_softmax_rows")
    return p


def ncthw_to_ndhwc(x, dtype, tpad: int = 0, ld: int = None):
    lib = L.load()
    _chk(x, "ncthw_to_ndhwc.x")
    assert x.dtype == torch.float32 and x.dim() == 5
    B, Cc, T, H, W = x.shape
    ld = ld or pad_channels(Cc)
    y = torch.empty((B, T + tpad, H, W, ld), dtype=dtype, device=x.device)
    L.check(lib.vt_ncthw_to_ndhwc(_ptr(x), _ptr(y), _DT[dtype], B, Cc, T, H, W, ld, tpad, _stream()),
# ... 591 lines not shown
```

### vidtok_amd/packing.py

```python
import torch

from . import lib as L
from . import ops
from .ops import pad_channels


def pack_conv_weight(weight: torch.Tensor, dtype: torch.dtype, cin_stored: int = None) -> torch.Tensor:
    cout, cin = weight.shape[:2]
    cin_p = cin_stored or pad_channels(cin)
    nd = weight.dim() - 2
    w = weight.detach().to(torch.float32)
    perm = (0,) + tuple(range(2, 2 + nd)) + (1,)
    w = w.permute(*perm)
    if cin_p != cin:
        w = torch.nn.functional.pad(w, (0, cin_p - cin))
    return w.reshape(cout, -1).to(dtype).contiguous()


ARITH_SPLIT3 = "bf16x3"
SPLIT3_DTYPE = torch.int32


def pack_split3(w2d: torch.Tensor) -> torch.Tensor:
    cout, K = w2d.shape
    Kp = (K + 31) // 32 * 32
    w = w2d.detach().to(torch.float32)
    if Kp != K:
        w = torch.nn.functional.pad(w, (0, Kp - K))
    hi = w.to(torch.bfloat16)
    lo = (w - hi.to(torch.float32)).to(torch.bfloat16)
    planes = torch.stack([hi.view(cout, Kp // 16, 16), lo.view(cout, Kp // 16, 16)], dim=2).contiguous()
    return planes.view(SPLIT3_DTYPE).reshape(cout, Kp)


def packed_caches(root: torch.nn.Module):
    def visit(v):
        if isinstance(v, ConvSite):
            yield v.pack
        elif isinstance(v, (tuple, list)):
            for e in v:
                yield from visit(e)

    for m in root.modules():
        for v in vars(m).values():
            yield from visit(v)


def set_arith(root: torch.nn.Module, arith):
    assert arith in (None, ARITH_SPLIT3)
    for cache in packed_caches(root):
        if not cache.pin_native:
            cache.arith = arith


def time_upsample_parity_weights(weight: torch.Tensor, early: bool):
    w = weight.detach().to(torch.float32)
    assert w.dim() == 5 and w.shape[2] == 3
    if early:
        return torch.stack([w[:, :, 0] + w[:, :, 1], w[:, :, 2]], dim=2)
    return torch.stack([w[:, :, 0], w[:, :, 1] + w[:, :, 2]], dim=2)


def space_upsample_parity_weights(weight: torch.Tensor, py: int, px: int):
    w = weight.detach().to(torch.float32)
    assert w.dim() == 4 and tuple(w.shape[2:]) == (3, 3)
    rows = torch.stack([w[:, :, 0], w[:, :, 1] + w[:, :, 2]], dim=2) if py == 0 else \
        torch.stack([w[:, :, 0] + w[:, :, 1], w[:, :, 2]], dim=2)
    return torch.stack([rows[..., 0], rows[..., 1] + rows[..., 2]], dim=3) if px == 0 else \
        torch.stack([rows[..., 0] + rows[..., 1], rows[..., 2]], dim=3)


def time_upsample_parity_mix(kdims, early: bool):
    kt, kh, kw = kdims
    assert kt == 3
    s = kh * kw
    first = [[0 * s + i, 1 * s + i] if early else [0 * s + i] for i in range(s)]
    second = [[2 * s + i] if early else [1 * s + i, 2 * s + i] for i in range(s)]
    return first + second


def space_upsample_parity_mix(kdims, py: int, px: int):
    assert tuple(kdims) == (3, 3)
    rows = [[0], [1, 2]] if py == 0 else [[0, 1], [2]]
    cols = [[0], [1, 2]] if px == 0 else [[0, 1], [2]]
    out = []
    for R in rows:
        for Cc in cols:
            m = [-1, -1, -1, -1]
            for ci, c in enumerate(Cc):
                for ri, r in enumerate(R):
                    m[2 * ci + ri] = r * 3 + c
            out.append(m)
    return out


class PackedCache:

    def __init__(self, transform=None, pin_native=False, mix=None):
        self._entries = {}
        self._transform = transform
        self._mix = mix
        assert (transform is None) == (mix is None)
        self.arith = None
        self.pin_native = pin_native

    def get(self, weight: torch.nn.Parameter, bias, dtype, cin_stored=None):
        arith = self.arith if dtype == torch.float32 else None
        key = (dtype, weight.device, weight._version, None if bias is None else bias._version, cin_stored,
               weight.data_ptr(), arith)
        slot = (dtype, arith, cin_stored)
        ent = self._entries.get(slot)
        if ent is None or ent[0] != key:
            if weight.is_cuda:
                wd = weight.detach()
                wd = wd if wd.dtype == torch.float32 and wd.is_contiguous() else wd.float().contiguous()
                mix = None if self._mix is None else self._mix(tuple(wd.shape[2:]))
                w = ops.pack_conv_weight(wd, dtype, cin_stored, mix=mix, split3=arith == ARITH_SPLIT3)
            else:
                w = pack_conv_weight(weight if self._transform is None else self._transform(weight), dtype, cin_stored)
                if arith == ARITH_SPLIT3:
                    w = pack_split3(w)
            b = None if bias is None else bias.detach().to(torch.float32).contiguous()
            ent = self._entries[slot] = (key, (w, b))
        return ent[1]


class DgradPackCache:

    def __init__(self):
        self._entries = {}

    def get(self, weight: torch.nn.Parameter, dtype, cout_stored):
        key = (weight.device, weight._version, weight.data_ptr())
        slot = (dtype, cout_stored)
        ent = self._entries.get(slot)
        if ent is None or ent[0] != key:
            wd = weight.detach()
            wd = wd if wd.dtype == torch.float32 and wd.is_contiguous() else wd.float().contiguous()
            ent = self._entries[slot] = (key, ops.pack_conv_weight_dgrad(wd, dtype, cout_stored))
        return ent[1]


class ConvSite:

    def __init__(self, conv, geom, *, clip_tmode=L.VT_TPAD_ZERO, transform=None, mix=None, pin_native=False):
        self.conv, self.geom, self.clip_tmode = conv, geom, clip_tmode
        self.cin, self.cout = conv.in_channels, conv.out_channels
        self.pack = PackedCache(transform, pin_native, mix)
        self._dgrad = None

    def rows(self, dt, cin_stored):
        return self.pack.get(self.conv.weight, self.conv.bias, dt, cin_stored=cin_stored)

    def run(self, x, dt, *, tmode=L.VT_TPAD_ZERO, cache=None, **kw):
        w, b = self.pack.get(self.conv.weight, self.conv.bias, dt, cin_stored=x.shape[-1])
        return ops.conv(x, w, b, self.geom, cout=self.cout, tmode=tmode, cache=cache, **kw)

    def run_clip(self, x, dt, **kw):
        return self.run(x, dt, tmode=self.clip_tmode, **kw)

    def dgrad_rows(self, dtype, cout_stored):
        if self._dgrad is None:
            self._dgrad = DgradPackCache()
        return self._dgrad.get(self.conv.weight, dtype, cout_stored)
```

Measured before the change: 918.9 frames/s.

## Fuse time-upsample parity convs into one paired 256x256 igemm with shared center tap

Replaces the two per-parity time-upsample conv launches with one path. A 2D 3x3 conv computes the shared center-tap term v. A single 256x256 igemm then computes the outer-tap term and writes both output frames from a paired epilogue that adds v for the current and previous frame, applies the mix with the residual, and optionally fuses LayerNorm. This removes duplicated GEMM work across the two parities but adds an extra conv pass and extra reads of v. Eligibility is gated by an option and by shape checks, and the build now checks the new kernel instantiations for register spills.

```diff
diff --git a/include/vidtok_amd.h b/include/vidtok_amd.h
--- a/include/vidtok_amd.h
+++ b/include/vidtok_amd.h
@@ -89,6 +89,9 @@
 int vt_conv_plan(const vt_conv_desc* d, int32_t* out8);
 int vt_conv_profile(const vt_conv_desc* d, uint64_t* stamps_out, vt_stream stream);
 int vt_conv_desc_size(void);
+
+int vt_time_upsample3_supported(const vt_conv_desc* u);
+int vt_time_upsample3(const vt_conv_desc* u, const void* v, int32_t ldv, vt_stream stream);
 
 typedef struct vt_tblock_desc {
   const void* x;
diff --git a/vidtok_amd/build.py b/vidtok_amd/build.py
--- a/vidtok_amd/build.py
+++ b/vidtok_amd/build.py
@@ -1,5 +1,6 @@
 import hashlib
 import os
+import re
 import shutil
 import subprocess
 import sys
@@ -13,7 +14,9 @@
 EXTRA_FLAGS = {"conv_ws2.hip": ["-fno-slp-vectorize"], "tblock_ws128.hip": ["-fno-slp-vectorize"]}
 
 
-NO_SPILL = {"tblock_ws128.hip": "tblock_pair_kernel", "conv_ws2.hip": "conv3x3_ws2_kernel"}
+NO_SPILL = {"tblock_ws128.hip": "tblock_pair_kernel", "conv_ws2.hip": "conv3x3_ws2_kernel",
+            "conv_igemm_bf16.hip": re.compile(r"conv_igemm_glds_kernel.*Lb[01]ELi2ELb0ELi\dELi0EEEvNS_8ConvArgsE$"),
+            "conv_igemm_f16.hip": re.compile(r"conv_igemm_glds_kernel.*Lb[01]ELi2ELb0ELi\dELi0EEEvNS_8ConvArgsE$")}
 LLVM_BIN = "/opt/rocm/lib/llvm/bin"
 
 
@@ -42,7 +45,8 @@
         obj = os.path.join(objdir, os.path.splitext(src)[0] + ".o")
         for name, _v, _a, spill, scratch in kernel_resources(obj):
             measured = name.endswith("Lb1EEEvNS_10TBlockArgsE") or name.endswith("Lb1EEEvNS_8ConvArgsE")
-            if kern in name and not measured and (spill or scratch):
+            hit = kern in name if isinstance(kern, str) else kern.search(name) is not None
+            if hit and not measured and (spill or scratch):
                 bad.append(f"{name}: {spill} spilled registers, {scratch} B scratch")
     if bad:
         raise RuntimeError("register spills in hand-scheduled kernels (wrong results, not only slow):\n  " + "\n  ".join(bad))
diff --git a/vidtok_amd/csrc/conv_common.h b/vidtok_amd/csrc/conv_common.h
--- a/vidtok_amd/csrc/conv_common.h
+++ b/vidtok_amd/csrc/conv_common.h
@@ -70,6 +70,8 @@
   int nt_store;
   unsigned long long* prof;
   int prof_mode;
+  const char* pair_v;
+  int ldv;
 };
 
 struct split3_t {
diff --git a/vidtok_amd/csrc/conv_igemm.hip b/vidtok_amd/csrc/conv_igemm.hip
--- a/vidtok_amd/csrc/conv_igemm.hip
+++ b/vidtok_amd/csrc/conv_igemm.hip
@@ -160,6 +160,27 @@
                           d->ln_eps, d->ln_mode == 2 ? 1 : 0, stream_);
 }
 
+extern "C" int vt_time_upsample3_supported(const vt_conv_desc* u) {
+  ConvArgs a;
+  ConvPlan p;
+  if (conv_decide(u, a, p) != VT_OK) return 0;
+  return tup3_eligible(u, a, p) ? 1 : 0;
+}
+
+extern "C" int vt_time_upsample3(const vt_conv_desc* u, const void* v, int32_t ldv, vt_stream stream_) {
+  ConvArgs a;
+  ConvPlan p;
+  const int rc = conv_decide(u, a, p);
+  if (rc != VT_OK) return rc;
+  VT_CHECK_ARG(tup3_eligible(u, a, p), "vt_time_upsample3: descriptor not covered (ask vt_time_upsample3_supported; the parity launches of vt_conv serve it)");
+  VT_CHECK_ARG(v != nullptr && (reinterpret_cast<uintptr_t>(v) & 15) == 0 && ldv >= u->Cout && ldv % 8 == 0,
+               "vt_time_upsample3: v must be 16-byte aligned with ldv = %d >= Cout and a multiple of 8", ldv);
+  a.pair_v = reinterpret_cast<const char*>(v);
+  a.ldv = ldv;
+  const IgemmVariant pair = {TILE_256x256, true, 2, 2, kRowBytes};
+  return launch_igemm(u->dtype, false, a, pair, 1, stream_);
+}
+
 extern "C" int vt_conv_act(const vt_conv_desc* d, int32_t act, vt_stream stream_) {
   VT_CHECK_ARG(act == VT_ACT_RELU, "vt_conv_act: act %d (VT_ACT_RELU = %d is the one activation)", act, VT_ACT_RELU);
   ConvArgs a;
diff --git a/vidtok_amd/csrc/conv_igemm_kernel.h b/vidtok_amd/csrc/conv_igemm_kernel.h
--- a/vidtok_amd/csrc/conv_igemm_kernel.h
+++ b/vidtok_amd/csrc/conv_igemm_kernel.h
@@ -365,6 +365,123 @@
         }
       }
       Oct<TOut>::store(ng + orow * p.ldn + 8 * j, o, p.nt_store != 0);
+    }
+  };
+  half(std::integral_constant<int, 0>{});
+  half(std::integral_constant<int, 1>{});
+}
+
+template <typename TOut>
+__device__ __forceinline__ void conv_epilogue_lds256_pair(const ConvArgs& p, f32x16 (&acc)[4][2], int m_blk, int n_blk, int wm, int wn, int lane,
+                                                          int tid, char* smem) {
+#pragma clang fp contract(off)
+  static_assert(sizeof(TOut) == 2, "paired epilogue: 16-bit storage");
+  typedef float f32x2 __attribute__((ext_vector_type(2)));
+  TOut* __restrict__ yg = reinterpret_cast<TOut*>(p.y);
+  const TOut* __restrict__ rg = reinterpret_cast<const TOut*>(p.res);
+  const TOut* __restrict__ vg = reinterpret_cast<const TOut*>(p.pair_v);
+  TOut* __restrict__ ng = reinterpret_cast<TOut*>(p.ln_out);
+  float* T = reinterpret_cast<float*>(smem);
+  const bool has_ln = p.ln_mode != 0;
+  const float alpha = 1.0f / (1.0f + __expf(-p.mix_factor[0]));
+  constexpr int RS = 16;
+  const int j = tid & 31, rsub = tid >> 5;
+  const long long hw = (long long)p.Ho * p.Wo;
+  const unsigned frame = fast_div((unsigned)m_blk, p.fd_hw);
+  const bool has_prev = frame != fast_div(frame, p.fd_to) * (unsigned)p.To;
+  const long long row0 = (long long)frame * hw;
+  f32x2 lg[4], lb[4];
+  if (has_ln) {
+    const f32x4 g0 = *reinterpret_cast<const f32x4*>(p.ln_gamma + 8 * j), g1 = *reinterpret_cast<const f32x4*>(p.ln_gamma + 8 * j + 4);
+    const f32x4 b0 = *reinterpret_cast<const f32x4*>(p.ln_beta + 8 * j), b1 = *reinterpret_cast<const f32x4*>(p.ln_beta + 8 * j + 4);
+    lg[0] = f32x2{g0[0], g0[1]}; lg[1] = f32x2{g0[2], g0[3]}; lg[2] = f32x2{g1[0], g1[1]}; lg[3] = f32x2{g1[2], g1[3]};
+    lb[0] = f32x2{b0[0], b0[1]}; lb[1] = f32x2{b0[2], b0[3]}; lb[2] = f32x2{b1[0], b1[1]}; lb[3] = f32x2{b1[2], b1[3]};
+    if (p.ln_mode == 2) {
+#pragma unroll
+      for (int q = 0; q < 4; ++q) {
+        lg[q] = lg[q] * kNegLog2e;
+        lb[q] = lb[q] * kNegLog2e;
+      }
+    }
+  }
+  auto emit = [&](const f32x2 (&t)[4], const Oct<TOut>& vq, const Oct<TOut>& xq, long long orow) {
+    f32x2 v[4];
+#pragma unroll
+    for (int q = 0; q < 4; ++q) {
+      v[q] = t[q] + f32x2{vq.get(2 * q), vq.get(2 * q + 1)};
+      v[q] = f32x2{xq.get(2 * q), xq.get(2 * q + 1)} * alpha + v[q] * (1.0f - alpha);
+    }
+    if (p.ln_keep_y || !has_ln) {
+      const float yv[8] = {v[0][0], v[0][1], v[1][0], v[1][1], v[2][0], v[2][1], v[3][0], v[3][1]};
+      Oct<TOut>::store(yg + orow * p.ldy + n_blk + 8 * j, yv, p.nt_store != 0);
+    }
+    if (!has_ln) return;
+    float o[8];
+    const f32x2 s = (v[0] + v[1]) + (v[2] + v[3]);
+    f32x2 qq = v[0] * v[0];
+#pragma unroll
+    for (int q = 1; q < 4; ++q) qq = __builtin_elementwise_fma(v[q], v[q], qq);
+    float nm;
+    const float rstd = ln_row_stats<32>(s[0] + s[1], qq[0] + qq[1], p.ln_eps, &nm);
+    const f32x2 rstd2 = {rstd, rstd}, nm2 = {nm, nm}, c2 = {kNegLog2e, kNegLog2e};
+#pragma unroll
+    for (int q = 0; q < 4; ++q) {
+      f32x2 u = __builtin_elementwise_fma(__builtin_elementwise_fma(v[q], rstd2, nm2), lg[q], lb[q]);
+      if (p.ln_mode == 2) {
+        const f32x2 den = __builtin_elementwise_fma(f32x2{__builtin_amdgcn_exp2f(u[0]), __builtin_amdgcn_exp2f(u[1])}, c2, c2);
+        u = u * f32x2{__builtin_amdgcn_rcpf(den[0]), __builtin_amdgcn_rcpf(den[1])};
+      }
+      o[2 * q] = u[0];
+      o[2 * q + 1] = u[1];
+    }
+    Oct<TOut>::store(ng + orow * p.ldn + 8 * j, o, p.nt_store != 0);
+  };
+  const int h = lane >> 5;
+  auto half = [&](auto pz_c) {
+    constexpr int PZ = decltype(pz_c)::value;
+    Oct<TOut> xq[8];
+#pragma unroll
+    for (int it = 0; it < 8; ++it) {
+      const long long m = (long long)m_blk + ((RS * it) >> 5) * 64 + PZ * 32 + rsub + ((RS * it) & 31);
+      xq[it].load(rg + m * p.ldr + n_blk + 8 * j);
+    }
+    __syncthreads();
+    {
+      const int prl = wm * 32 + (lane & 31);
+#pragma unroll
+      for (int a = 0; a < 4; ++a)
+#pragma unroll
+        for (int g = 0; g < 4; ++g) {
+          const int c = wn * 128 + 32 * a + 8 * g + 4 * h;
+          f32x4 bq;
+          if (p.bias) bq = *reinterpret_cast<const f32x4*>(p.bias + n_blk + c);
+          else bq[0] = bq[1] = bq[2] = bq[3] = 0.0f;
+          f32x4 v;
+#pragma unroll
+          for (int e = 0; e < 4; ++e) v[e] = acc[a][PZ][4 * g + e] + bq[e];
+          *reinterpret_cast<f32x4*>(T + prl * 256 + (((c >> 2) ^ (prl & 63)) << 2)) = v;
+        }
+    }
+    __syncthreads();
+    Oct<TOut> vp[4], vc[4];
+#pragma unroll
+    for (int it = 0; it < 8; ++it) {
+      if ((it & 3) == 0) {
+#pragma unroll
+        for (int k = 0; k < 4; ++k) {
+          const long long m = (long long)m_blk + ((RS * (it + k)) >> 5) * 64 + PZ * 32 + rsub + ((RS * (it + k)) & 31);
+          vc[k].load(vg + m * p.ldv + n_blk + 8 * j);
+          if (has_prev) vp[k].load(vg + (m - hw) * p.ldv + n_blk + 8 * j);
+          else vp[k].w = u32x4{0u, 0u, 0u, 0u};
+        }
+      }
+      const int r = rsub + RS * it;
+      const long long m = (long long)m_blk + ((RS * it) >> 5) * 64 + PZ * 32 + rsub + ((RS * it) & 31);
+      const f32x4 t0 = *reinterpret_cast<const f32x4*>(T + r * 256 + (((2 * j) ^ (r & 63)) << 2));
+      const f32x4 t1 = *reinterpret_cast<const f32x4*>(T + r * 256 + (((2 * j + 1) ^ (r & 63)) << 2));
+      const f32x2 t[4] = {f32x2{t0[0], t0[1]}, f32x2{t0[2], t0[3]}, f32x2{t1[0], t1[1]}, f32x2{t1[2], t1[3]}};
+      emit(t, vp[it & 3], xq[it], m + row0);
+      emit(t, vc[it & 3], xq[it], m + row0 + hw);
     }
   };
   half(std::integral_constant<int, 0>{});
@@ -1058,7 +1175,12 @@
     static_assert(WAVES_M == 4 && WAVES_N == 2 && TM == 2 && TN == 4 && std::is_same<typename storage_of<MT>::type, TOut>::value, "LN256: the 8-wave 256 x 256 tile");
     static_assert(STAGES * STAGE_BYTES >= 128 * 256 * 4, "LN256: the transposition tile must fit the ring");
     if constexpr (!BUF) wait_vmcnt<0>();
-    conv_epilogue_lds256<TOut, ACT>(p, acc, m_blk, n_blk, wm, wn, lane, tid, smem, z);
+    if constexpr (LN256 == 2) {
+      static_assert(ACT == 0 && is_h16<MT>::value, "LN256 = 2: the paired epilogue of vt_time_upsample3, 16-bit types");
+      conv_epilogue_lds256_pair<TOut>(p, acc, m_blk, n_blk, wm, wn, lane, tid, smem);
+    } else {
+      conv_epilogue_lds256<TOut, ACT>(p, acc, m_blk, n_blk, wm, wn, lane, tid, smem, z);
+    }
     return;
   }
   if constexpr (WAVES_M == 2 && WAVES_N == 2 && TM == 2 && TN == 2 && STAGES * STAGE_BYTES >= 128 * 128 * 4) {
@@ -1097,7 +1219,7 @@
   const unsigned long long cb = a.tmode == VT_TPAD_CACHE ? (unsigned long long)a.B * a.ncache * a.Hi * a.Wi * a.Cin * sizeof(MT) : 0ull;
   const bool cache_ok = a.tmode != VT_TPAD_CACHE ||
                         (FAST && (nbatch == 1 || a.ksplit) && a.prof == nullptr && cb < 0xFFFF0000ull && ((long long)a.Ho * a.Wo) % BM == 0 && a.ups_t == 0);
-  const bool buf = conv_buf() && xb < 0xFFFF0000ull && wb < 0xFFFF0000ull && cache_ok &&
+  const bool buf = desc_gather_fits(a, (int)sizeof(MT)) && cache_ok &&
                    a.KH <= 8 && a.KW <= 8;
   VT_CHECK_ARG(!a.ksplit || buf, "vt_conv: split-K needs the descriptor gather");
   a.tskip = (FAST && buf && vt_opt(OPT_CONV_TSKIP) != 0 && a.tmode == VT_TPAD_ZERO && a.KT > 1 && a.pt > 0 && a.ups_t == 0 && !a.ksplit &&
@@ -1106,12 +1228,14 @@
   constexpr int SCHED_BUF = !(EIGHT && FAST) ? 0
                             : (is_split3<MT>::value ? ((ROWB == 64 && STAGES == 4) ? 5 : 0)
                                : ((ROWB == kRowBytes && STAGES == 2) ? (is_h16<MT>::value ? 2 : 1) : 0));
-  const void* kern;
+  const void* kern = nullptr;
   if (buf) {
     a.x_bytes = (unsigned)xb;
     a.w_bytes = (unsigned)wb;
     a.c_bytes = (unsigned)cb;
     kern = reinterpret_cast<const void*>(&conv_igemm_glds_kernel<MT, TOut, WAVES_M, WAVES_N, TM, TN, FAST, ROWB, STAGES, true, LN256, false, SCHED_BUF, ACT>);
+  } else if constexpr (LN256 == 2) {
+    VT_CHECK_ARG(false, "vt_time_upsample3: the descriptor gather is required (option conv_buf, tensors below 4 GiB)");
   } else {
     kern = reinterpret_cast<const void*>(&conv_igemm_glds_kernel<MT, TOut, WAVES_M, WAVES_N, TM, TN, FAST, ROWB, STAGES, false, LN256, false, 0, ACT>);
   }
@@ -1164,6 +1288,12 @@
           return v.ln256 ? launch_tile<MT, TOut, TILE_256x256, true, 1, 4, 64>(a, nbatch, stream) : launch_tile<MT, TOut, TILE_256x256, true, 0, 4, 64>(a, nbatch, stream);
         }
       } else if constexpr (std::is_same<MT, TOut>::value) {
+        if constexpr (is_h16<MT>::value) {
+          if (v.ln256 == 2) {
+            VT_CHECK_VARIANT(v.fast && v.stages == 2 && v.rowb == kRowBytes && a.pair_v != nullptr);
+            return launch_tile<MT, TOut, TILE_256x256, true, 2>(a, nbatch, stream);
+          }
+        }
         if (v.ln256) {
           VT_CHECK_VARIANT(v.fast && v.stages == 2 && v.rowb == kRowBytes);
           return launch_tile<MT, TOut, TILE_256x256, true, 1>(a, nbatch, stream);
diff --git a/vidtok_amd/csrc/conv_select.h b/vidtok_amd/csrc/conv_select.h
--- a/vidtok_amd/csrc/conv_select.h
+++ b/vidtok_amd/csrc/conv_select.h
@@ -61,6 +61,16 @@
   return true;
 }
 
+inline bool tile256_wanted(long long tiles) {
+  const int force = vt_opt(OPT_CONV_TILE);
+  return force != 128 && (tiles >= vt_opt(OPT_CONV_TILE_MIN) || force == 256);
+}
+
+inline bool desc_gather_fits(const ConvArgs& a, int elem_bytes) {
+  const unsigned long long xb = (unsigned long long)a.B * a.Ti * a.Hi * a.Wi * a.Cin * elem_bytes, wb = (unsigned long long)a.Cout * a.ldw * elem_bytes;
+  return conv_buf() && xb < 0xFFFF0000ull && wb < 0xFFFF0000ull;
+}
+
 inline TileKind select_tile(const ConvArgs& a, int nbatch) {
   auto blocks = [&](int bm, int bn) {
     return (long long)((a.M + bm - 1) / bm) * ((a.Cout + bn - 1) / bn) * nbatch;
@@ -68,8 +78,7 @@
   const bool vec_epi = a.out_layout == VT_NDHWC && (a.ldy & 3) == 0 && (a.res_mode == VT_RES_NONE || (a.ldr & 3) == 0);
   if (a.Cout <= 32) return TILE_256x32;
   if (a.Cout <= 64) return TILE_256x64;
-  const int force = vt_opt(OPT_CONV_TILE);
-  if (a.Cout % 256 == 0 && vec_epi && force != 128 && (blocks(256, 256) >= vt_opt(OPT_CONV_TILE_MIN) || force == 256)) return TILE_256x256;
+  if (a.Cout % 256 == 0 && vec_epi && tile256_wanted(blocks(256, 256))) return TILE_256x256;
   return TILE_128x128;
 }
 
@@ -112,6 +121,21 @@
   if (tile != TILE_256x256 && tile != TILE_128x128) return 0;
   const long long clip_tiles = (((long long)a.To * a.Ho * a.Wo + 127) / 128) * ((a.Cout + 127) / 128);
   return clip_tiles <= device_cus() ? 3 : 0;
+}
+
+inline bool tup3_eligible(const vt_conv_desc* d, const ConvArgs& a, const ConvPlan& p) {
+  if (vt_opt(OPT_CONV_TUP3) == 0 || a.prof != nullptr) return false;
+  const bool h16_io = vt_is_h16(d->dtype) && d->out_dtype == d->dtype;
+  if (a.KT != 2 || a.KH != 3 || a.KW != 3 || a.st != 1 || a.sh != 1 || a.sw != 1 || a.pt != 1 || a.ph != 1 || a.pw != 1) return false;
+  if (a.tmode != VT_TPAD_ZERO || a.ups_t || a.ups_s || a.To != a.Ti || a.Ho != a.Hi || a.Wo != a.Wi) return false;
+  if (a.yt_mul != 2 || a.yt_base != 0 || a.ys_mul == 2 || a.res_mode != VT_RES_MIX) return false;
+  if (d->ln_mode != 0 && (!p.ln_fused || (a.ldn & 7) != 0)) return false;
+  ConvArgs e = a;
+  e.ln_mode = 0;
+  if (!lds256_plain_eligible(e, p.nbatch, h16_io)) return false;
+  const long long hw = (long long)a.Ho * a.Wo;
+  if (!desc_gather_fits(a, 2) || hw % 256 != 0) return false;
+  return tile256_wanted((a.To * hw / 256) * (a.Cout / 256));
 }
 
 inline int conv_decide(const vt_conv_desc* d, ConvArgs& a, ConvPlan& p, unsigned long long* prof = nullptr, int act = 0) {
diff --git a/vidtok_amd/csrc/model.cpp b/vidtok_amd/csrc/model.cpp
--- a/vidtok_amd/csrc/model.cpp
+++ b/vidtok_amd/csrc/model.cpp
@@ -77,6 +77,7 @@
   const Norm* norm = nullptr;
   bool silu = false;
   bool has_n() const { return norm != nullptr; }
+  bool tup3 = false;
 };
 struct NormRef {
   const Norm* norm = nullptr;
@@ -263,6 +264,22 @@
   shape[2] = 2;
   return o;
 }
+std::vector<float> xf_time_up3(const Param& p, std::vector<int64_t>& shape, int part, int) {
+  const int64_t co = shape[0], ci = shape[1], hw = shape[3] * shape[4];
+  const int kt = part == 2 ? 2 : 1;
+  std::vector<float> o((size_t)co * ci * kt * hw);
+  for (int64_t a = 0; a < co * ci; ++a)
+    for (int64_t s = 0; s < hw; ++s) {
+      if (part == 2) {
+        o[(a * 2 + 0) * hw + s] = p.data[(a * 3 + 0) * hw + s];
+        o[(a * 2 + 1) * hw + s] = p.data[(a * 3 + 2) * hw + s];
+      } else {
+        o[a * hw + s] = p.data[(a * 3 + 1) * hw + s];
+      }
+    }
+  shape[2] = kt;
+  return o;
+}
 std::vector<float> xf_space_parity(const Param& p, std::vector<int64_t>& shape, int py, int px) {
   const int64_t n = shape[0] * shape[1];
   std::vector<float> o((size_t)n * 4);
@@ -347,6 +364,8 @@
   Tens* ln_out = nullptr;
   bool ln_optional = false;
   bool plan_only = false;
+  bool tup3_probe = false;
+  const Tens* tup3_v = nullptr;
   int yt_mul = 1, yt_off = 0, ys = 0, ys_oh = 0, ys_ow = 0;
   float* ncthw = nullptr;
   int t_trim = 0;
@@ -417,7 +436,17 @@
       r.n = Tens(); r.norm = nullptr;
     }
   }
+  if (o.tup3_probe) {
+    vt_conv_desc q = d;
+    standins(q);
+    if (q.ln_mode != 0 && q.ln_out == nullptr) q.ln_out = (void*)16;
+    r.tup3 = vt_time_upsample3_supported(&q) == 1;
+  }
   if (o.plan_only) return r;
+  if (o.tup3_v) {
+    if (!c.dry) M_CALL(vt_time_upsample3(&d, o.tup3_v->p, o.tup3_v->ld, c.stream));
+    return r;
+  }
   {
     vt_conv_desc q = d;
     standins(q);
@@ -836,6 +865,30 @@
     const float* mf = c.m->f32(key + ".mix_factor", c.dry);
     const bool nc = c.m->noncausal();
     const std::string ck = key + ".conv" + c.m->cv();
+    if (!nc) {
+      ConvOpts o;
+      Tens probe = r.y;
+      probe.p = nullptr;
+      o.out = &r.y; o.yt_mul = 2; o.yt_off = 0; o.plan_only = true; o.tup3_probe = true;
+      if (emit_ln) { o.ln = next; o.ln_out = &probe; o.ln_optional = true; }
+      o.res = &xp; o.res_mode = VT_RES_MIX; o.mix = mf;
+      const Act q = conv(c, xp, (const void*)16, 18 * xp.ld, nullptr, g, ch, o);
+      if (q.tup3) {
+        Geom gv;
+        gv.kh = 3; gv.kw = 3; gv.ph = 1; gv.pw = 1; gv.ph_hi = 1; gv.pw_hi = 1;
+        const Act v = conv(c, xp, c.m->conv_w(ck + ".weight", xp.ld, c.dry, xf_time_up3, 3, 0), 9 * xp.ld, nullptr, gv, ch, ConvOpts());
+        ConvOpts u;
+        u.out = &r.y; u.yt_mul = 2; u.yt_off = 0; u.tup3_v = &v.y;
+        u.res = &xp; u.res_mode = VT_RES_MIX; u.mix = mf;
+        if (q.has_n()) {
+          nbuf = c.alloc(xp.B, 2 * xp.T, xp.H, xp.W, pad8(ch), c.m->dt, ch);
+          u.ln = next; u.ln_out = &nbuf;
+        }
+        conv(c, xp, c.m->conv_w(ck + ".weight", xp.ld, c.dry, xf_time_up3, 2, 0), 18 * xp.ld, c.m->f32(ck + ".bias", c.dry), g, ch, u);
+        if (q.has_n()) { r.n = nbuf; r.norm = next.norm; r.silu = next.silu; }
+        return r;
+      }
+    }
     if (emit_ln) {
       ConvOpts o;
       Tens probe = r.y;
diff --git a/vidtok_amd/csrc/options.cpp b/vidtok_amd/csrc/options.cpp
--- a/vidtok_amd/csrc/options.cpp
+++ b/vidtok_amd/csrc/options.cpp
@@ -21,6 +21,7 @@
     {"tblock_fused", 1},    {"tblock_prof_mode", 0},
     {"conv_deep", 1},       {"ws_prof_mode", 0},    {"attn_flash", 1},      {"conv_splitk", 1},
     {"conv_tskip", 1},      {"conv_in8", 1},        {"conv_tup_ln", 1},     {"conv_nt_mb", 64},
+    {"conv_tup3", 1},
 };
 std::atomic<int> g_val[OPT_COUNT];
 std::once_flag g_once;
diff --git a/vidtok_amd/csrc/options.h b/vidtok_amd/csrc/options.h
--- a/vidtok_amd/csrc/options.h
+++ b/vidtok_amd/csrc/options.h
@@ -20,6 +20,7 @@
   OPT_CONV_IN8,
   OPT_CONV_TUP_LN,
   OPT_CONV_NT_MB,
+  OPT_CONV_TUP3,
   OPT_COUNT
 };
 
diff --git a/vidtok_amd/lib.py b/vidtok_amd/lib.py
--- a/vidtok_amd/lib.py
+++ b/vidtok_amd/lib.py
@@ -145,6 +145,8 @@
     "vt_conv_work_bytes": (_I64, [C.POINTER(ConvDesc)]),
     "vt_conv_plan": (C.c_int, [C.POINTER(ConvDesc), C.POINTER(_I32)]),
     "vt_conv_profile": (C.c_int, [C.POINTER(ConvDesc), _P, _P]),
+    "vt_time_upsample3_supported": (C.c_int, [C.POINTER(ConvDesc)]),
+    "vt_time_upsample3": (C.c_int, [C.POINTER(ConvDesc), _P, _I32, _P]),
     "vt_frames_work_floats": (_I64, [_I32, _I32, _I32]),
     "vt_frames_u8_to_ncthw": (C.c_int, [_P, _I32, _I32, _I32, _I32, _I32, _I32, _I32, _P, _I32, _I32, _I32, _I32, _P, _P]),
     "vt_ncthw_to_frames_u8": (C.c_int, [_P, _I32, _I32, _I32, _I32, _I32, _P, _I32, _I32, _P]),
diff --git a/vidtok_amd/modules.py b/vidtok_amd/modules.py
--- a/vidtok_amd/modules.py
+++ b/vidtok_amd/modules.py
@@ -8,8 +8,8 @@
 from . import lib as L
 from . import ops
 from .ops import ConvGeom
-from .packing import (ConvSite, space_upsample_parity_mix, space_upsample_parity_weights, time_upsample_parity_mix,
-                      time_upsample_parity_weights)
+from .packing import (ConvSite, space_upsample_parity_mix, space_upsample_parity_weights, time_upsample3_mix, time_upsample3_weights,
+                      time_upsample_parity_mix, time_upsample_parity_weights)
 
 
 def _check_norm(norm_type):
@@ -292,7 +292,7 @@
                     mix=functools.partial(time_upsample_parity_mix, early=early))
 
 
-def time_parity_upsample(sites, x, dt, mix_factor, next_norm):
+def time_parity_upsample(sites, x, dt, mix_factor, next_norm, tup3=None):
     B, T, H, W, _C = x.shape
     cout = sites[0].cout
     ld = ops.pad_channels(cout)
@@ -303,6 +303,12 @@
     def alloc_n():
         return (torch.empty if ld == cout else torch.zeros)(y.shape, dtype=dt, device=x.device)
 
+    if tup3 is not None:
+        su, sv = tup3
+        r = ops.time_upsample3(x, lambda: su.rows(dt, x.shape[-1]), lambda: sv.run(x, dt), mix_factor, y, cout=cout,
+                               **(dict(ln=emit["ln"], ln_out=alloc_n) if emit else {}))
+        if r is not None:
+            return Normed(y, r[1], next_norm[0], next_norm[1]) if isinstance(r, tuple) else y
     for par, site in enumerate(sites):
         r = site.run(x, dt, res=x, res_mode=L.VT_RES_MIX, mix_factor=mix_factor, out=y, out_t=(2, par),
                      **(dict(emit, ln_out=(alloc_n if n is None else n), ln_optional=True) if emit else {}))
@@ -328,6 +334,11 @@
         self.causal_cache = None
         g = ConvGeom(kt=2, kh=3, kw=3, pt=1, ph=1, pw=1, ph_hi=1, pw_hi=1)
         self.parity_sites = (time_parity_class(self.conv.conv, g, early=True), time_parity_class(self.conv.conv, g, early=False))
+        self.tup3_sites = (ConvSite(self.conv.conv, ops.TUP3_GEOM, transform=functools.partial(time_upsample3_weights, part="u"),
+                                    mix=functools.partial(time_upsample3_mix, part="u")),
+                           ConvSite(self.conv.conv, ConvGeom(kh=3, kw=3, ph=1, pw=1, ph_hi=1, pw_hi=1), bias=False,
+                                    transform=functools.partial(time_upsample3_weights, part="v"),
+                                    mix=functools.partial(time_upsample3_mix, part="v")))
 
     def _interp_v11(self, x):
         n, T = self.num_temp_upsample, x.shape[1]
@@ -361,7 +372,7 @@
         x = plain(x)
         mf = self.mix_factor.detach()
         if self.version == "v1_0":
-            return time_parity_upsample(self.parity_sites, x, dt, mf, next_norm)
+            return time_parity_upsample(self.parity_sites, x, dt, mf, next_norm, tup3=self.tup3_sites)
         xi = self._interp_v11(x)
         return _wrap(self.conv.run(xi, dt, res=xi, res_mode=L.VT_RES_MIX, mix_factor=mf, **_emit(next_norm)), next_norm)
 
diff --git a/vidtok_amd/ops.py b/vidtok_amd/ops.py
--- a/vidtok_amd/ops.py
+++ b/vidtok_amd/ops.py
@@ -18,6 +18,16 @@
     L.check(lib.vt_conv(C.byref(d), _stream()), what)
     if CONV_RECORD is not None:
         CONV_RECORD.append((d, keep, (d.B * d.To * d.Ho * d.Wo * max(1, d.nbatch), d.Cout, d.KT * d.KH * d.KW * d.Cin)))
+
+
+class TimeUp3Desc(L.ConvDesc):
+
+    v_ptr = None
+    ldv = 0
+
+
+def time_upsample3_supported(d) -> bool:
+    return bool(L.load().vt_time_upsample3_supported(C.byref(d)))
 
 
 def conv_plan(d):
@@ -37,6 +47,9 @@
             _, q, k, vT, bias, o, scale = d
             L.check(lib.vt_flash_attention(_ptr(q), _ptr(k), _ptr(vT), _ptr(bias), _ptr(o), _DT[q.dtype], q.shape[0], q.shape[1], q.shape[2],
                                            vT.shape[2], scale, _stream()), "vt_flash_attention(replay)")
+            continue
+        if isinstance(d, TimeUp3Desc):
+            L.check(lib.vt_time_upsample3(C.byref(d), C.c_void_p(d.v_ptr), d.ldv, _stream()), "vt_time_upsample3(replay)")
             continue
         if conv_kernel_only and d.ln_mode != 0 and not conv_plan(d)["ln_fused"]:
             d2 = L.ConvDesc()
@@ -191,6 +204,66 @@
     return (y, n) if ln_keep_y else n
 
 
+TUP3_GEOM = ConvGeom(kt=2, kh=3, kw=3, pt=1, ph=1, pw=1, ph_hi=1, pw_hi=1)
+
+
+def time_upsample3(x, wu, v, mix_factor, out, *, cout: int, ln=None, ln_out=None):
+    if not x.is_cuda or x.dtype not in _DT:
+        return None
+    lib = L.load()
+    _chk(x, "time_upsample3.x"); _chk(out, "time_upsample3.out")
+    B, T, H, W, Cin = x.shape
+    ld = out.shape[4]
+    assert out.dtype == x.dtype and tuple(out.shape[:4]) == (B, 2 * T, H, W) and ld >= cout, (out.shape, x.shape)
+    assert mix_factor.dtype == torch.float32 and mix_factor.is_cuda
+    g = TUP3_GEOM
+    d = TimeUp3Desc()
+    d.x, d.w, d.y = x.data_ptr(), x.data_ptr(), out.data_ptr()
+    d.B, d.Ti, d.Hi, d.Wi, d.Cin = B, T, H, W, Cin
+    d.To, d.Ho, d.Wo, d.Cout = T, H, W, cout
+    d.ldw, d.ldy = g.kt * g.kh * g.kw * Cin, ld
+    d.KT, d.KH, d.KW, d.st, d.sh, d.sw, d.pt, d.ph, d.pw = g.kt, g.kh, g.kw, 1, 1, 1, g.pt, g.ph, g.pw
+    d.tmode = L.VT_TPAD_ZERO
+    d.res_mode, d.res, d.res_tshift, d.Tr, d.ldr, d.mix_factor = L.VT_RES_MIX, x.data_ptr(), 0, T, Cin, mix_factor.data_ptr()
+    d.out_layout, d.dtype, d.out_dtype, d.nbatch = L.VT_NDHWC, _DT[x.dtype], _DT[x.dtype], 1
+    d.yt_mul, d.yt_off = 2, 0
+    if ln is not None:
+        gamma, beta, eps, silu = ln
+        assert gamma.dtype == torch.float32 and beta.dtype == torch.float32 and gamma.numel() >= cout and beta.numel() >= cout
+        d.ln_gamma, d.ln_beta, d.ln_out = gamma.data_ptr(), beta.data_ptr(), out.data_ptr()
+        d.ln_mode, d.ln_keep_y, d.ldn, d.ln_eps = (2 if silu else 1), 1, ld, float(eps)
+        try:
+            fused = conv_plan(d)["ln_fused"]
+        except L.VtError:
+            fused = False
+        if not fused:
+            d.ln_gamma = d.ln_beta = d.ln_out = None
+            d.ln_mode = 0
+            ln = None
+    if not time_upsample3_supported(d):
+        return None
+    w, bias = wu() if callable(wu) else wu
+    _chk(w, "time_upsample3.w")
+    assert w.dtype == x.dtype and tuple(w.shape) == (cout, d.ldw), (w.shape, w.dtype)
+    assert bias is None or (bias.dtype == torch.float32 and bias.numel() >= cout)
+    d.w, d.bias = w.data_ptr(), (bias.data_ptr() if bias is not None else None)
+    v = v() if callable(v) else v
+    _chk(v, "time_upsample3.v")
+    assert v.dtype == x.dtype and tuple(v.shape[:4]) == (B, T, H, W) and v.shape[4] >= cout, (v.shape, x.shape)
+    d.v_ptr, d.ldv = v.data_ptr(), v.shape[4]
+    n = None
+    if ln is not None:
+        n = ln_out() if callable(ln_out) else ln_out
+        if n is None:
+            n = (torch.zeros if ld != cout else torch.empty)(out.shape, dtype=out.dtype, device=x.device)
+        assert n.shape == out.shape and n.dtype == out.dtype and n.is_contiguous()
+        d.ln_out = n.data_ptr()
+    L.check(lib.vt_time_upsample3(C.byref(d), C.c_void_p(d.v_ptr), d.ldv, _stream()), "vt_time_upsample3")
+    if CONV_RECORD is not None:
+        CONV_RECORD.append((d, (x, w, bias, out, mix_factor, n, ln, v), (B * T * H * W, cout, d.ldw)))
+    return out if n is None else (out, n)
+
+
 def _tblock_desc(x, tmode, c=None, caches=None, cache_offset=0):
     d = L.TBlockDesc()
     B, T, H, W, ld = x.shape
@@ -320,6 +393,9 @@
         es = 2
         px = d.B * d.T * d.HW
         return px * d.ld * es * (1 + (1 if d.keep_y else 0) + (1 if d.ln_next_mode else 0)) + 2 * d.C * 3 * d.C * es
+    if isinstance(d, TimeUp3Desc):
+        px = d.B * d.To * d.Ho * d.Wo
+        return px * d.Cin * 2 + d.Cout * d.ldw * 2 + px * d.Cout * 2 * (1 + 2 + (2 if d.ln_mode != 0 else 0))
     es = 2 if d.dtype in (L.VT_BF16, L.VT_F16) else 4
     eo = 4 if d.out_dtype == L.VT_F32 else 2
     nb = max(1, d.nbatch)
diff --git a/vidtok_amd/packing.py b/vidtok_amd/packing.py
--- a/vidtok_amd/packing.py
+++ b/vidtok_amd/packing.py
@@ -79,6 +79,23 @@
     return first + second
 
 
+def time_upsample3_weights(weight: torch.Tensor, part: str):
+    w = weight.detach().to(torch.float32)
+    assert w.dim() == 5 and w.shape[2] == 3 and part in ("u", "v")
+    if part == "u":
+        return torch.stack([w[:, :, 0], w[:, :, 2]], dim=2)
+    return w[:, :, 1:2]
+
+
+def time_upsample3_mix(kdims, part: str):
+    kt, kh, kw = kdims
+    assert kt == 3 and part in ("u", "v")
+    s = kh * kw
+    if part == "u":
+        return [[0 * s + i] for i in range(s)] + [[2 * s + i] for i in range(s)]
+    return [[1 * s + i] for i in range(s)]
+
+
 def space_upsample_parity_mix(kdims, py: int, px: int):
     assert tuple(kdims) == (3, 3)
     rows = [[0], [1, 2]] if py == 0 else [[0, 1], [2]]
@@ -143,17 +160,18 @@
 
 class ConvSite:
 
-    def __init__(self, conv, geom, *, clip_tmode=L.VT_TPAD_ZERO, transform=None, mix=None, pin_native=False):
+    def __init__(self, conv, geom, *, clip_tmode=L.VT_TPAD_ZERO, transform=None, mix=None, pin_native=False, bias=True):
         self.conv, self.geom, self.clip_tmode = conv, geom, clip_tmode
+        self.bias = bias
         self.cin, self.cout = conv.in_channels, conv.out_channels
         self.pack = PackedCache(transform, pin_native, mix)
         self._dgrad = None
 
     def rows(self, dt, cin_stored):
-        return self.pack.get(self.conv.weight, self.conv.bias, dt, cin_stored=cin_stored)
+        return self.pack.get(self.conv.weight, self.conv.bias if self.bias else None, dt, cin_stored=cin_stored)
 
     def run(self, x, dt, *, tmode=L.VT_TPAD_ZERO, cache=None, **kw):
-        w, b = self.pack.get(self.conv.weight, self.conv.bias, dt, cin_stored=x.shape[-1])
+        w, b = self.rows(dt, x.shape[-1])
         return ops.conv(x, w, b, self.geom, cout=self.cout, tmode=tmode, cache=cache, **kw)
 
     def run_clip(self, x, dt, **kw):
```

Measured after the change: 954.6 frames/s, median of 6. 1.04x the previous value.
